# SebastianBitsch/SRGAN-ST

Measured on AMD Instinct MI355X. Metric: HR images/sec (96px x4, B=16/GPU) G+D+ST-loss step, higher is better.
Workload: dtype f32; 1 GPU; srgan_x4_hr96_b16_G+D+ST-loss step: adv+mse+st, D updated every step (train.py:116-164; BASELINE metric); global_batch=16, hr=96, lr=24, parallelism=dp1, hip_graph=True, d_update_interval=1, d_sr_forward=run: all three discriminator forwards of train.py:136,155,158

## Files before the change

include/srganst.h:

```cpp
#ifndef SRGANST_H
#define SRGANST_H
#include <stdint.h>
#ifdef __cplusplus
extern "C" {
#endif

const char* sst_last_error(void);
int sst_version(void);
const char* sst_arch(void);
int sst_clear_error(void);
int sst_reload_env(void);

int sst_st_loss_workspace(int B, int H, int W, int64_t* partial_floats);
int sst_st_loss_fwd(const float* sr, const float* gt, float* loss, float* gS, float* partials,
                    unsigned* counter, int B, int H, int W, float sigma, float rho, int normalize,
                    void* stream);
int sst_st_loss_bwd(const float* sr, const float* gS, float* dsr, const float* scale_dev,
                    float scale_host, int accumulate, int B, int H, int W, float sigma, float rho,
                    void* stream);
int sst_st_maps_workspace(int B, int H, int W, int64_t* tile_floats);
int sst_st_maps(const float* x, const float* gt, float* Sx, float* Sgt, float* Fx, float* Fgt, float* d, float* tile_sums,
                int B, int H, int W, float sigma, float rho, int normalize, void* stream);
int sst_st_pixel_loss_fwd(const float* sr, const float* gt, float* loss, float* gS, float* partials, unsigned* counter,
                          float* pix_loss, float* pix_partials, int pix_mode, int B, int H, int W, float sigma, float rho,
                          int normalize, void* stream);
int sst_st_pixel_loss_bwd(const float* sr, const float* gt, const float* gS, float* dsr, const float* scale_dev, float scale_host,
                          float pix_weight, int pix_mode, int accumulate, int B, int H, int W, float sigma, float rho,
                          void* stream);

int64_t sst_conv_packed_floats(int Cout, int Cin, int ksize);
int sst_conv_pack(const float* w, float* wp, int Cout, int Cin, int ksize, int mode, void* stream);
int sst_conv_pack_multi(const void* jobs, int njobs, int total_blocks, void* stream);
int sst_conv_mtiles(int B, int Ho, int Wo);
int sst_conv_stat_tiles(int B, int H, int W, int Cin, int Cout, int ksize, int stride);
const char* sst_conv_kernel_name(int B, int H, int W, int Cin, int Cout, int ksize, int stride, int out_mode, int fused_in);
const char* sst_conv_wgrad_kernel_name(int B, int H, int W, int Cin, int Cout, int ksize, int stride, int njobs);
long sst_debug_big_tile_launches(void);
long sst_debug_band_launches(void);
long sst_debug_wgrad_band_launches(void);
int sst_debug_mfma_peak(float* out, int blocks, int iters, void* stream);
int sst_debug_bf16x3(const float* A, const float* B, float* C32, float* C3, int K, int mode, int blocks, void* stream);
int sst_debug_stamp(unsigned long long* out, int slot, void* stream);
int sst_conv_fwd(const float* x, const float* wp, float* y, float* y_pre, const float* bias,
                 const float* in_scale, const float* in_shift, const float* in_slope,
                 float in_slope_const, int in_act, const float* residual, float* stats,
                 float* stats_cnt, int out_mode, int B, int H, int W, int Cin, int Cout, int ksize,
                 int stride, void* stream);
int sst_conv_pipe_supported(int B, int H, int W, int Cin, int Cout, int ksize, int stride);
int sst_conv_pipe_stat_tiles(int B, int H, int W, int Cin, int Cout, int ksize, int stride);
int64_t sst_conv_pipe_ws_floats(int B, int H, int W, int Cin, int Cout, int ksize, int stride);
int sst_conv_pipe_fwd(const float* x, const float* wp, float* y, const float* bias, const float* in_scale,
                      const float* in_shift, const float* in_slope, float in_slope_const, int in_act, float* stats,
                      float* stats_cnt, const float* epi_y, const float* epi_scale, const float* epi_shift,
                      const float* epi_slope, float epi_slope_const, int epi_act, float* epi_partial, float* ws, int B,
                      int H, int W, int Cin, int Cout, int ksize, int stride, void* stream);
int sst_conv_pipe_groups_ok(int B, int H, int W, int Cin, int Cout, int ksize, int stride, int grp_images);
int sst_conv_pipe_fwd_grp(const float* x, const float* wp, float* y, const float* bias, const float* in_scale,
                          const float* in_shift, const float* in_slope, float in_slope_const, int in_act, float* stats,
                          float* stats_cnt, const float* epi_y, const float* epi_scale, const float* epi_shift,
                          const float* epi_slope, float epi_slope_const, int epi_act, float* epi_partial, float* ws, int B,
                          int H, int W, int Cin, int Cout, int ksize, int stride, int grp_images, void* stream);
int sst_conv_ns_supported(int B, int H, int W, int Cin, int Cout, int ksize, int stride, int out_mode);
int sst_conv_ns_fwd(const float* x, const float* wp, float* y, const float* bias, const float* in_scale,
                    const float* in_shift, const float* in_slope, float in_slope_const, int in_act, float* stats,
                    float* stats_cnt, const float* epi_y, const float* epi_scale, const float* epi_shift,
                    const float* epi_slope, float epi_slope_const, int epi_act, float* epi_partial, int B, int H, int W,
                    int Cin, int Cout, int ksize, int stride, int out_mode, int grp_images, void* stream);
int sst_conv_s2_dgrad_pipe_supported(int B, int H, int W, int Cin, int Cout);
int64_t sst_conv_s2_dgrad_pipe_ws_floats(int B, int H, int W, int Cin, int Cout);
int sst_conv_s2_dgrad_pipe(const float* dy, const float* wp, float* dx, float* ws, int B, int H, int W, int Cin, int Cout,
                           void* stream);
int sst_conv_s2_dgrad_pipe_stat_tiles(int B, int H, int W, int Cin, int Cout);
int sst_conv_s2_dgrad_pipe_bwdstats(const float* dy, const float* wp, float* dx, float* ws, const float* epi_y,
                                    const float* epi_scale, const float* epi_shift, const float* epi_slope,
                                    float epi_slope_const, int epi_act, float* epi_partial, int B, int H, int W, int Cin,
                                    int Cout, void* stream);
int sst_conv_s2_dgrad_pipe_groups_ok(int B, int H, int W, int Cin, int Cout, int grp_images);
int sst_conv_s2_dgrad_pipe_bwdstats_grp(const float* dy, const float* wp, float* dx, float* ws, const float* epi_y,
                                    const float* epi_scale, const float* epi_shift, const float* epi_slope,
                                    float epi_slope_const, int epi_act, float* epi_partial, int B, int H, int W, int Cin,
                                    int Cout, int grp_images, void* stream);
int sst_conv_dgrad_bwdstats(const float* x, const float* wp, float* y, const float* residual, const float* epi_y,
                            const float* epi_scale, const float* epi_shift, const float* epi_slope,
                            float epi_slope_const, int epi_act, float* epi_partial, int B, int H, int W, int Cin,
                            int Cout, int ksize, void* stream);
int sst_conv_acc_supported(int B, int H, int W, int Cin, int Cout, int ksize, int stride);
int sst_conv_fwd_acc(const float* x, const float* in2, float* side_out, const float* ones, const float* wp, float* y,
                     const float* bias, const float* in_slope, float in_slope_const, int in_act, const double* in_acc,
                     const float* in_gamma, const float* in_beta, float in_n, float eps, float momentum, float* o_mean,
                     float* o_rstd, float* o_scale, float* o_shift, float* run_mean, float* run_var, double* st_acc,
                     int nrep, int B, int H, int W, int Cin, int Cout, int ksize, void* stream);
int sst_conv_dgrad_fused_acc(const float* g, const float* y2, const float* in_scale, const float* in_shift,
                             const float* in_slope, float in_slope_const, int in_act, float* dy_out, const float* wp,
                             float* out, const float* residual, const float* epi_y, const float* epi_scale,
                             const float* epi_shift, const float* epi_slope, float epi_slope_const, int epi_act,
                             const double* bw_in_acc, const float* mean, const float* rstd, const float* gamma, float n,
                             float* dgamma, float* dbeta, float* dslope, double* bw_st_acc, int nrep, int B, int H,
                             int W, int Cin, int Cout, int ksize, void* stream);
int sst_bn_finalize_acc(const double* acc, int nrep, int C, float n, const float* gamma, const float* beta,
                        float* run_mean, float* run_var, float* mean, float* rstd, float* scale, float* shift,
                        float eps, float momentum, void* stream);
int sst_conv_fwd_resin(const float* x, const float* y2, const float* ones, const float* bn_scale, const float* bn_shift,
                       float* h_out, const float* wp, float* y, const float* bias, float* stats, float* stats_cnt,
                       int B, int H, int W, int Cin, int Cout, int ksize, void* stream);
int sst_conv_dgrad_fused(const float* g, const float* y2, const float* cA, const float* cB, const float* cC,
                         const float* in_scale, const float* in_shift, const float* in_slope, float in_slope_const,
                         int in_act, float* dy_out, const float* wp, float* out, const float* residual,
                         const float* epi_y, const float* epi_scale, const float* epi_shift, const float* epi_slope,
                         float epi_slope_const, int epi_act, float* epi_partial, int B, int H, int W, int Cin, int Cout,
                         int ksize, void* stream);
int sst_conv_wgrad_chunks(int B, int Ho, int Wo, int Cin, int Cout, int ksize);
int sst_conv_wgrad_chunks2(int B, int H, int W, int Cin, int Cout, int ksize, int stride, int njobs);
int sst_conv_wgrad(const float* x, const float* dy, float* slab, float* dw, const float* in_scale,
                   const float* in_shift, const float* in_slope, float in_slope_const, int in_act,
                   int B, int H, int W, int Cin, int Cout, int stride, int ksize, int accumulate,
                   void* stream);
int sst_conv_wgrad_groups_ok(int B, int H, int W, int Cin, int Cout, int ksize, int stride, int grp_images);
int sst_conv_wgrad_grp(const float* x, const float* dy, float* slab, float* dw, const float* in_scale,
                   const float* in_shift, const float* in_slope, float in_slope_const, int in_act,
                   int B, int H, int W, int Cin, int Cout, int stride, int ksize, int accumulate,
                       int grp_images, void* stream);
int sst_conv_wgrad_pending_reduce(int B, int H, int W, int Cin, int Cout, int ksize, int stride, int has_in_scale, int in_act);
int sst_wgrad_reduce_multi(const void* jobs, int njobs, void* stream);
int sst_wgrad_c3_supported(int C, int ksize);
int64_t sst_wgrad_c3_slab_floats(int B, int H, int W, int C);
int sst_wgrad_c3(const float* big, const float* small, float* slab, float* dw, const float* in_slope,
                 float in_slope_const, int in_act, int kind, int B, int H, int W, int C, int accumulate,
                 void* stream);

int64_t sst_conv9_c3_packed_floats(int Cout_eff);
int sst_conv9_c3_pack(const float* w, float* wp, int Cout, int Cin, int mode, void* stream);
int sst_conv9_c3_fwd(const float* x, const float* wp, float* y, const float* bias, int B, int H, int W,
                     int Cout, void* stream);
int64_t sst_conv9_to3_packed_floats(int C);
int sst_conv9_to3_pack(const float* w, float* wp, int C, void* stream);
int sst_conv9_to3_fwd(const float* x, const float* wp, float* y, float* y_pre, const float* bias,
                      const float* in_slope, float in_slope_const, int in_act, int B, int H, int W, int C,
                      void* stream);

int64_t sst_conv_s2_dgrad_packed_floats(int Cout, int Cin);
int sst_conv_s2_dgrad_pack(const float* w, float* wp, int Cout, int Cin, void* stream);
int sst_conv_s2_dgrad(const float* dy, const float* wp, float* dx, int B, int H, int W, int Cin, int Cout,
                      void* stream);
int sst_conv_s2_dgrad_tiles(int B, int H, int W);
const char* sst_conv_s2_dgrad_kernel_name(int B, int H, int W, int Cin, int Cout, int fused);
int sst_conv_s2_dgrad_fused(const float* g, const float* y2, const float* cA, const float* cB, const float* cC,
                            const float* in_scale, const float* in_shift, const float* in_slope, float in_slope_const,
                            int in_act, float* dy_out, const float* wp, float* dx, const float* epi_y,
                            const float* epi_scale, const float* epi_shift, const float* epi_slope, float epi_slope_const,
                            int epi_act, float* epi_partial, int B, int H, int W, int Cin, int Cout, void* stream);

int sst_conv_wgrad_grouped(const void* jobs, int njobs, int B, int H, int W, int Cin, int Cout, int stride,
                           int ksize, int accumulate, void* stream);

int sst_bn_finalize(const float* stats, const float* cnt, int ntiles, int C, const float* gamma,
                    const float* beta, float* run_mean, float* run_var, float* mean, float* rstd,
                    float* scale, float* shift, float eps, float momentum, void* stream);
int sst_bn_finalize_grp(const float* stats, const float* cnt, int ntiles, int C, int groups, const float* gamma,
                        const float* beta, float* run_mean, float* run_var, float* mean, float* rstd, float* scale,
                        float* shift, float eps, float momentum, void* stream);
int sst_bn_eval_affine(const float* gamma, const float* beta, const float* run_mean,
                       const float* run_var, float* scale, float* shift, int C, float eps, void* stream);
int sst_bn_residual(const float* y, const float* scale, const float* shift, const float* res,
                    const float* res_slope, float* out, int64_t R, int C, void* stream);
int sst_bwd_reduce_blocks(int64_t R, int C);
int sst_bwd_reduce(const float* g, const float* g2, const float* y, const float* scale,
                   const float* shift, const float* slope, float slope_const, int act, float* partial,
                   int64_t R, int C, void* stream);
int sst_bwd_finalize(const float* partial, int nblk, int C, float n, const float* mean,
                     const float* rstd, const float* gamma, float* dgamma, float* dbeta, float* cA,
                     float* cB, float* cC, float* dslope, int accumulate, void* stream);
int sst_bwd_reduce_grp(const float* g, const float* g2, const float* y, const float* scale, const float* shift,
                       const float* slope, float slope_const, int act, float* partial, int64_t R, int C, int groups,
                       void* stream);
int sst_bwd_finalize_grp(const float* partial, int nblk, int C, float n, int groups, const float* mean, const float* rstd,
                         const float* gamma, float* dgamma, float* dbeta, float* cA, float* cB, float* cC, int accumulate,
                         void* stream);
int sst_bwd_apply_grp(const float* g, const float* g2, const float* y, const float* scale, const float* shift,
                      const float* slope, float slope_const, int act, const float* cA, const float* cB, const float* cC,
                      float* dy, int64_t R, int C, int groups, void* stream);
int sst_bwd_finalize_wide(const float* partial, int nblk, int C, float n, const float* mean, const float* rstd,
                          const float* gamma, float* dgamma, float* dbeta, float* cA, float* cB, float* cC,
                          float* dslope, int accumulate, float* scratch, unsigned* counter, void* stream);
int sst_act_bwd_partial_blocks(int64_t stored_rows);
int sst_act_bwd_partial(const float* g, const float* g2, const float* y, const float* slope, float slope_const,
                        float* dy, float* partial, int64_t R, int C, int unshuffle_H, int unshuffle_W, void* stream);
int sst_bwd_apply(const float* g, const float* g2, const float* y, const float* scale,
                  const float* shift, const float* slope, float slope_const, int act, const float* cA,
                  const float* cB, const float* cC, float* dy, int64_t R, int C, int unshuffle_H,
                  int unshuffle_W, void* stream);
int sst_add(const float* a, const float* b, float* out, int64_t n, void* stream);

int sst_transpose(const float* src, float* dst, int B, int C, int H, int W, int to_nchw, void* stream);
int sst_feat_loss_fwd(const float* x, const float* gt, const float* scale, const float* shift, float slope, int C,
                      float* loss, float* partials, unsigned* counter, int64_t n, int mode, void* stream);
int sst_feat_loss_bwd(const float* x, const float* gt, const float* scale, const float* shift, float slope, int C,
                      float* dx, const float* scale_dev, float scale_host, int accumulate, int64_t n, int mode,
                      void* stream);
int sst_transpose_affine(const float* src, float* dst, int B, int C, int H, int W, int to_nchw,
                         const float* scale, const float* shift, void* stream);
int sst_maxpool_relu_fwd(const float* y, float* out, int B, int H, int W, int C, void* stream);
int sst_maxpool_relu_bwd(const float* g, const float* y, float* dy, int B, int H, int W, int C, void* stream);
int sst_clamp_bwd_blocks(int B, int H, int W);
int sst_clamp_bwd(const float* g, const float* pre, float* out, float* partial, float* dbias,
                  int accumulate, int B, int C, int H, int W, void* stream);
int sst_pixel_loss_blocks(int64_t n);
int sst_pixel_loss_fwd(const float* x, const float* gt, float* loss, float* partials, unsigned* counter,
                       int64_t n, int mode, void* stream);
int sst_pixel_loss_bwd(const float* x, const float* gt, float* dx, const float* scale_dev,
                       float scale_host, int accumulate, int64_t n, int mode, void* stream);
int sst_bce_logits(const float* logits, float target, float* loss, float* dlogits,
                   const float* scale_dev, float scale_host, int n, void* stream);
int sst_bicubic(const float* x, float* y, const float* wy, const int* iy, const float* wx, const int* ix,
                int64_t planes, int H, int W, int oh, int ow, int Ty, int Tx, int round_grid, void* stream);
int sst_gather_batch(const uint8_t* src, int64_t N, const int* idx, int B, int H, int W, const float* lut, float* gt, float* lr,
                     const float* wy, const int* iy, const float* wx, const int* ix, int oh, int ow, int Ty, int Tx,
                     void* stream);
int sst_gather_crops(const uint8_t* arena, int64_t arena_bytes, const int64_t* table, int64_t N, const int* desc, int B, int S,
                     const float* lut, float* gt, float* lr, const float* wy, const int* iy, const float* wx, const int* ix,
                     int oh, int ow, int Ty, int Tx, int span, void* stream);
int sst_image_metrics_workspace(int B, int H, int W, int64_t* partial_doubles);
int sst_image_metrics(const float* sr, const float* hr, int B, int H, int W, double* out, uint8_t* sr_u8, uint8_t* hr_u8,
                      double* workspace, void* stream);
int sst_bb_blocks(int B, int H, int W);
int sst_bb_feature_dim(int mode);
int sst_bb_patches(const float* img, float* cand, float* cnrm, int B, int H, int W, int ncand_total, int cand_off,
                   int mode, const float* st_mats, void* stream);
int sst_bb_match(const float* sr, const float* cand, const float* cnrm, int* ind, float* dsr, float* partials, int B,
                 int H, int W, int ncand, float alpha, float beta, int criterion_l2, int mode, const float* st_mats,
                 void* stream);
int sst_bb_match_dist(const float* sr, const float* cand, const float* cnrm, int* ind, float* dsr, float* partials, int B,
                 int H, int W, int ncand, float alpha, float beta, int criterion_l2, int mode, const float* st_mats, int dist_l1,
                      void* stream);
int sst_bbg_patches(int H, int W, int k, int pad, int stride);
int sst_bbg_blocks(int B, int np);
int sst_bbg_unfold(const float* img, float* table, float* nrm, int B, int H, int W, int k, int pad, int stride, int nrows_total,
                   int row_off, void* stream);
int sst_bbg_match(const float* srf, const float* cand, const float* cnrm, int* ind, float* gfeat, float* partials, int B, int np,
                  int ncand, int D, float alpha, float beta, int criterion_l2, int dist_l1, void* stream);
int sst_bbg_fold(const float* gfeat, float* dsr, int B, int H, int W, int k, int pad, int stride, void* stream);
int sst_weighted_sum(const float* const* terms, const float* weights, int n, float* out, float* weighted,
                     void* stream);

int sst_linear_ksplit(int M, int N, int K);
int sst_linear_fwd(const float* x, const float* w, const float* bias, float* y, float* slab, int M, int N,
                   int K, void* stream);
int sst_linear_dgrad(const float* dy, const float* w, float* dx, int M, int N, int K, int nhwc_C,
                     int nhwc_HW, void* stream);
int sst_linear_wgrad(const float* dy, const float* x, float* dw, float* db, int M, int N, int K,
                     int accumulate, void* stream);
int sst_head_fwd(const float* h, const float* w, const float* b, float* y, int M, int N, int K, float slope,
                 void* stream);
int sst_head_bwd(const float* h, const float* w, const float* dy, float* dh, float* dw, float* db, int M,
                 int N, int K, float slope, int accumulate, void* stream);
int sst_flatten_act(const float* y, const float* scale, const float* shift, float slope, int act,
                    float* flat, int B, int HW, int C, void* stream);
int sst_flatten_act_grp(const float* y, const float* scale, const float* shift, float slope, int act,
                        float* flat, int B, int HW, int C, int grp_images, void* stream);

int sst_adam_flat(float* p, const float* g, float* m, float* v, int64_t n, const float* lr, float* steps,
                  int nsteps, double beta1, double beta2, double eps, double weight_decay, void* stream);

#ifdef __cplusplus
}
#endif
#endif
```

srgan-st_amd/csrc/api.hip:

```cpp
#include "common.h"
#include <cstring>

static thread_local char g_err[512] = "";

int sst_set_error(int code, const char* fmt, ...) {
  va_list ap;
  va_start(ap, fmt);
  vsnprintf(g_err, sizeof(g_err), fmt, ap);
  va_end(ap);
  return code;
}

SST_API const char* sst_last_error(void) { return g_err; }

#include <cstdlib>
#include <mutex>
namespace {
struct EnvEntry { char name[40]; char value[24]; bool set; };
constexpr int ENV_MAX = 64;
EnvEntry g_env[ENV_MAX];
int g_env_n = 0;
std::mutex g_env_mu;
}
const char* sst_env(const char* name) {
  std::lock_guard<std::mutex> lk(g_env_mu);
  for (int i = 0; i < g_env_n; ++i)
    if (!strcmp(g_env[i].name, name)) return g_env[i].set ? g_env[i].value : nullptr;
  const char* v = std::getenv(name);
  if (g_env_n == ENV_MAX || strlen(name) >= sizeof(g_env[0].name)) return v;
  EnvEntry& e = g_env[g_env_n++];
  snprintf(e.name, sizeof(e.name), "%s", name);
  e.set = v != nullptr;
  snprintf(e.value, sizeof(e.value), "%s", v ? v : "");
  return e.set ? e.value : nullptr;
}
SST_API int sst_reload_env(void) {
  std::lock_guard<std::mutex> lk(g_env_mu);
  g_env_n = 0;
  return SST_OK;
}
SST_API int sst_version(void) { return 100; }
SST_API const char* sst_arch(void) { return "gfx950"; }
SST_API int sst_clear_error(void) { g_err[0] = 0; return (int)hipGetLastError(); }

typedef float f32x16_t __attribute__((ext_vector_type(16)));
template <int SHAPE>
__global__ __launch_bounds__(256) void mfma_peak_kernel(float* out, int iters) {
  f32x16_t acc[4];
#pragma unroll
  for (int k = 0; k < 4; ++k)
#pragma unroll
    for (int r = 0; r < 16; ++r) acc[k][r] = 0.f;
  unsigned ua = threadIdx.x * 2654435761u + blockIdx.x, ub = ua ^ 0x9e3779b9u;
  for (int i = 0; i < iters; ++i) {
    ua = ua * 1664525u + 1013904223u;
    ub = ub * 22695477u + 1u;
    const float a = __uint_as_float((ua >> 9) | 0x3f800000u) - 1.5f, b = __uint_as_float((ub >> 9) | 0x3f800000u) - 1.5f;
#pragma unroll
    for (int k = 0; k < 4; ++k) acc[k] = __builtin_amdgcn_mfma_f32_32x32x2f32(a, b, acc[k], 0, 0, 0);
  }
  float s = 0.f;
#pragma unroll
  for (int k = 0; k < 4; ++k)
#pragma unroll
    for (int r = 0; r < 16; ++r) s += acc[k][r];
  if (s == 12345.678f) out[0] = s;
}
SST_API int sst_debug_mfma_peak(float* out, int blocks, int iters, void* stream) {
  SST_REQUIRE(out && blocks > 0 && iters > 0, "sst_debug_mfma_peak: bad argument");
  mfma_peak_kernel<0><<<blocks, 256, 0, sst_stream(stream)>>>(out, iters);
  SST_LAUNCH_CHECK("mfma_peak_kernel");
  return SST_OK;
}

typedef __bf16 bf16x8_t __attribute__((ext_vector_type(8)));
__device__ __forceinline__ void split3(float x, __bf16& a, __bf16& b, __bf16& c) {
  a = (__bf16)x;
  const float r1 = x - (float)a;
  b = (__bf16)r1;
  c = (__bf16)(r1 - (float)b);
}
__global__ __launch_bounds__(64) void bf16x3_probe_kernel(const float* __restrict__ A, const float* __restrict__ B, float* __restrict__ C32,
                                                          float* __restrict__ C3, int K) {
  const int lane = threadIdx.x, li = lane & 31, lh = lane >> 5;
  f32x16_t acc32, acc3;
#pragma unroll
  for (int r = 0; r < 16; ++r) acc32[r] = acc3[r] = 0.f;
  for (int k = 0; k < K; k += 2)
    acc32 = __builtin_amdgcn_mfma_f32_32x32x2f32(A[li * K + k + lh], B[(k + lh) * 32 + li], acc32, 0, 0, 0);
  for (int k = 0; k < K; k += 16) {
    bf16x8_t a[3], b[3];
#pragma unroll
    for (int j = 0; j < 8; ++j) {
      __bf16 t0, t1, t2;
      split3(A[li * K + k + 8 * lh + j], t0, t1, t2);
      a[0][j] = t0; a[1][j] = t1; a[2][j] = t2;
      split3(B[(k + 8 * lh + j) * 32 + li], t0, t1, t2);
      b[0][j] = t0; b[1][j] = t1; b[2][j] = t2;
    }
    acc3 = __builtin_amdgcn_mfma_f32_32x32x16_bf16(a[2], b[0], acc3, 0, 0, 0);
    acc3 = __builtin_amdgcn_mfma_f32_32x32x16_bf16(a[1], b[1], acc3, 0, 0, 0);
    acc3 = __builtin_amdgcn_mfma_f32_32x32x16_bf16(a[0], b[2], acc3, 0, 0, 0);
    acc3 = __builtin_amdgcn_mfma_f32_32x32x16_bf16(a[1], b[0], acc3, 0, 0, 0);
    acc3 = __builtin_amdgcn_mfma_f32_32x32x16_bf16(a[0], b[1], acc3, 0, 0, 0);
    acc3 = __builtin_amdgcn_mfma_f32_32x32x16_bf16(a[0], b[0], acc3, 0, 0, 0);
  }
#pragma unroll
  for (int r = 0; r < 16; ++r) {
    const int row = (r & 3) + 8 * (r >> 2) + 4 * lh;
    C32[row * 32 + li] = acc32[r];
    C3[row * 32 + li] = acc3[r];
  }
}
typedef unsigned u32x4_t __attribute__((ext_vector_type(4)));
__global__ __launch_bounds__(256) void bf16x3_rate_kernel(float* out, int iters) {
  f32x16_t acc[4];
#pragma unroll
  for (int k = 0; k < 4; ++k)
#pragma unroll
    for (int r = 0; r < 16; ++r) acc[k][r] = 0.f;
  u32x4_t a[3], b[3];
  unsigned ua = threadIdx.x * 2654435761u + blockIdx.x;
#pragma unroll
  for (int t = 0; t < 3; ++t)
#pragma unroll
    for (int j = 0; j < 4; ++j) {
      ua = ua * 1664525u + 1013904223u;
      a[t][j] = (ua & 0x807F807Fu) | 0x3F803F80u;
      ua = ua * 1664525u + 1013904223u;
      b[t][j] = (ua & 0x807F807Fu) | 0x3F803F80u;
    }
  for (int i = 0; i < iters; i += 12) {
#pragma unroll
    for (int u = 0; u < 12; ++u) {
      ua = ua * 1664525u + 1013904223u;
      a[u % 3][u / 3] ^= ua & 0x807F807Fu;
      b[(u + 1) % 3][u / 3] ^= (ua >> 3) & 0x807F807Fu;
      bf16x8_t av[3], bv[3];
#pragma unroll
      for (int t = 0; t < 3; ++t) {
        av[t] = __builtin_bit_cast(bf16x8_t, a[t]);
        bv[t] = __builtin_bit_cast(bf16x8_t, b[t]);
      }
#pragma unroll
      for (int k = 0; k < 4; ++k) {
        acc[k] = __builtin_amdgcn_mfma_f32_32x32x16_bf16(av[2], bv[0], acc[k], 0, 0, 0);
        acc[k] = __builtin_amdgcn_mfma_f32_32x32x16_bf16(av[1], bv[1], acc[k], 0, 0, 0);
        acc[k] = __builtin_amdgcn_mfma_f32_32x32x16_bf16(av[0], bv[2], acc[k], 0, 0, 0);
        acc[k] = __builtin_amdgcn_mfma_f32_32x32x16_bf16(av[1], bv[0], acc[k], 0, 0, 0);
        acc[k] = __builtin_amdgcn_mfma_f32_32x32x16_bf16(av[0], bv[1], acc[k], 0, 0, 0);
        acc[k] = __builtin_amdgcn_mfma_f32_32x32x16_bf16(av[0], bv[0], acc[k], 0, 0, 0);
      }
    }
  }
  float s = 0.f;
#pragma unroll
  for (int k = 0; k < 4; ++k)
#pragma unroll
    for (int r = 0; r < 16; ++r) s += acc[k][r];
  if (s == 12345.678f) out[0] = s;
}
SST_API int sst_debug_bf16x3(const float* A, const float* B, float* C32, float* C3, int K, int mode, int blocks, void* stream) {
  if (mode == 0) {
    SST_REQUIRE(A && B && C32 && C3 && K > 0 && K % 16 == 0, "sst_debug_bf16x3: bad argument");
    bf16x3_probe_kernel<<<1, 64, 0, sst_stream(stream)>>>(A, B, C32, C3, K);
  } else {
    SST_REQUIRE(C32 && K > 0 && blocks > 0, "sst_debug_bf16x3: bad argument");
    bf16x3_rate_kernel<<<blocks, 256, 0, sst_stream(stream)>>>(C32, K);
  }
  SST_LAUNCH_CHECK("bf16x3 probe");
  return SST_OK;
}

__global__ void stamp_kernel(unsigned long long* out, int slot) { out[slot] = wall_clock64(); }
SST_API int sst_debug_stamp(unsigned long long* out, int slot, void* stream) {
  SST_REQUIRE(out && slot >= 0, "sst_debug_stamp: bad argument");
  stamp_kernel<<<1, 1, 0, sst_stream(stream)>>>(out, slot);
  SST_LAUNCH_CHECK("stamp_kernel");
  return SST_OK;
}
```

srgan-st_amd/csrc/common.h:

```cpp
#pragma once
#include <hip/hip_runtime.h>
#include <cstdarg>
#include <cstdio>
#include <cstdint>

#define SST_API extern "C" __attribute__((visibility("default")))

enum : int {
  SST_OK = 0,
  SST_ERR_ARG = -1,
  SST_ERR_UNSUPPORTED = -2,
  SST_ERR_HIP = -3,
};

int sst_set_error(int code, const char* fmt, ...);

#define SST_REQUIRE(cond, ...)                                   \
  do {                                                           \
    if (!(cond)) return sst_set_error(SST_ERR_ARG, __VA_ARGS__); \
  } while (0)

#define SST_LAUNCH_CHECK(name)                                                                   \
  do {                                                                                           \
    hipError_t e_ = hipGetLastError();                                                           \
    if (e_ != hipSuccess) return sst_set_error(SST_ERR_HIP, "%s: %s", name, hipGetErrorString(e_)); \
  } while (0)

const char* sst_env(const char* name);

static inline hipStream_t sst_stream(void* s) { return reinterpret_cast<hipStream_t>(s); }

__device__ __forceinline__ float wave_sum(float v) {
#pragma unroll
  for (int o = 32; o > 0; o >>= 1) v += __shfl_xor(v, o, 64);
  return v;
}

template <int NT>
__device__ __forceinline__ float block_sum(float v, float* red) {
  v = wave_sum(v);
  const int wid = threadIdx.x >> 6, lane = threadIdx.x & 63;
  __syncthreads();
  if (lane == 0) red[wid] = v;
  __syncthreads();
  float t = 0.f;
#pragma unroll
  for (int i = 0; i < NT / 64; ++i) t += red[i];
  return t;
}

__device__ __forceinline__ double wave_sum_d(double v) {
#pragma unroll
  for (int o = 32; o > 0; o >>= 1) v += __shfl_xor(v, o, 64);
  return v;
}
template <int NT>
__device__ __forceinline__ double block_sum_d(double v, double* red) {
  v = wave_sum_d(v);
  const int wid = threadIdx.x >> 6, lane = threadIdx.x & 63;
  __syncthreads();
  if (lane == 0) red[wid] = v;
  __syncthreads();
  double t = 0.0;
#pragma unroll
  for (int i = 0; i < NT / 64; ++i) t += red[i];
  return t;
}

__device__ __forceinline__ unsigned publish_and_ticket(unsigned* counter) {
  __builtin_amdgcn_fence(__ATOMIC_RELEASE, "agent");
  asm volatile("s_waitcnt vmcnt(0)" ::: "memory");
  return __hip_atomic_fetch_add(counter, 1u, __ATOMIC_RELAXED, __HIP_MEMORY_SCOPE_AGENT);
}
__device__ __forceinline__ void acquire_after_ticket() {
  __builtin_amdgcn_fence(__ATOMIC_ACQUIRE, "agent");
  asm volatile("s_waitcnt vmcnt(0)" ::: "memory");
}
__device__ __forceinline__ float load_agent(const float* p) {
  return __hip_atomic_load(p, __ATOMIC_RELAXED, __HIP_MEMORY_SCOPE_AGENT);
}

template <int NT>
__device__ __forceinline__ bool last_block_total(const float* partials, unsigned* counter, unsigned nblk, unsigned* s_flag,
                                                 float* red, float& total) {
  if (threadIdx.x == 0) *s_flag = (publish_and_ticket(counter) == nblk - 1) ? 1u : 0u;
  __syncthreads();
  if (!*s_flag) return false;
  if (threadIdx.x == 0) acquire_after_ticket();
  __syncthreads();
  float t = 0.f;
  for (unsigned i = threadIdx.x; i < nblk; i += NT) t += load_agent(partials + i);
  total = block_sum<NT>(t, red);
  if (threadIdx.x == 0) __hip_atomic_store(counter, 0u, __ATOMIC_RELAXED, __HIP_MEMORY_SCOPE_AGENT);
  return true;
}
```

srgan-st_amd/csrc/conv_fwd.hip:

```cpp
#include "conv_common.h"
#include <cstdlib>
#include "conv_epilogue.h"

int sst_launch_conv_fwd2(const Conv3Args& a, int stride, hipStream_t st);
int sst_launch_conv_band(const Conv3Args& a, int R, hipStream_t st, const BandAcc* acc);
int sst_conv_band_rows(int B, int H, int W, int Cin, int Cout, int ksize, int stride);

namespace {

constexpr int BIG_MIN_TILES = 2048;
inline bool use_big_tiles(const Conv3Args& a, int ksize) {
  if (ksize != 3 || a.Cout < 64 || a.in2 || a.side_out) return false;
  if (a.out_mode != OUT_NHWC && a.out_mode != OUT_SHUFFLE && a.out_mode != OUT_STRIDE2) return false;
  if (const char* e = sst_env("SST_CONV_BIG")) return atoi(e) != 0;
  const long tiles = (long)a.B * ((a.Ho + 7) / 8) * ((a.Wo + 7) / 8) * ((a.Cout + 63) / 64);
  return tiles >= BIG_MIN_TILES;
}

template <int KS, int S>
__device__ __forceinline__ void conv_fwd_body(const Conv3Args& a, const int bx, const int by) {
  const int KK = a.ksy * a.ksx;
  constexpr int PW = (TWO - 1) * S + KS, PH = (THO - 1) * S + KS, NP = PW * PH;
  constexpr int LDS_FLOATS = (NP * LDSC > 4 * 32 * 33) ? NP * LDSC : 4 * 32 * 33;
  __shared__ __attribute__((aligned(16))) float lds[LDS_FLOATS];
// ... 316 lines not shown
#pragma unroll
        for (int i = 0; i < 6; ++i) bq[(g + 1) & 1][i] = load_b((g + 1) * 6 + i);
      }
#pragma unroll
      for (int i = 0; i < 6; ++i) {
        const int q = g * 6 + i, combo = q >> 1, cls = CLS_OF[combo], tap = TAP_OF[combo];
        const int ntx = 1 + (cls & 1), jy = tap / ntx, jx = tap - jy * ntx;
        const int ks = 2 * wave + (q & 1);
        if (ks < nks) {
          const f32x4 av = *reinterpret_cast<const f32x4*>(&lds[a_base + (jy * PW + jx) * LDSC + ks * 8]);
          const f32x4 bv = bq[g & 1][i];
#pragma unroll
          for (int j = 0; j < 4; ++j) acc[cls] = __builtin_amdgcn_mfma_f32_32x32x2f32(av[j], bv[j], acc[cls], 0, 0, 0);
        }
      }
    }
  }
  const bool tile_ok = oy0 < nh && ox0 < nw;
#pragma unroll
  for (int cls = 0; cls < 4; ++cls) {
    Conv3Args t = a;
    t.sub_y = cls >> 1;
    t.sub_x = cls & 1;
    t.Ho = nh;
    t.Wo = nw;
    t.in2 = nullptr;
    t.side_out = nullptr;
    if (FUSED && a.epi_partial) t.epi_partial = a.epi_partial + (size_t)c.tile_base[cls] * 3 * a.Cout;
    if (!FUSED) t.epi_partial = nullptr;
    conv_tile_epilogue(t, lds, sstat, acc[cls], b, oy0, ox0, nf, mt, tile_ok, tid, wave, lane);
  }
}

__global__ __launch_bounds__(CONV_NT) void conv3_c3in_kernel(const float* __restrict__ x, const float* __restrict__ wp,
                                                             const float* __restrict__ bias, float* __restrict__ y, int B, int H, int W,
                                                             int Cout) {
  extern __shared__ __attribute__((aligned(16))) float xs[];
  const int RS = (W + 2) * 3 + 1;
  const int b = blockIdx.x / H, oy = blockIdx.x - b * H;
  for (int i = threadIdx.x; i < 3 * RS; i += CONV_NT) {
    const int r = i / RS, o = i - r * RS;
    const int px = o / 3 - 1, iy = oy - 1 + r;
    float v = 0.f;
    if (o < (W + 2) * 3 && (unsigned)px < (unsigned)W && (unsigned)iy < (unsigned)H)
      v = x[(((size_t)b * H + iy) * W + px) * 3 + (o - (px + 1) * 3)];
    xs[i] = v;
  }
  const int nq = Cout >> 2;
  const int cq = threadIdx.x % nq, pl = threadIdx.x / nq, npl = CONV_NT / nq;
  const int co = cq * 4;
  float w[27][4];
#pragma unroll
  for (int t = 0; t < 9; ++t)
#pragma unroll
    for (int ci = 0; ci < 3; ++ci)
#pragma unroll
      for (int j = 0; j < 4; ++j) w[t * 3 + ci][j] = wp[((((co + j) >> 5) * 9 + t) * 512 + ((co + j) & 31)) * 4 + ci];
  f32x4 bv = {0.f, 0.f, 0.f, 0.f};
  if (bias) bv = *reinterpret_cast<const f32x4*>(bias + co);
  __syncthreads();
  for (int ox = pl; ox < W; ox += npl) {
    f32x4 acc = bv;
#pragma unroll
    for (int ky = 0; ky < 3; ++ky) {
      const float* row = xs + ky * RS + ox * 3;
#pragma unroll
      for (int q = 0; q < 9; ++q) {
        const float v = row[q];
#pragma unroll
        for (int j = 0; j < 4; ++j) acc[j] = fmaf(v, w[ky * 9 + q][j], acc[j]);
      }
    }
    *reinterpret_cast<f32x4*>(y + (((size_t)b * H + oy) * W + ox) * Cout + co) = acc;
  }
}

constexpr int C3F_ROW = 104;
constexpr int C3F_OST = 68;
__global__ __launch_bounds__(CONV_NT) void conv3_c3in_mfma_kernel(const float* __restrict__ x, const float* __restrict__ wp,
                                                                  const float* __restrict__ bias, float* __restrict__ y, int B, int H,
                                                                  int W, int ntiles) {
  __shared__ __attribute__((aligned(16))) float ost[4][32 * C3F_OST];
  __shared__ float wl[15 * 2 * 64];
  constexpr int Cout = 64;
  const int tid = threadIdx.x, wave = __builtin_amdgcn_readfirstlane(tid >> 6), lane = tid & 63;
  const int li = lane & 31, lh = lane >> 5;
  for (int i = tid; i < 15 * 2 * 64; i += CONV_NT) {
    const int l = i & 63, h = (i >> 6) & 1, ks = i >> 7;
    const int ky = ks / 5, j = 2 * (ks - ky * 5) + (l >> 5);
    wl[i] = j < 9 ? wp[((size_t)(h * 9 + ky * 3 + j / 3) * 512 + (l & 31)) * 4 + j % 3] : 0.f;
  }
  float* const ps = ost[wave];
  const int tpr = W >> 5;
  float pv[5];
  auto load_patch = [&](int t) {
    const int b = t / (H * tpr), rem = t - b * (H * tpr);
    const int oy = rem / tpr, x0 = (rem - oy * tpr) << 5;
#pragma unroll
    for (int u = 0; u < 5; ++u) {
      const int i = lane + 64 * u;
      const int r = i / C3F_ROW, c = i - r * C3F_ROW;
      const int iy = oy - 1 + r, fx = (x0 - 1) * 3 + c;
      const bool ok = i < 3 * C3F_ROW + 8 && r < 3 && c < 102 && (unsigned)iy < (unsigned)H && (unsigned)fx < (unsigned)(W * 3);
      pv[u] = ok ? x[((size_t)b * H + iy) * W * 3 + fx] : 0.f;
    }
  };
  int t = blockIdx.x * 4 + wave;
  if (t < ntiles) load_patch(t);
  __syncthreads();
  const float* const bl = ps + li * 3 + lh;
  for (; t < ntiles; t += gridDim.x * 4) {
#pragma unroll
    for (int u = 0; u < 5; ++u) {
      const int i = lane + 64 * u;
      if (i < 3 * C3F_ROW + 8) ps[i] = pv[u];
    }
    const int tn = t + gridDim.x * 4;
    if (tn < ntiles) load_patch(tn);
    f32x16 acc[2];
#pragma unroll
    for (int h = 0; h < 2; ++h)
#pragma unroll
      for (int r = 0; r < 16; ++r) acc[h][r] = 0.f;
#pragma unroll
    for (int ky = 0; ky < 3; ++ky)
#pragma unroll
      for (int s2 = 0; s2 < 5; ++s2) {
        const float bv = bl[ky * C3F_ROW + 2 * s2];
        const int ks = ky * 5 + s2;
        acc[0] = __builtin_amdgcn_mfma_f32_32x32x2f32(wl[(ks * 2 + 0) * 64 + lane], bv, acc[0], 0, 0, 0);
        acc[1] = __builtin_amdgcn_mfma_f32_32x32x2f32(wl[(ks * 2 + 1) * 64 + lane], bv, acc[1], 0, 0, 0);
      }
#pragma unroll
    for (int h = 0; h < 2; ++h)
#pragma unroll
      for (int q = 0; q < 4; ++q) {
        const int c = 32 * h + 8 * q + 4 * lh;
        f32x4 v = {acc[h][4 * q], acc[h][4 * q + 1], acc[h][4 * q + 2], acc[h][4 * q + 3]};
        if (bias) v += *reinterpret_cast<const f32x4*>(bias + c);
        *reinterpret_cast<f32x4*>(ps + li * C3F_OST + c) = v;
      }
    const int b = t / (H * tpr), rem = t - b * (H * tpr);
    const int oy = rem / tpr, x0 = (rem - oy * tpr) << 5;
    float* const yp = y + (((size_t)b * H + oy) * W + x0) * Cout;
#pragma unroll
    for (int i = 0; i < 8; ++i) {
      const int idx = lane + 64 * i, px = idx >> 4, c4 = (idx & 15) * 4;
      *reinterpret_cast<f32x4*>(yp + (size_t)px * Cout + c4) = *reinterpret_cast<const f32x4*>(ps + px * C3F_OST + c4);
    }
  }
}

typedef float f32x4c __attribute__((ext_vector_type(4)));
__global__ __launch_bounds__(CONV_NT) void conv3_to3_kernel(const float* __restrict__ x, const float* __restrict__ wp,
                                                            float* __restrict__ y, int B, int H, int W, int nmt, int nsp) {
  extern __shared__ __attribute__((aligned(16))) float pl_all[];
  const int wave = __builtin_amdgcn_readfirstlane(threadIdx.x >> 6), lane = threadIdx.x & 63;
  const int seg = blockIdx.x * 4 + wave;
  if (seg >= B * H * nsp) return;
  const int row = seg / nsp, Ws = W / nsp, xb = (seg - row * nsp) * Ws;
  const int b = row / H, oy = row - b * H;
  const int lm = lane & 15, lg = lane >> 4;
  float* const pl = pl_all + (size_t)wave * nmt * 16 * 12;
  float bw[3][4][4];
  {
    const int tx = lm / 3, ci = lm - tx * 3;
#pragma unroll
    for (int ty = 0; ty < 3; ++ty)
#pragma unroll
      for (int q = 0; q < 4; ++q)
#pragma unroll
        for (int t = 0; t < 4; ++t) {
          const int co = 16 * q + 4 * lg + t, tap = ty * 3 + tx;
          bw[ty][q][t] = lm < 9 ? wp[(size_t)(tap * 8 + (co >> 3)) * 256 + (((co & 7) >> 2) * 32 + ci) * 4 + (co & 3)] : 0.f;
        }
  }
  auto load_tile = [&](int mt, f32x4c (&a)[3][4]) {
    const int xp = xb + mt * 16 + lm - 1;
#pragma unroll
    for (int ty = 0; ty < 3; ++ty) {
      const int iy = oy - 1 + ty;
      const bool ok = (unsigned)iy < (unsigned)H && (unsigned)xp < (unsigned)W;
      const float* src = x + (((size_t)b * H + (ok ? iy : 0)) * W + (ok ? xp : 0)) * 64 + 4 * lg;
#pragma unroll
      for (int q = 0; q < 4; ++q) {
        const f32x4c v = *reinterpret_cast<const f32x4c*>(src + 16 * q);
        a[ty][q] = ok ? v : f32x4c{0.f, 0.f, 0.f, 0.f};
      }
    }
  };
  f32x4c ac[3][4], an[3][4];
  load_tile(0, ac);
  for (int mt = 0; mt < nmt; ++mt) {
    if (mt + 1 < nmt) load_tile(mt + 1, an);
    f32x4c acc = {0.f, 0.f, 0.f, 0.f};
#pragma unroll
    for (int ty = 0; ty < 3; ++ty)
#pragma unroll
      for (int q = 0; q < 4; ++q)
#pragma unroll
        for (int t = 0; t < 4; ++t) acc = __builtin_amdgcn_mfma_f32_16x16x4f32(ac[ty][q][t], bw[ty][q][t], acc, 0, 0, 0);
    if (lm < 9) {
#pragma unroll
      for (int r = 0; r < 4; ++r) pl[(mt * 16 + 4 * lg + r) * 12 + lm] = acc[r];
    }
#pragma unroll
    for (int ty = 0; ty < 3; ++ty)
#pragma unroll
      for (int q = 0; q < 4; ++q) ac[ty][q] = an[ty][q];
  }
  float* const out = y + (((size_t)b * H + oy) * W + xb) * 3;
  for (int i = lane; i < 3 * Ws; i += 64) {
    const int xo = i / 3, ci = i - xo * 3;
    out[i] = (pl[xo * 12 + ci] + pl[(xo + 1) * 12 + 3 + ci]) + pl[(xo + 2) * 12 + 6 + ci];
  }
}

__global__ void pack_conv_kernel(const float* __restrict__ w, float* __restrict__ wp, int Cout, int Cin, int KK,
                                 int mode, int64_t total) {
  const int O = mode ? Cin : Cout, I = mode ? Cout : Cin;
  const int ncb = (I + 63) / 64;
  const int64_t base = packed_floats_base(O, I, KK);
  for (int64_t idx = blockIdx.x * (int64_t)blockDim.x + threadIdx.x; idx < total; idx += (int64_t)gridDim.x * blockDim.x) {
    if (idx >= base) {
      const int64_t q = idx - base;
      const int l = (q >> 2) & 63, tap = (q >> 10) % 9;
      const int o = (int)((q >> 10) / 9) * 16 + (l & 15), i = ((q >> 8) & 3) * 16 + (l >> 4) * 4 + (q & 3);
      wp[idx] = mode == 0 ? w[((size_t)o * Cin + i) * KK + tap] : w[((size_t)i * Cin + o) * KK + (KK - 1 - tap)];
      continue;
    }
    const int j = idx & 3;
    const int l = (idx >> 2) & 63;
    const int ks = (idx >> 8) & 7;
    int64_t rest = idx >> 11;
    const int tap = rest % KK;
    rest /= KK;
    const int cbk = rest % ncb;
    const int of = rest / ncb;
    const int o = of * 32 + (l & 31);
    const int i = cbk * 64 + ks * 8 + (l >> 5) * 4 + j;
    float v = 0.f;
    if (of < (O + 31) / 32 && o < O && i < I) {
      if (mode == 0)
        v = w[((size_t)o * Cin + i) * KK + tap];
      else
        v = w[((size_t)i * Cin + o) * KK + (KK - 1 - tap)];
    }
    wp[idx] = v;
  }
}

struct PackJob {
  const float* w;
  float* wp;
  int Cout, Cin, KK, mode;
  long long total;
  long long block_begin;
};
constexpr int PM_MAXJOBS = 512;
__global__ __launch_bounds__(256) void pack_multi_kernel(const PackJob* __restrict__ jobs, int njobs) {
  __shared__ long long s_begin[PM_MAXJOBS];
  for (int j = threadIdx.x; j < njobs; j += 256) s_begin[j] = jobs[j].block_begin;
  __syncthreads();
  int lo = 0, hi = njobs - 1;
  while (lo < hi) {
    const int mid = (lo + hi + 1) >> 1;
    if (s_begin[mid] <= (long long)blockIdx.x) lo = mid; else hi = mid - 1;
  }
  const PackJob jb = jobs[lo];
  if (jb.mode >= 2) {
    const long long base = ((long long)blockIdx.x - jb.block_begin) * 1024;
#pragma unroll
    for (int u = 0; u < 4; ++u) {
      const long long idx = base + u * 256 + threadIdx.x;
      if (idx >= jb.total) break;
      if (jb.mode == 5) { jb.wp[idx] = 0.f; continue; }
      if (jb.mode == 6) { reinterpret_cast<long long*>(jb.wp)[idx] += jb.Cout; continue; }
      jb.wp[idx] = jb.mode == 4 ? pack_to3_value(jb.w, idx, jb.Cin) : pack_c3_value(jb.w, idx, jb.Cout, jb.Cin, jb.mode - 2);
    }
    return;
  }
  const int O = jb.mode ? jb.Cin : jb.Cout, I = jb.mode ? jb.Cout : jb.Cin;
  const int ncb = (I + 63) / 64;
  const unsigned wl = (unsigned)((long long)blockIdx.x - jb.block_begin);
  const unsigned bbase = (unsigned)packed_floats_base(O, I, jb.KK), total = (unsigned)jb.total;
  if (jb.KK == 9) {
    __shared__ float tile[64 * 145];
    const unsigned nhalf = (unsigned)((O + 31) / 32) * ncb * 9 * 2;
    const bool band = wl >= nhalf + PACK_PAD / 1024;
    if (!band && wl >= nhalf) {
#pragma unroll
      for (int u = 0; u < 4; ++u) jb.wp[wl * 1024 + u * 256 + threadIdx.x] = 0.f;
      return;
    }
    if (!band) {
      const unsigned ngrp = nhalf / 9;
      if (wl >= ngrp) return;
      const int h = wl & 1, cbk = (wl >> 1) % (unsigned)ncb, of = (wl >> 1) / (unsigned)ncb;
      const int o0 = of * 32, i0 = cbk * 64 + h * 32;
      float v[36];
#pragma unroll
      for (int k = 0; k < 36; ++k) {
        const int e = k * 256 + threadIdx.x;
        const int r = e / 288, c = e - r * 288, q = c / 9;
        v[k] = 0.f;
        if (jb.mode == 0) {
          if (o0 + r < O && i0 + q < I) v[k] = jb.w[((size_t)(o0 + r) * jb.Cin + i0) * 9 + c];
        } else {
          if (i0 + r < I && o0 + q < O) v[k] = jb.w[((size_t)(i0 + r) * jb.Cin + o0) * 9 + c];
        }
      }
#pragma unroll
      for (int k = 0; k < 36; ++k) {
        const int e = k * 256 + threadIdx.x;
        const int r = e / 288, c = e - r * 288;
        tile[r * 289 + c] = v[k];
      }
      __syncthreads();
      for (int tap = 0; tap < 9; ++tap) {
        float* dst = jb.wp + ((size_t)((of * ncb + cbk) * 9 + tap) * 2 + h) * 1024;
#pragma unroll
        for (int u = 0; u < 4; ++u) {
          const int x = u * 256 + threadIdx.x;
          const int j = x & 3, l = (x >> 2) & 63, ks = x >> 8;
          const int ol = l & 31, il = ks * 8 + (l >> 5) * 4 + j;
          dst[x] = jb.mode == 0 ? tile[ol * 289 + il * 9 + tap] : tile[il * 289 + ol * 9 + (8 - tap)];
        }
      }
      return;
    }
    const unsigned wb = wl - nhalf - PACK_PAD / 1024;
    if (wb >= (unsigned)(O / 16)) return;
    const int o0 = wb * 16;
    {
      float v[36];
      const int RL = jb.mode == 0 ? 576 : 144;
#pragma unroll
      for (int k = 0; k < 36; ++k) {
        const int e = k * 256 + threadIdx.x;
        const int r = e / RL, c = e - r * RL;
        v[k] = jb.mode == 0 ? jb.w[((size_t)(o0 + r) * jb.Cin) * 9 + c] : jb.w[((size_t)r * jb.Cin + o0) * 9 + c];
      }
#pragma unroll
      for (int k = 0; k < 36; ++k) {
        const int e = k * 256 + threadIdx.x;
        const int r = e / RL, c = e - r * RL;
        tile[r * (RL + 1) + c] = v[k];
      }
    }
    __syncthreads();
    for (int tap = 0; tap < 9; ++tap) {
      float* dst = jb.wp + bbase + ((size_t)wb * 9 + tap) * 1024;
#pragma unroll
      for (int u = 0; u < 4; ++u) {
        const int x = u * 256 + threadIdx.x;
        const int l = (x >> 2) & 63;
        const int ol = l & 15, i = (x >> 8) * 16 + (l >> 4) * 4 + (x & 3);
        dst[x] = jb.mode == 0 ? tile[ol * 577 + i * 9 + tap] : tile[i * 145 + ol * 9 + (8 - tap)];
      }
    }
    return;
  }
  const unsigned base = wl * 1024;
  const unsigned top = base >> 11;
  int tap = top % (unsigned)jb.KK;
  const unsigned rr = top / (unsigned)jb.KK;
  int a2 = (int)(rr % (unsigned)ncb) * 64, a1 = (int)(rr / (unsigned)ncb) * 32;
  tap = __builtin_amdgcn_readfirstlane(tap); a1 = __builtin_amdgcn_readfirstlane(a1); a2 = __builtin_amdgcn_readfirstlane(a2);
#pragma unroll
  for (int u = 0; u < 4; ++u) {
    const unsigned idx = base + u * 256 + threadIdx.x;
    if (idx >= total) break;
    const int j = idx & 3, l = (idx >> 2) & 63, ks = (idx >> 8) & 7;
    const int o = a1 + (l & 31), i = a2 + ks * 8 + (l >> 5) * 4 + j;
    float v = 0.f;
    if (a1 < ((O + 31) / 32) * 32 && o < O && i < I) {
      if (jb.mode == 0)
        v = jb.w[((size_t)o * jb.Cin + i) * jb.KK + tap];
      else
        v = jb.w[((size_t)i * jb.Cin + o) * jb.KK + (jb.KK - 1 - tap)];
    }
    jb.wp[idx] = v;
  }
}

__host__ __device__ inline int64_t s2_class_offset(int cls, int Cin, int Cout) {
  int64_t off = 0;
  for (int c = 0; c < cls; ++c) off += packed_floats(Cin, Cout, (1 + (c >> 1)) * (1 + (c & 1)));
  return off;
}
__global__ void pack_s2_dgrad_kernel(const float* __restrict__ w, float* __restrict__ wp, int Cout, int Cin) {
  if (blockIdx.y == 4) {
    const int O = Cin, I = Cout, ncb = (I + 63) / 64;
    float* dst = wp + s2_class_offset(4, Cin, Cout);
    const int64_t total = packed_floats_base(O, I, 9);
    for (int64_t idx = blockIdx.x * (int64_t)blockDim.x + threadIdx.x; idx < total; idx += (int64_t)gridDim.x * blockDim.x) {
      const int j = idx & 3, l = (idx >> 2) & 63, ks = (idx >> 8) & 7;
      int64_t rest = idx >> 11;
      const int combo = rest % 9;
      rest /= 9;
      const int cbk = rest % ncb;
      const int of = rest / ncb;
      const int o = of * 32 + (l & 31), i = cbk * 64 + ks * 8 + (l >> 5) * 4 + j;
      float v = 0.f;
      if (of < (O + 31) / 32 && o < O && i < I) {
        const int cls = combo == 0 ? 0 : (combo < 3 ? 1 : (combo < 5 ? 2 : 3));
        const int tap = combo == 0 ? 0 : (combo < 3 ? combo - 1 : (combo < 5 ? combo - 3 : combo - 5));
        const int py = cls >> 1, px = cls & 1, ntx = 1 + px;
        const int jy = tap / ntx, jx = tap - jy * ntx;
        const int ky = py ? (jy ? 0 : 2) : 1, kx = px ? (jx ? 0 : 2) : 1;
        v = w[(((size_t)i * Cin + o) * 3 + ky) * 3 + kx];
      }
      dst[idx] = v;
    }
    return;
  }
  const int cls = blockIdx.y, py = cls >> 1, px = cls & 1;
  const int nty = 1 + py, ntx = 1 + px, KKc = nty * ntx;
  const int O = Cin, I = Cout, ncb = (I + 63) / 64;
  float* dst = wp + s2_class_offset(cls, Cin, Cout);
  const int64_t total = packed_floats(O, I, KKc);
  for (int64_t idx = blockIdx.x * (int64_t)blockDim.x + threadIdx.x; idx < total; idx += (int64_t)gridDim.x * blockDim.x) {
    const int j = idx & 3, l = (idx >> 2) & 63, ks = (idx >> 8) & 7;
    int64_t rest = idx >> 11;
    const int tap = rest % KKc;
    rest /= KKc;
    const int cbk = rest % ncb;
    const int of = rest / ncb;
    const int o = of * 32 + (l & 31), i = cbk * 64 + ks * 8 + (l >> 5) * 4 + j;
    float v = 0.f;
    if (of < (O + 31) / 32 && o < O && i < I) {
      const int jy = tap / ntx, jx = tap - jy * ntx;
      const int ky = py ? (jy ? 0 : 2) : 1, kx = px ? (jx ? 0 : 2) : 1;
      v = w[(((size_t)i * Cin + o) * 3 + ky) * 3 + kx];
    }
    dst[idx] = v;
  }
}

}

SST_API int64_t sst_conv_packed_floats(int Cout, int Cin, int ksize) { return packed_floats(Cout, Cin, ksize * ksize); }

SST_API int sst_conv_pack(const float* w, float* wp, int Cout, int Cin, int ksize, int mode, void* stream) {
  SST_REQUIRE(w && wp && Cout > 0 && Cin > 0 && (ksize == 3 || ksize == 9) && (mode == 0 || mode == 1),
              "sst_conv_pack: bad argument");
  const int O = mode ? Cin : Cout, I = mode ? Cout : Cin;
  const int64_t total = packed_floats(O, I, ksize * ksize);
  const int blocks = (int)((total + 255) / 256 < 2048 ? (total + 255) / 256 : 2048);
  pack_conv_kernel<<<blocks, 256, 0, sst_stream(stream)>>>(w, wp, Cout, Cin, ksize * ksize, mode, total);
  SST_LAUNCH_CHECK("pack_conv_kernel");
  return SST_OK;
}

SST_API int sst_conv_pack_multi(const void* jobs, int njobs, int total_blocks, void* stream) {
  SST_REQUIRE(jobs && njobs > 0 && njobs <= PM_MAXJOBS && total_blocks > 0, "sst_conv_pack_multi: bad argument (at most %d jobs)", PM_MAXJOBS);
  static_assert(sizeof(PackJob) == 48, "PackJob layout");
  pack_multi_kernel<<<total_blocks, 256, 0, sst_stream(stream)>>>(reinterpret_cast<const PackJob*>(jobs), njobs);
  SST_LAUNCH_CHECK("pack_multi_kernel");
  return SST_OK;
}

SST_API int sst_conv_mtiles(int B, int Ho, int Wo) { return B * ((Ho + THO - 1) / THO) * ((Wo + TWO - 1) / TWO); }

SST_API int sst_conv_stat_tiles(int B, int H, int W, int Cin, int Cout, int ksize, int stride) {
  const int R = sst_conv_band_rows(B, H, W, Cin, Cout, ksize, stride);
  if (R) return B * (H / R);
  const int p = ksize / 2;
  return sst_conv_mtiles(B, (H + 2 * p - ksize) / stride + 1, (W + 2 * p - ksize) / stride + 1);
}

namespace {
enum class FwdKind { TO3, C3IN_MFMA, C3IN, BAND, BIG_TILES, GENERAL };
struct FwdSel {
  FwdKind kind;
  int nsp, nmt;
  int wgs;
  int R;
  size_t lds;
  const char* name;
};

void conv_shape_args(Conv3Args& a, int B, int H, int W, int Cin, int Cout, int ksize, int stride) {
  a.B = B; a.H = H; a.W = W; a.Cin = Cin; a.Cout = Cout;
  a.ksy = a.ksx = ksize; a.pad_y = a.pad_x = ksize / 2; a.sub_y = a.sub_x = 0; a.Hy = a.Wy = 0;
  a.Ho = (H + 2 * (ksize / 2) - ksize) / stride + 1;
  a.Wo = (W + 2 * (ksize / 2) - ksize) / stride + 1;
}

FwdSel conv_fwd_select(const Conv3Args& a, int ksize, int stride, int dbg_bits) {
  FwdSel s{};
  const bool bare = ksize == 3 && stride == 1 && a.out_mode == OUT_NHWC && !a.in_scale && a.in_act == ACT_NONE && !a.residual && !a.stats &&
                    !a.y_pre && !a.epi_partial && !a.in2 && dbg_bits == 0;
  if (bare && a.Cin == 64 && a.Cout == 3 && !a.bias && !sst_env("SST_NO_TO3")) {
    s.nsp = (a.W % 32 == 0 && a.W >= 64 && !sst_env("SST_TO3_NO_SPLIT")) ? 2 : 1;
    s.nmt = (a.W / s.nsp + 2 + 15) / 16;
    s.lds = (size_t)4 * s.nmt * 16 * 12 * sizeof(float);
    if (s.lds <= 60 * 1024) {
      s.kind = FwdKind::TO3; s.name = "conv3_to3_kernel";
      return s;
    }
  }
  if (bare && a.Cin == 3 && (a.Cout & 3) == 0 && CONV_NT % (a.Cout >> 2) == 0 && !sst_env("SST_NO_C3IN")) {
    if ((a.W & 31) == 0 && a.Cout == 64 && !sst_env("SST_NO_C3IN_MFMA")) {
      s.kind = FwdKind::C3IN_MFMA; s.name = "conv3_c3in_mfma_kernel";
      s.wgs = (a.B * a.H * (a.W >> 5) + 3) / 4;
      return s;
    }
    s.lds = (size_t)3 * ((a.W + 2) * 3 + 1) * sizeof(float);
    if (s.lds <= 48 * 1024) {
      s.kind = FwdKind::C3IN; s.name = "conv3_c3in_kernel";
      return s;
    }
  }
  if (a.out_mode == OUT_NHWC && !(dbg_bits & 8)) {
    s.R = sst_conv_band_rows(a.B, a.H, a.W, a.Cin, a.Cout, ksize, stride);
    if (s.R) {
      s.kind = FwdKind::BAND; s.name = s.R * a.W / 16 == 9 ? "conv_band_kernel<9>" : "conv_band_kernel<3>";
      return s;
    }
  }
  if (dbg_bits == 0 && use_big_tiles(a, ksize)) {
    s.kind = FwdKind::BIG_TILES; s.name = stride == 1 ? "conv_fwd2_kernel<1>" : "conv_fwd2_kernel<2>";
    return s;
  }
  s.kind = FwdKind::GENERAL;
  s.name = ksize != 3 ? "conv_fwd_kernel<9, 1>" : (stride == 1 ? "conv_fwd_kernel<3, 1>" : "conv_fwd_kernel<3, 2>");
  return s;
}
}

static int conv_fwd_impl(const float* x, const float* wp, float* y, float* y_pre, const float* bias, const float* in_scale,
                         const float* in_shift, const float* in_slope, float in_slope_const, int in_act,
                         const float* residual, float* stats, float* stats_cnt, int out_mode, int B, int H, int W, int Cin,
                         int Cout, int ksize, int stride, const float* epi_y, const float* epi_scale, const float* epi_shift,
                         const float* epi_slope, float epi_slope_const, int epi_act, float* epi_partial, void* stream,
                         const float* in2 = nullptr, const float* in_cA = nullptr, const float* in_cB = nullptr,
                         const float* in_cC = nullptr, float* side_out = nullptr, const BandAcc* band_acc = nullptr) {
  SST_REQUIRE(x && wp && y, "sst_conv_fwd: null pointer");
  SST_REQUIRE(B > 0 && H > 0 && W > 0 && Cin > 0 && Cout > 0 && (stride == 1 || stride == 2) && (ksize == 3 || ksize == 9),
              "sst_conv_fwd: bad shape B=%d H=%d W=%d Cin=%d Cout=%d k=%d stride=%d", B, H, W, Cin, Cout, ksize, stride);
  SST_REQUIRE(!(ksize == 9 && stride == 2), "sst_conv_fwd: 9x9 stride 2 not built");
  SST_REQUIRE((in_scale == nullptr) == (in_shift == nullptr), "sst_conv_fwd: in_scale/in_shift must come together");
  SST_REQUIRE(!stats || stats_cnt, "sst_conv_fwd: stats needs stats_cnt");
  const int dbg_bits = out_mode >> 8;
  out_mode &= 0xff;
  SST_REQUIRE(out_mode >= 0 && out_mode <= 3, "sst_conv_fwd: bad out_mode");
  SST_REQUIRE(out_mode != OUT_SHUFFLE || (Cout & 3) == 0, "sst_conv_fwd: shuffle store needs Cout %% 4 == 0");
  SST_REQUIRE(out_mode == OUT_NHWC || (!residual && !stats && !epi_partial), "sst_conv_fwd: residual/stats only with NHWC store");
  SST_REQUIRE(!epi_partial || (epi_y && !stats && ((epi_scale == nullptr) == (epi_shift == nullptr))),
              "sst_conv_fwd: backward partials need epi_y and exclude forward stats");
  Conv3Args a;
  a.x = x; a.wp = wp; a.y = y; a.y_pre = y_pre; a.bias = bias; a.in_scale = in_scale; a.in_shift = in_shift;
  a.in_slope = in_slope; a.in_slope_const = in_slope_const; a.in_act = in_act; a.residual = residual; a.stats = stats;
  a.stats_cnt = stats_cnt; a.out_mode = out_mode; a.dbg = dbg_bits;
  a.epi_y = epi_y; a.epi_scale = epi_scale; a.epi_shift = epi_shift; a.epi_slope = epi_slope;
  a.epi_slope_const = epi_slope_const; a.epi_act = epi_act; a.epi_partial = epi_partial;
  a.in2 = in2; a.in_cA = in_cA; a.in_cB = in_cB; a.in_cC = in_cC; a.side_out = side_out;
  SST_REQUIRE(!in2 || ((Cin & 3) == 0 && stride == 1), "sst_conv_fwd: fused BN-backward input needs Cin %% 4 == 0, stride 1");
  SST_REQUIRE(!in_cA || (in2 && in_cB && in_cC), "sst_conv_fwd: cA/cB/cC need in2");
  conv_shape_args(a, B, H, W, Cin, Cout, ksize, stride);
  SST_REQUIRE(out_mode != OUT_UNSHUFFLE || ((a.Ho & 1) == 0 && (a.Wo & 1) == 0), "sst_conv_fwd: unshuffle needs even Ho,Wo");
  const int64_t mt = sst_conv_mtiles(B, a.Ho, a.Wo);
  SST_REQUIRE(mt < (1ll << 31), "sst_conv_fwd: too many tiles");
  dim3 grid((unsigned)mt, (Cout + 31) / 32);
  hipStream_t st = sst_stream(stream);
  const size_t extra_lds = (size_t)(dbg_bits >> 4) * 1024;
  a.dbg = dbg_bits & 15;
  const FwdSel s = conv_fwd_select(a, ksize, stride, dbg_bits);
  switch (s.kind) {
    case FwdKind::TO3:
      conv3_to3_kernel<<<(unsigned)((B * H * s.nsp + 3) / 4), CONV_NT, s.lds, st>>>(x, wp, y, B, H, W, s.nmt, s.nsp);
      break;
    case FwdKind::C3IN_MFMA:
      conv3_c3in_mfma_kernel<<<(unsigned)(s.wgs < 768 ? s.wgs : 768), CONV_NT, 0, st>>>(x, wp, bias, y, B, H, W, B * H * (W >> 5));
      break;
    case FwdKind::C3IN:
      conv3_c3in_kernel<<<(unsigned)(B * H), CONV_NT, s.lds, st>>>(x, wp, bias, y, B, H, W, Cout);
      break;
    case FwdKind::BAND: return sst_launch_conv_band(a, s.R, st, band_acc);
    case FwdKind::BIG_TILES: return sst_launch_conv_fwd2(a, stride, st);
    case FwdKind::GENERAL:
      if (ksize == 3 && stride == 1)
        conv_fwd_kernel<3, 1><<<grid, CONV_NT, extra_lds, st>>>(a);
      else if (ksize == 3)
        conv_fwd_kernel<3, 2><<<grid, CONV_NT, 0, st>>>(a);
      else
        conv_fwd_kernel<9, 1><<<grid, CONV_NT, 0, st>>>(a);
      break;
  }
  SST_LAUNCH_CHECK(s.name);
  return SST_OK;
}

SST_API const char* sst_conv_kernel_name(int B, int H, int W, int Cin, int Cout, int ksize, int stride, int out_mode, int fused_in) {
  Conv3Args a{};
  conv_shape_args(a, B, H, W, Cin, Cout, ksize, stride);
  a.out_mode = out_mode;
  a.in2 = fused_in ? reinterpret_cast<const float*>(1) : nullptr;
  return conv_fwd_select(a, ksize, stride, 0).name;
}

SST_API int sst_conv_fwd(const float* x, const float* wp, float* y, float* y_pre, const float* bias, const float* in_scale,
                         const float* in_shift, const float* in_slope, float in_slope_const, int in_act,
                         const float* residual, float* stats, float* stats_cnt, int out_mode, int B, int H, int W, int Cin,
                         int Cout, int ksize, int stride, void* stream) {
  return conv_fwd_impl(x, wp, y, y_pre, bias, in_scale, in_shift, in_slope, in_slope_const, in_act, residual, stats, stats_cnt,
                       out_mode, B, H, W, Cin, Cout, ksize, stride, nullptr, nullptr, nullptr, nullptr, 0.f, 0, nullptr, stream);
}

SST_API int sst_conv_dgrad_bwdstats(const float* x, const float* wp, float* y, const float* residual, const float* epi_y,
                                    const float* epi_scale, const float* epi_shift, const float* epi_slope,
                                    float epi_slope_const, int epi_act, float* epi_partial, int B, int H, int W, int Cin,
                                    int Cout, int ksize, void* stream) {
  SST_REQUIRE(epi_y && epi_partial, "sst_conv_dgrad_bwdstats: epi_y / epi_partial");
  return conv_fwd_impl(x, wp, y, nullptr, nullptr, nullptr, nullptr, nullptr, 0.f, ACT_NONE, residual, nullptr, nullptr, OUT_NHWC,
                       B, H, W, Cin, Cout, ksize, 1, epi_y, epi_scale, epi_shift, epi_slope, epi_slope_const, epi_act, epi_partial,
                       stream);
}

SST_API int sst_conv_dgrad_fused(const float* g, const float* y2, const float* cA, const float* cB, const float* cC,
                                 const float* in_scale, const float* in_shift, const float* in_slope, float in_slope_const,
                                 int in_act, float* dy_out, const float* wp, float* out, const float* residual,
                                 const float* epi_y, const float* epi_scale, const float* epi_shift, const float* epi_slope,
                                 float epi_slope_const, int epi_act, float* epi_partial, int B, int H, int W, int Cin, int Cout,
                                 int ksize, void* stream) {
  SST_REQUIRE(g && y2 && dy_out, "sst_conv_dgrad_fused: g / y2 / dy_out");
  SST_REQUIRE((epi_partial == nullptr) == (epi_y == nullptr), "sst_conv_dgrad_fused: epi_y and epi_partial come together");
  return conv_fwd_impl(g, wp, out, nullptr, nullptr, in_scale, in_shift, in_slope, in_slope_const, in_act, residual, nullptr,
                       nullptr, OUT_NHWC, B, H, W, Cin, Cout, ksize, 1, epi_y, epi_scale, epi_shift, epi_slope, epi_slope_const,
                       epi_act, epi_partial, stream, y2, cA, cB, cC, dy_out);
}

SST_API int sst_conv_fwd_resin(const float* x, const float* y2, const float* ones, const float* bn_scale, const float* bn_shift,
                               float* h_out, const float* wp, float* y, const float* bias, float* stats, float* stats_cnt, int B,
                               int H, int W, int Cin, int Cout, int ksize, void* stream) {
  SST_REQUIRE(x && y2 && ones && bn_scale && bn_shift && h_out, "sst_conv_fwd_resin: null pointer");
  return conv_fwd_impl(x, wp, y, nullptr, bias, nullptr, nullptr, nullptr, 0.f, ACT_NONE, nullptr, stats, stats_cnt, OUT_NHWC, B, H, W,
                       Cin, Cout, ksize, 1, nullptr, nullptr, nullptr, nullptr, 0.f, 0, nullptr, stream, y2, ones, bn_scale, bn_shift,
                       h_out);
}

SST_API int sst_conv_acc_supported(int B, int H, int W, int Cin, int Cout, int ksize, int stride) {
  return Cin == 64 && sst_conv_band_rows(B, H, W, Cin, Cout, ksize, stride) != 0;
}

SST_API int sst_conv_fwd_acc(const float* x, const float* in2, float* side_out, const float* ones, const float* wp, float* y,
                             const float* bias, const float* in_slope, float in_slope_const, int in_act, const double* in_acc,
                             const float* in_gamma, const float* in_beta, float in_n, float eps, float momentum, float* o_mean,
                             float* o_rstd, float* o_scale, float* o_shift, float* run_mean, float* run_var, double* st_acc,
                             int nrep, int B, int H, int W, int Cin, int Cout, int ksize, void* stream) {
  SST_REQUIRE(sst_conv_acc_supported(B, H, W, Cin, Cout, ksize, 1), "sst_conv_fwd_acc: shape not covered by the band kernel");
  SST_REQUIRE(nrep > 0 && nrep <= 16 && (in_acc || st_acc), "sst_conv_fwd_acc: no accumulator given / nrep > 16");
  SST_REQUIRE(!in_acc || (in_gamma && in_beta && in_n > 0.f), "sst_conv_fwd_acc: in_acc needs gamma / beta / n");
  SST_REQUIRE(!in2 || (side_out && ones), "sst_conv_fwd_acc: residual form needs side_out and the ones vector");
  BandAcc ba{};
  ba.st_acc = st_acc; ba.in_acc = in_acc; ba.nrep = nrep; ba.in_target = in2 ? 1 : 0;
  ba.in_gamma = in_gamma; ba.in_beta = in_beta; ba.in_n = in_n; ba.in_eps = eps; ba.momentum = momentum;
  ba.o_mean = o_mean; ba.o_rstd = o_rstd; ba.o_scale = o_scale; ba.o_shift = o_shift; ba.run_mean = run_mean; ba.run_var = run_var;
  return conv_fwd_impl(x, wp, y, nullptr, bias, nullptr, nullptr, in_slope, in_slope_const, in_act, nullptr, nullptr, nullptr, OUT_NHWC,
                       B, H, W, Cin, Cout, ksize, 1, nullptr, nullptr, nullptr, nullptr, 0.f, 0, nullptr, stream, in2, in2 ? ones : nullptr,
                       in2 ? ones : nullptr, in2 ? ones : nullptr, side_out, &ba);
}

SST_API int sst_conv_dgrad_fused_acc(const float* g, const float* y2, const float* in_scale, const float* in_shift, const float* in_slope,
                                     float in_slope_const, int in_act, float* dy_out, const float* wp, float* out,
                                     const float* residual, const float* epi_y, const float* epi_scale, const float* epi_shift,
                                     const float* epi_slope, float epi_slope_const, int epi_act, const double* bw_in_acc,
                                     const float* mean, const float* rstd, const float* gamma, float n, float* dgamma, float* dbeta,
                                     float* dslope, double* bw_st_acc, int nrep, int B, int H, int W, int Cin, int Cout, int ksize,
                                     void* stream) {
  SST_REQUIRE(sst_conv_acc_supported(B, H, W, Cin, Cout, ksize, 1), "sst_conv_dgrad_fused_acc: shape not covered by the band kernel");
  SST_REQUIRE(nrep > 0 && nrep <= 16 && (bw_in_acc || bw_st_acc), "sst_conv_dgrad_fused_acc: no accumulator given / nrep > 16");
  SST_REQUIRE(!bw_in_acc || (y2 && dy_out && mean && rstd && gamma && dgamma && dbeta && n > 0.f),
              "sst_conv_dgrad_fused_acc: bw_in_acc needs y2 / dy_out / mean / rstd / gamma / dgamma / dbeta / n");
  SST_REQUIRE(!bw_st_acc || epi_y, "sst_conv_dgrad_fused_acc: bw_st_acc needs epi_y");
  SST_REQUIRE(!y2 || dy_out, "sst_conv_dgrad_fused_acc: y2 needs dy_out");
  BandAcc ba{};
  ba.nrep = nrep;
  ba.bw_st_acc = bw_st_acc; ba.bw_in_acc = bw_in_acc; ba.bw_mean = mean; ba.bw_rstd = rstd; ba.bw_gamma = gamma; ba.bw_n = n;
  ba.o_dgamma = dgamma; ba.o_dbeta = dbeta; ba.o_dslope = dslope;
  return conv_fwd_impl(g, wp, out, nullptr, nullptr, in_scale, in_shift, in_slope, in_slope_const, in_act, residual, nullptr, nullptr,
                       OUT_NHWC, B, H, W, Cin, Cout, ksize, 1, epi_y, epi_scale, epi_shift, epi_slope, epi_slope_const, epi_act, nullptr,
                       stream, y2, nullptr, nullptr, nullptr, y2 ? dy_out : nullptr, &ba);
}

SST_API int64_t sst_conv_s2_dgrad_packed_floats(int Cout, int Cin) { return s2_class_offset(4, Cin, Cout) + packed_floats_base(Cin, Cout, 9); }
int64_t sst_conv_s2_dgrad_pipe_section(int Cout, int Cin) { return s2_class_offset(4, Cin, Cout); }

SST_API int sst_conv_s2_dgrad_pack(const float* w, float* wp, int Cout, int Cin, void* stream) {
  SST_REQUIRE(w && wp && Cout > 0 && Cin > 0, "sst_conv_s2_dgrad_pack: bad argument");
  pack_s2_dgrad_kernel<<<dim3(256, 5), 256, 0, sst_stream(stream)>>>(w, wp, Cout, Cin);
  SST_LAUNCH_CHECK("pack_s2_dgrad_kernel");
  return SST_OK;
}

struct S2Fused {
  const float* in2; const float* cA; const float* cB; const float* cC; const float* in_scale; const float* in_shift;
  const float* in_slope; float in_slope_const; int in_act; float* dy_out;
  const float* epi_y; const float* epi_scale; const float* epi_shift; const float* epi_slope; float epi_slope_const; int epi_act;
  float* epi_partial;
};
SST_API int sst_conv_s2_dgrad_tiles(int B, int H, int W) {
  int t = 0;
  for (int cls = 0; cls < 4; ++cls) {
    const int nh = (H - (cls >> 1) + 1) / 2, nw = (W - (cls & 1) + 1) / 2;
    if (nh > 0 && nw > 0) t += sst_conv_mtiles(B, nh, nw);
  }
  return t;
}
namespace {
enum class S2Kind { MERGED4, MERGED, PER_CLASS };
struct S2Sel {
  S2Kind kind;
  S2Classes c;
  int max_tiles;
  const char* name;
};

Conv3Args s2_dgrad_args(const float* dy, const float* wp, float* dx, int B, int H, int W, int Cin, int Cout, int cls) {
  Conv3Args a{};
  const int py = cls < 0 ? 0 : cls >> 1, px = cls < 0 ? 0 : cls & 1;
  a.x = dy; a.wp = cls < 0 ? wp : wp + s2_class_offset(cls, Cin, Cout); a.y = dx;
  a.in_act = ACT_NONE; a.out_mode = OUT_STRIDE2;
  a.B = B; a.H = (H - 1) / 2 + 1; a.W = (W - 1) / 2 + 1; a.Cin = Cout; a.Cout = Cin;
  a.ksy = 1 + py; a.ksx = 1 + px; a.sub_y = py; a.sub_x = px;
  if (cls >= 0) { a.Ho = (H - py + 1) / 2; a.Wo = (W - px + 1) / 2; }
  a.Hy = H; a.Wy = W;
  return a;
}

S2Sel s2_dgrad_select(int B, int H, int W, int Cin, int Cout, bool fused) {
  S2Sel s{};
  bool ok = !sst_env("SST_S2_SPLIT") || fused;
  int tbase = 0;
  for (int cls = 0; cls < 4; ++cls) {
    const Conv3Args t = s2_dgrad_args(nullptr, nullptr, nullptr, B, H, W, Cin, Cout, cls);
    S2Classes& c = s.c;
    c.nh[cls] = t.Ho;
    c.nw[cls] = t.Wo;
    c.wp_off[cls] = s2_class_offset(cls, Cin, Cout);
    c.tiles[cls] = (t.Ho > 0 && t.Wo > 0) ? sst_conv_mtiles(B, t.Ho, t.Wo) : 0;
    c.tile_base[cls] = tbase;
    tbase += c.tiles[cls];
    if (!fused && (c.tiles[cls] == 0 || use_big_tiles(t, 3))) ok = false;
    if (cls == 0) s.name = use_big_tiles(t, 3) ? "conv_fwd2_kernel<1>" : "conv_fwd_kernel<3, 1>";
    s.max_tiles = c.tiles[cls] > s.max_tiles ? c.tiles[cls] : s.max_tiles;
  }
  const bool s2d4 = !(sst_env("SST_S2DGRAD4") && atoi(sst_env("SST_S2DGRAD4")) == 0);
  s.kind = S2Kind::PER_CLASS;
  if (ok && s2d4 && !(H & 1) && !(W & 1) && !(Cout & 3) && !(Cin & 3)) {
    s.kind = S2Kind::MERGED4;
    s.name = fused ? "conv_s2dgrad4_kernel<true>" : "conv_s2dgrad4_kernel<false>";
// ... 72 lines not shown
```

srgan-st_amd/csrc/conv_wgrad.hip:

```cpp
#include "conv_common.h"
#include <cstring>
#include <cstdlib>

namespace {

constexpr int SUB = 64;
constexpr int WLD = 64 + 4;

struct WgJob {
  const float* x; const float* dy; float* slab; float* dw;
  const float* in_scale; const float* in_shift; const float* in_slope;
  float in_slope_const; int in_act;
};

constexpr int WG_TAB_MAX = 40;
struct WgJobTab { WgJob j[WG_TAB_MAX]; };

struct WgradArgs {
  int grouped;
  int nchunk;
  const float* x;
  const float* dy;
  float* slab;
  const float* in_scale;
// ... 228 lines not shown
    }
  };
  auto stage_store = [&]() {
#pragma unroll
    for (int u = 0; u < XS; ++u) {
      const int p = (tid + u * CONV_NT) >> 4;
      if (p >= npx_x) break;
      f32x4 xv = rx[u];
      if (a.in_scale) {
#pragma unroll
        for (int j = 0; j < 4; ++j) xv[j] = fmaf(xv[j], sc4[j], sh4[j]);
      }
      if (a.in_act == ACT_SLOPE) {
#pragma unroll
        for (int j = 0; j < 4; ++j) xv[j] = xv[j] > 0.f ? xv[j] : xv[j] * slope;
      }
      if (!((rvalid >> u) & 1u)) xv = f32x4{0.f, 0.f, 0.f, 0.f};
      *reinterpret_cast<f32x4*>(&sX[p * WLD + c4]) = xv;
    }
#pragma unroll
    for (int u = 0; u < WB_DS; ++u) {
      const int p = (tid + u * CONV_NT) >> 4;
      if (p < npx_d) *reinterpret_cast<f32x4*>(&sD[p * WLD + c4]) = rd[u];
    }
  };

  f32x16 acc[9];
#pragma unroll
  for (int t = 0; t < 9; ++t)
#pragma unroll
    for (int r = 0; r < 16; ++r) acc[t][r] = 0.f;

  const int la = lh * WLD + wco + li, lb = lh * WLD + wci + li;
  int tofs[9];
#pragma unroll
  for (int t = 0; t < 9; ++t) tofs[t] = ((t / 3) * PW + (t % 3)) * WLD;
  const int halfw = W >> 1, npairs = R * halfw;

  if (band_begin < band_end) stage_load(band_begin);
  for (int band = band_begin; band < band_end; ++band) {
    __syncthreads();
    stage_store();
    __syncthreads();
    if (band + 1 < band_end && !(a.dbg & 1)) stage_load(band + 1);
    if (a.dbg & 2) continue;
    int pa = 0, pb = 0, x2 = 0;
    auto advance = [&]() {
      pa += 2 * WLD;
      pb += 2 * WLD;
      if (++x2 == halfw) { x2 = 0; pb += 2 * WLD; }
    };
    float av0 = sD[pa + la], av1;
    float bv0[9], bv1[9];
#pragma unroll
    for (int t = 0; t < 9; ++t) bv0[t] = sX[pb + tofs[t] + lb];
    for (int i = 0; i < npairs; i += 2) {
      advance();
      av1 = sD[pa + la];
#pragma unroll
      for (int t = 0; t < 9; ++t) bv1[t] = sX[pb + tofs[t] + lb];
#pragma unroll
      for (int t = 0; t < 9; ++t) acc[t] = __builtin_amdgcn_mfma_f32_32x32x2f32(av0, bv0[t], acc[t], 0, 0, 0);
      if (i + 2 < npairs) advance();
      av0 = sD[pa + la];
#pragma unroll
      for (int t = 0; t < 9; ++t) bv0[t] = sX[pb + tofs[t] + lb];
#pragma unroll
      for (int t = 0; t < 9; ++t) acc[t] = __builtin_amdgcn_mfma_f32_32x32x2f32(av1, bv1[t], acc[t], 0, 0, 0);
    }
  }

  if (a.dbg & 4) {
    if (acc[0][0] == 12345.f) a.slab[0] = 1.f;
    return;
  }
  const int ci = ci0 + wci + li;
#pragma unroll
  for (int t = 0; t < 9; ++t) {
    float* out = a.slab + ((size_t)chunk * 9 + t) * a.Cout * a.Cin;
#pragma unroll
    for (int r = 0; r < 16; ++r) {
      const int co = co0 + wco + (r & 3) + 8 * (r >> 2) + 4 * lh;
      out[(size_t)co * a.Cin + ci] = acc[t][r];
    }
  }
}

constexpr int C3_ROWS = 8;
__global__ __launch_bounds__(CONV_NT) void wgrad_k3c3_kernel(const float* __restrict__ x, const float* __restrict__ dy,
                                                             float* __restrict__ slab, int B, int H, int W, int Cout) {
  extern __shared__ __attribute__((aligned(16))) float xs[];
  __shared__ float red[3][64][28];
  const int bands = (H + C3_ROWS - 1) / C3_ROWS;
  const int b = blockIdx.x / bands, y0 = (blockIdx.x - b * bands) * C3_ROWS;
  const int rows = min(C3_ROWS, H - y0);
  const int RS = (W + 2) * 3 + 3;
  for (int i = threadIdx.x; i < (C3_ROWS + 2) * RS; i += CONV_NT) {
    const int r = i / RS, o = i - r * RS;
    const int px = o / 3 - 1, y = y0 - 1 + r;
    float v = 0.f;
    if (o < (W + 2) * 3 && (unsigned)px < (unsigned)W && (unsigned)y < (unsigned)H)
      v = x[(((size_t)b * H + y) * W + px) * 3 + (o - (px + 1) * 3)];
    xs[i] = v;
  }
  __syncthreads();
  const int co = threadIdx.x & 63, pl = threadIdx.x >> 6;
  for (int cob = blockIdx.y * 64; cob < Cout; cob += gridDim.y * 64) {
    float acc[27];
#pragma unroll
    for (int k = 0; k < 27; ++k) acc[k] = 0.f;
    if (cob + co < Cout) {
      constexpr int UNR = 8;
      const int npx = rows * W;
      const float* dyb = dy + ((size_t)b * H + y0) * W * Cout + cob + co;
      for (int p0 = pl; p0 < npx; p0 += UNR * (CONV_NT / 64)) {
        float g[UNR];
#pragma unroll
        for (int u = 0; u < UNR; ++u) {
          const int p = p0 + u * (CONV_NT / 64);
          g[u] = p < npx ? dyb[(size_t)p * Cout] : 0.f;
        }
#pragma unroll
        for (int u = 0; u < UNR; ++u) {
          const int p = min(p0 + u * (CONV_NT / 64), npx - 1);
          const int r = p / W, c = p - r * W;
          const float* w0 = xs + r * RS + c * 3;
#pragma unroll
          for (int ky = 0; ky < 3; ++ky)
#pragma unroll
            for (int q = 0; q < 9; ++q) acc[ky * 9 + q] = fmaf(g[u], w0[ky * RS + q], acc[ky * 9 + q]);
        }
      }
    }
    __syncthreads();
    if (pl > 0) {
#pragma unroll
      for (int k = 0; k < 27; ++k) red[pl - 1][co][k] = acc[k];
    }
    __syncthreads();
    if (pl == 0 && cob + co < Cout) {
      float* out = slab + (size_t)blockIdx.x * 9 * Cout * 3;
#pragma unroll
      for (int k = 0; k < 27; ++k) {
        const float t = ((acc[k] + red[0][co][k]) + red[1][co][k]) + red[2][co][k];
        const int ky = k / 9, kx = (k % 9) / 3, ci = k % 3;
        out[((size_t)(ky * 3 + kx) * Cout + cob + co) * 3 + ci] = t;
      }
    }
  }
}
constexpr int C3M_ROW = 104;
constexpr int C3M_WAVE = 3 * C3M_ROW + 96;
constexpr int C3M_TPW = 4;
__global__ __launch_bounds__(CONV_NT) void wgrad_k3c3_mfma_kernel(const float* __restrict__ x, const float* __restrict__ dy,
                                                                  float* __restrict__ slab, int B, int H, int W, int ntiles) {
  __shared__ float patch[4 * C3M_WAVE];
  __shared__ float scr[4 * 32 * 33];
  const int tid = threadIdx.x, wave = __builtin_amdgcn_readfirstlane(tid >> 6), lane = tid & 63;
  const int li = lane & 31, lh = lane >> 5;
  constexpr int Cout = 64;
  float* const ps = patch + wave * C3M_WAVE;
  const int tpr = W >> 5;
  const int ky = li / 9, kr = li - ky * 9;
  const float* const bl = ps + (li < 27 ? ky * C3M_ROW + kr + 3 * lh : 3 * C3M_ROW);
  f32x16 acc[2];
#pragma unroll
  for (int h = 0; h < 2; ++h)
#pragma unroll
    for (int r = 0; r < 16; ++r) acc[h][r] = 0.f;
  for (int i = lane; i < 96; i += 64) ps[3 * C3M_ROW + i] = 0.f;
  float av[2][16][2], xv[2][5];
  auto issue = [&](int it, float (&a_)[16][2], float (&x_)[5]) {
    const int t = (blockIdx.x * C3M_TPW + it) * 4 + wave;
    const bool live = it < C3M_TPW && t < ntiles;
    const int b = t / (H * tpr), rem = t - b * (H * tpr);
    const int y = rem / tpr, x0 = (rem - y * tpr) << 5;
    const float* dp = dy + (live ? (((size_t)b * H + y) * W + x0 + lh) * Cout + li : 0);
#pragma unroll
    for (int ks = 0; ks < 16; ++ks) {
      a_[ks][0] = live ? dp[(size_t)(2 * ks) * Cout] : 0.f;
      a_[ks][1] = live ? dp[(size_t)(2 * ks) * Cout + 32] : 0.f;
    }
#pragma unroll
    for (int u = 0; u < 5; ++u) {
      const int i = lane + 64 * u;
      const int r = i / 102, c = i - r * 102;
      const int iy = y - 1 + r, fx = (x0 - 1) * 3 + c;
      const bool ok = live && i < 306 && (unsigned)iy < (unsigned)H && (unsigned)fx < (unsigned)(W * 3);
      x_[u] = ok ? x[((size_t)b * H + iy) * W * 3 + fx] : 0.f;
    }
  };
  issue(0, av[0], xv[0]);
#pragma unroll
  for (int it = 0; it < C3M_TPW; ++it) {
#pragma unroll
    for (int u = 0; u < 5; ++u) {
      const int i = lane + 64 * u;
      if (i < 306) ps[(i / 102) * C3M_ROW + i % 102] = xv[it & 1][u];
    }
    if (it + 1 < C3M_TPW) issue(it + 1, av[(it + 1) & 1], xv[(it + 1) & 1]);
#pragma unroll
    for (int ks = 0; ks < 16; ++ks) {
      const float bv = bl[6 * ks];
      acc[0] = __builtin_amdgcn_mfma_f32_32x32x2f32(av[it & 1][ks][0], bv, acc[0], 0, 0, 0);
      acc[1] = __builtin_amdgcn_mfma_f32_32x32x2f32(av[it & 1][ks][1], bv, acc[1], 0, 0, 0);
    }
  }
  float* const out = slab + (size_t)blockIdx.x * 9 * Cout * 3;
#pragma unroll
  for (int h = 0; h < 2; ++h) {
    __syncthreads();
#pragma unroll
    for (int r = 0; r < 16; ++r) scr[(wave * 32 + (r & 3) + 8 * (r >> 2) + 4 * lh) * 33 + li] = acc[h][r];
    __syncthreads();
#pragma unroll
    for (int j = 0; j < 4; ++j) {
      const int row = 8 * wave + 4 * lh + j;
      const float v = ((scr[row * 33 + li] + scr[(32 + row) * 33 + li]) + scr[(64 + row) * 33 + li]) + scr[(96 + row) * 33 + li];
      if (li < 27) out[((size_t)(li / 3) * Cout + 32 * h + row) * 3 + li % 3] = v;
    }
  }
}
constexpr int C3R_OUT = 16, C3R_GRP = 1024 / C3R_OUT;
__global__ __launch_bounds__(1024) void c3m_reduce_kernel(const float* __restrict__ slab, float* __restrict__ dw, int nchunk,
                                                          int accumulate) {
  __shared__ float part[C3R_GRP][C3R_OUT + 1];
  constexpr int TOTAL = 9 * 64 * 3;
  const int o = threadIdx.x & (C3R_OUT - 1), gq = threadIdx.x / C3R_OUT;
  const int i = blockIdx.x * C3R_OUT + o;
  float t = 0.f;
  int c = gq;
  for (; c + 7 * C3R_GRP < nchunk; c += 8 * C3R_GRP) {
    float v[8];
#pragma unroll
    for (int u = 0; u < 8; ++u) v[u] = slab[(size_t)(c + C3R_GRP * u) * TOTAL + i];
#pragma unroll
    for (int u = 0; u < 8; ++u) t += v[u];
  }
  {
    float v[8];
#pragma unroll
    for (int u = 0; u < 8; ++u) v[u] = c + C3R_GRP * u < nchunk ? slab[(size_t)(c + C3R_GRP * u) * TOTAL + i] : 0.f;
#pragma unroll
    for (int u = 0; u < 8; ++u) t += v[u];
  }
  part[gq][o] = t;
  __syncthreads();
  if (threadIdx.x < 64) {
    const int oo = threadIdx.x & (C3R_OUT - 1), q = threadIdx.x / C3R_OUT;
    t = 0.f;
#pragma unroll
    for (int k = 0; k < C3R_GRP / 4; ++k) t += part[q * (C3R_GRP / 4) + k][oo];
    t += __shfl_xor(t, 16, 64);
    t += __shfl_xor(t, 32, 64);
    if (q == 0) {
      const int ii = blockIdx.x * C3R_OUT + oo;
      const int tap = ii / 192, oc = ii - tap * 192;
      float* d = dw + (size_t)oc * 9 + tap;
      *d = accumulate ? *d + t : t;
    }
  }
}
inline bool k3c3_mfma_applies(int W, int Cout) { return (W & 31) == 0 && Cout == 64 && !sst_env("SST_WGRAD_NO_K3C3_MFMA"); }
inline int k3c3_mfma_chunks(int B, int H, int W) { return (B * H * (W >> 5) + 4 * C3M_TPW - 1) / (4 * C3M_TPW); }

inline bool k3c3_applies(int Cin, int ksize, int stride, bool has_in_scale, int in_act) {
  return Cin == 3 && ksize == 3 && stride == 1 && !has_in_scale && in_act == ACT_NONE;
}

struct WgBandPlan { int R, bpc, nchunk, nbands; size_t lds; };
inline WgBandPlan wgrad_band_plan(int B, int H, int W, int Cin, int Cout, int ksize, int stride, int njobs) {
  WgBandPlan best{0, 0, 0, 0, 0};
  if (ksize != 3 || stride != 1 || (Cin & 63) || (Cout & 63) || (W & 3) || W < 4) return best;
  if (const char* e = sst_env("SST_WGRAD_BAND")) {
    if (atoi(e) == 0) return best;
  }
  if (2.0 * B * H * W * Cin * Cout * 9 * njobs < 2.5e9 && !sst_env("SST_WGRAD_BAND")) return best;
  const int nblk = (Cout >> 6) * (Cin >> 6);
  long slots = 512;
  int rmax = 2;
  if (const char* e = sst_env("SST_WGRAD_BAND_SLOTS")) slots = atoi(e);
  if (const char* e = sst_env("SST_WGRAD_BAND_R")) rmax = atoi(e);
  double best_cost = 1e30;
  for (int R = rmax; R >= 1; --R) {
    if (H % R) continue;
    const int npx_x = (R + 2) * (W + 2), npx_d = R * W;
    if ((npx_x * 16 + CONV_NT - 1) / CONV_NT > WB_XS || (npx_d * 16 + CONV_NT - 1) / CONV_NT > WB_DS) continue;
    const size_t lds = (size_t)(npx_x + npx_d) * WLD * sizeof(float);
    if (lds > 78 * 1024) continue;
    const long nbands = (long)B * (H / R);
    const long per = (long)nblk * njobs;
    long bpc = (nbands * per + slots - 1) / slots;
    if (bpc < 1) bpc = 1;
    const long nchunk = (nbands + bpc - 1) / bpc;
    const long rounds = (nchunk * per + slots - 1) / slots;
    const double cost = (double)rounds * ((double)bpc * R + 1.4);
    if (cost < best_cost) {
      best_cost = cost;
      best = WgBandPlan{R, (int)bpc, (int)nchunk, (int)nbands, lds};
    }
  }
  return best;
}

__global__ __launch_bounds__(256) void wgrad_reduce_kernel(const float* __restrict__ slab, float* __restrict__ dw, int nchunk,
                                                           int KK, int Cout, int Cin, int accumulate, int grouped, WgJobTab tab) {
  if (grouped) {
    slab = tab.j[blockIdx.y].slab;
    dw = tab.j[blockIdx.y].dw;
  }
  const int64_t per_tap = (int64_t)Cout * Cin, total = per_tap * KK;
  const bool split = accumulate & 2;
  accumulate &= 1;
  if (split) {
    __shared__ f32x4 part[4][64];
    const int item = threadIdx.x & 63, cg = threadIdx.x >> 6;
    const int64_t i4 = blockIdx.x * 64ll + item, total4 = total >> 2;
    f32x4 t = {0.f, 0.f, 0.f, 0.f};
    if (i4 < total4) {
#pragma unroll 4
      for (int s = cg; s < nchunk; s += 4) t += *reinterpret_cast<const f32x4*>(slab + (size_t)s * total + (i4 << 2));
    }
    part[cg][item] = t;
    __syncthreads();
    if (cg == 0 && i4 < total4) {
      t = part[0][item] + part[1][item];
      t += part[2][item];
      t += part[3][item];
      const int64_t i = i4 << 2;
      const int tap = (int)(i / per_tap);
      const int64_t oc = i - (int64_t)tap * per_tap;
#pragma unroll
      for (int j = 0; j < 4; ++j) {
        float* d = dw + (oc + j) * KK + tap;
        *d = accumulate ? *d + t[j] : t[j];
      }
    }
    return;
  }
  if ((Cin & 3) == 0) {
    const int64_t total4 = total >> 2;
    for (int64_t i4 = blockIdx.x * 256ll + threadIdx.x; i4 < total4; i4 += (int64_t)gridDim.x * 256) {
      const int64_t i = i4 << 2;
      const int tap = (int)(i / per_tap);
      const int64_t oc = i - (int64_t)tap * per_tap;
      f32x4 t = {0.f, 0.f, 0.f, 0.f};
#pragma unroll 4
      for (int s = 0; s < nchunk; ++s) t += *reinterpret_cast<const f32x4*>(slab + (size_t)s * total + i);
#pragma unroll
      for (int j = 0; j < 4; ++j) {
        float* d = dw + (oc + j) * KK + tap;
        *d = accumulate ? *d + t[j] : t[j];
      }
// ... 217 lines not shown
#pragma unroll
    for (int u = 0; u < DQ; ++u) *reinterpret_cast<f32x4*>(ds + ((lane >> 3) + 8 * u) * 32 + q4) = dr[u];
  };

  int t = t0 + wave;
  if (t < t1 && !(a.dbg & 2)) issue_any(t);
  const float* const dl = ds + lh * 32 + li;
  const float* const xl = xs + S * lh * 32 + li;
  for (; t < t1; t += S2_NW) {
    if (!(a.dbg & 1)) {
      if (edge) store(std::true_type{}); else store(std::false_type{});
    }
    if (t + S2_NW < t1 && !(a.dbg & 2)) issue_any(t + S2_NW);
    if (a.dbg & 4) continue;
    float av, bv[9];
    auto fetch = [&](int ks, float& a_, float (&b_)[9]) {
      const int py = (2 * ks) / TW, px = (2 * ks) % TW;
      a_ = dl[2 * ks * 32];
#pragma unroll
      for (int tap = 0; tap < 9; ++tap) b_[tap] = xl[((S * py + tap / 3) * PW + S * px + tap % 3) * 32];
    };
    fetch(0, av, bv);
    __builtin_amdgcn_sched_barrier(0);
#pragma unroll
    for (int ks = 0; ks < NPIX / 2; ++ks) {
      float an = 0.f, bn[9] = {0.f, 0.f, 0.f, 0.f, 0.f, 0.f, 0.f, 0.f, 0.f};
      if (ks + 1 < NPIX / 2) fetch(ks + 1, an, bn);
      __builtin_amdgcn_sched_barrier(0);
#pragma unroll
      for (int tap = 0; tap < 9; ++tap) acc[tap] = __builtin_amdgcn_mfma_f32_32x32x2f32(av, bv[tap], acc[tap], 0, 0, 0);
      __builtin_amdgcn_sched_barrier(0);
      av = an;
#pragma unroll
      for (int tap = 0; tap < 9; ++tap) bv[tap] = bn[tap];
    }
  }

  if (a.dbg & 8) {
    if (acc[0][0] == 12345.f) a.slab[0] = 1.f;
    return;
  }
  float* const scr = wlds;
  float* const out = a.slab + (size_t)blockIdx.x * 9 * a.Cout * a.Cin;
  __syncthreads();
#pragma unroll
  for (int tap = 0; tap < 9; ++tap) {
    float* const sb = scr + (tap & 1) * (S2_NW * 32 * 33);
#pragma unroll
    for (int r = 0; r < 16; ++r) {
      const int row = (r & 3) + 8 * (r >> 2) + 4 * lh;
      sb[(wave * 32 + row) * 33 + li] = acc[tap][r];
    }
    __syncthreads();
    constexpr int RPW = 32 / S2_NW;
#pragma unroll
    for (int j = 0; j < RPW / 2; ++j) {
      const int row = RPW * wave + (RPW / 2) * lh + j;
      float v = sb[row * 33 + li];
#pragma unroll
      for (int w = 1; w < S2_NW; ++w) v += sb[(w * 32 + row) * 33 + li];
      if (a.dw) {
        float* d = a.dw + ((size_t)(co0 + row) * a.Cin + ci0 + li) * 9 + tap;
        *d = a.accumulate ? *d + v : v;
      } else {
        out[((size_t)tap * a.Cout + co0 + row) * a.Cin + ci0 + li] = v;
      }
    }
  }
}

struct WgS2Plan { int th, tw, nw, nchunk, tpc, ntiles; };
inline WgS2Plan wgrad_s2_plan(int B, int H, int W, int Cin, int Cout, int ksize, int stride) {
  WgS2Plan pl{0, 0, 0, 0, 0, 0};
  if (ksize != 3 || (stride != 1 && stride != 2) || (Cin & 31) || (Cout & 31) || B <= 0) return pl;
  if (stride == 2 && ((H | W) & 1)) return pl;
  bool force = false;
  if (const char* e = sst_env(stride == 2 ? "SST_WGRAD_S2" : "SST_WGRAD_S1T")) {
    if (atoi(e) == 0) return pl;
    force = true;
  }
  const int Ho = H / stride, Wo = W / stride;
  constexpr int NW = 8;
  int th = 0, tw = 0;
  if (stride == 2) {
    if (Wo % 8 == 0 && Ho % 2 == 0) { th = 2; tw = 8; }
    else if (Wo % 6 == 0 && Ho % 2 == 0) { th = 2; tw = 6; }
  } else {
    if (2.0 * B * H * W * Cin * Cout * 9 < 2.5e9 && !force) return pl;
    if (Wo % 8 == 0 && Ho % 4 == 0) { th = 4; tw = 8; }
    else if (Wo % 6 == 0 && Ho % 4 == 0) { th = 4; tw = 6; }
  }
  if (!th || (int64_t)B * H * W * Cin >= (1ll << 31)) return pl;
  const int ntiles = B * (Ho / th) * (Wo / tw);
  const int nblk = (Cout >> 5) * (Cin >> 5);
  int nchunk = 256 / nblk;
  if (nchunk < 1) nchunk = 1;
  int tpc = ((ntiles + nchunk - 1) / nchunk + NW - 1) / NW * NW;
  if (tpc < NW) tpc = NW;
  nchunk = (ntiles + tpc - 1) / tpc;
  pl = WgS2Plan{th, tw, NW, nchunk, tpc, ntiles};
  return pl;
}

template <int S, int TH, int TW, int S2_NW>
static int launch_wgrad_s2_t(const WgS2Args& a, const WgS2Plan& pl, hipStream_t st) {
  using G = WgS2Geom<S, TH, TW, S2_NW>;
  static bool lds_ok = false;
  if (!lds_ok) {
    if (hipFuncSetAttribute(reinterpret_cast<const void*>(&conv_wgrad_tile_kernel<S, TH, TW, S2_NW>),
                            hipFuncAttributeMaxDynamicSharedMemorySize, (int)G::LDS_BYTES) != hipSuccess)
      return sst_set_error(SST_ERR_HIP, "conv_wgrad_tile: cannot raise the LDS limit");
    lds_ok = true;
  }
  conv_wgrad_tile_kernel<S, TH, TW, S2_NW><<<dim3(pl.nchunk, (a.Cout >> 5) * (a.Cin >> 5)), S2_NW * 64, G::LDS_BYTES, st>>>(a);
  return SST_OK;
}

static long g_wgrad_band_launches = 0;
SST_API long sst_debug_wgrad_band_launches(void) { return g_wgrad_band_launches; }

static int launch_wgrad_band(WgradArgs& a, const WgBandPlan& pl, int njobs, hipStream_t st, const WgJobTab& tab) {
  ++g_wgrad_band_launches;
  static bool big_lds_enabled = false;
  if (!big_lds_enabled) {
    if (hipFuncSetAttribute(reinterpret_cast<const void*>(&conv_wgrad_band_kernel<7>), hipFuncAttributeMaxDynamicSharedMemorySize,
                            80 * 1024) != hipSuccess ||
        hipFuncSetAttribute(reinterpret_cast<const void*>(&conv_wgrad_band_kernel<WB_XS>),
                            hipFuncAttributeMaxDynamicSharedMemorySize, 80 * 1024) != hipSuccess)
      return sst_set_error(SST_ERR_HIP, "conv_wgrad_band: cannot raise the LDS limit");
    big_lds_enabled = true;
  }
  a.R = pl.R; a.bpc = pl.bpc; a.nbands = pl.nbands; a.nchunk = pl.nchunk;
  dim3 grid((unsigned)pl.nchunk * njobs, (a.Cout >> 6) * (a.Cin >> 6));
  const int xslots = ((pl.R + 2) * (a.W + 2) * 16 + CONV_NT - 1) / CONV_NT;
  if (xslots <= 7)
    conv_wgrad_band_kernel<7><<<grid, CONV_NT, pl.lds, st>>>(a, tab);
  else
    conv_wgrad_band_kernel<WB_XS><<<grid, CONV_NT, pl.lds, st>>>(a, tab);
  SST_LAUNCH_CHECK("conv_wgrad_band_kernel");
  return SST_OK;
}

namespace {
enum class WgKind { TILE, BAND, K3C3_MFMA, K3C3, GENERAL_VEC, GENERAL_SCALAR };
struct WgradPlan {
  WgKind kind;
  int nchunk;
  int pending;
  int slab_chunks;
  int chunk_px;
  WgS2Plan tile;
  WgBandPlan band;
  const char* name;
};

WgradPlan wgrad_plan(int B, int H, int W, int Cin, int Cout, int ksize, int stride, int njobs, bool has_in_scale, int in_act,
                     bool grouped) {
  WgradPlan p{};
  if (!grouped) p.tile = wgrad_s2_plan(B, H, W, Cin, Cout, ksize, stride);
  if (p.tile.th) {
    static const char* const names[2][2] = {{"conv_wgrad_tile_kernel<1, 4, 8, 8>", "conv_wgrad_tile_kernel<1, 4, 6, 8>"},
                                            {"conv_wgrad_tile_kernel<2, 2, 8, 8>", "conv_wgrad_tile_kernel<2, 2, 6, 8>"}};
    const bool direct = p.tile.nchunk == 1 && !sst_env("SST_WGRAD_TILE_NO_DIRECT");
    p.kind = WgKind::TILE;
    p.nchunk = p.slab_chunks = p.tile.nchunk;
    p.pending = direct ? 0 : p.nchunk;
    p.name = names[stride == 2][p.tile.tw == 6];
    return p;
  }
  p.band = wgrad_band_plan(B, H, W, Cin, Cout, ksize, stride, njobs);
  if (p.band.R) {
    p.kind = WgKind::BAND;
    p.nchunk = p.slab_chunks = p.band.nchunk;
    p.pending = grouped ? 0 : p.nchunk;
    p.name = ((p.band.R + 2) * (W + 2) * 16 + CONV_NT - 1) / CONV_NT <= 7 ? "conv_wgrad_band_kernel<7>" : "conv_wgrad_band_kernel<10>";
    return p;
  }
  const int pad = ksize / 2, Ho = (H + 2 * pad - ksize) / stride + 1, Wo = (W + 2 * pad - ksize) / stride + 1;
  const int64_t M = (int64_t)B * Ho * Wo;
  int nchunk = sst_conv_wgrad_chunks(B, Ho, Wo, Cin, Cout, ksize);
  p.slab_chunks = nchunk;
  if (Cin == 3 && ksize == 3 && stride == 1) {
    const int rows = B * ((H + C3_ROWS - 1) / C3_ROWS);
    const bool mfma = k3c3_mfma_applies(W, Cout);
    if (rows > p.slab_chunks) p.slab_chunks = rows;
    if (mfma && k3c3_mfma_chunks(B, H, W) > p.slab_chunks) p.slab_chunks = k3c3_mfma_chunks(B, H, W);
    if (!grouped && k3c3_applies(Cin, ksize, stride, has_in_scale, in_act)) {
      if (mfma) {
        p.kind = WgKind::K3C3_MFMA;
        p.nchunk = k3c3_mfma_chunks(B, H, W);
        p.name = "wgrad_k3c3_mfma_kernel";
        return p;
      }
      if (!sst_env("SST_WGRAD_NO_K3C3")) {
        p.kind = WgKind::K3C3;
        p.nchunk = p.pending = rows;
        p.name = "wgrad_k3c3_kernel";
        return p;
      }
    }
  }
  if (grouped) {
    int target = 2048;
    if (const char* e = sst_env("SST_WGRAD_GROUP_WGS")) target = atoi(e);
    const int nblk = ((Cout + 63) / 64) * ((Cin + 63) / 64);
    int want = (target + ksize * ksize * nblk * njobs - 1) / (ksize * ksize * nblk * njobs);
    if (want < 1) want = 1;
    if (target > 0 && want < nchunk) {
      const int64_t cpx = ((M + want - 1) / want + SUB - 1) / SUB * SUB;
      nchunk = (int)((M + cpx - 1) / cpx);
    }
  }
  const bool vec = (Cin & 3) == 0 && (Cout & 3) == 0;
  p.kind = vec ? WgKind::GENERAL_VEC : WgKind::GENERAL_SCALAR;
  p.nchunk = nchunk;
  p.pending = grouped ? 0 : nchunk;
  p.chunk_px = (int)(((M + nchunk - 1) / nchunk + SUB - 1) / SUB * SUB);
  p.name = vec ? "conv_wgrad_kernel<true>" : "conv_wgrad_kernel<false>";
  return p;
}

void wgrad_shape_args(WgradArgs& a, const WgradPlan& pl, int B, int H, int W, int Cin, int Cout, int ksize, int stride) {
  a.B = B; a.H = H; a.W = W; a.Cin = Cin; a.Cout = Cout; a.stride = stride; a.KS = ksize; a.pad = ksize / 2;
  a.Ho = (H + 2 * a.pad - ksize) / stride + 1;
  a.Wo = (W + 2 * a.pad - ksize) / stride + 1;
  a.chunk_px = pl.chunk_px;
}
}

SST_API int sst_conv_wgrad_chunks2(int B, int H, int W, int Cin, int Cout, int ksize, int stride, int njobs) {
  return wgrad_plan(B, H, W, Cin, Cout, ksize, stride, njobs, false, ACT_NONE, njobs > 1).slab_chunks;
}

SST_API const char* sst_conv_wgrad_kernel_name(int B, int H, int W, int Cin, int Cout, int ksize, int stride, int njobs) {
  return wgrad_plan(B, H, W, Cin, Cout, ksize, stride, njobs, false, ACT_NONE, njobs > 1).name;
}

SST_API int sst_conv_wgrad_groups_ok(int B, int H, int W, int Cin, int Cout, int ksize, int stride, int grp_images) {
  return grp_images > 0 && B > 0 && B % grp_images == 0 &&
         wgrad_plan(B, H, W, Cin, Cout, ksize, stride, 1, true, ACT_NONE, false).kind == WgKind::TILE;
}

SST_API int sst_conv_wgrad_pending_reduce(int B, int H, int W, int Cin, int Cout, int ksize, int stride, int has_in_scale, int in_act) {
  return wgrad_plan(B, H, W, Cin, Cout, ksize, stride, 1, has_in_scale != 0, in_act, false).pending;
}

SST_API int sst_conv_wgrad_grp(const float* x, const float* dy, float* slab, float* dw, const float* in_scale,
                               const float* in_shift, const float* in_slope, float in_slope_const, int in_act, int B, int H,
                               int W, int Cin, int Cout, int stride, int ksize, int accumulate, int grp_images, void* stream) {
  SST_REQUIRE(x && dy && slab && dw, "sst_conv_wgrad: null pointer");
  SST_REQUIRE(B > 0 && H > 0 && W > 0 && Cin > 0 && Cout > 0 && (stride == 1 || stride == 2) && (ksize & 1) && ksize <= 9,
              "sst_conv_wgrad: bad shape");
  const WgradPlan pl = wgrad_plan(B, H, W, Cin, Cout, ksize, stride, 1, in_scale != nullptr, in_act, false);
  const bool grouped = grp_images > 0 && grp_images < B && in_scale;
  SST_REQUIRE(!grouped || (B % grp_images == 0 && pl.kind == WgKind::TILE),
              "sst_conv_wgrad: coefficient groups are only taken by the all-taps tile kernel (B=%d H=%d W=%d Cin=%d Cout=%d stride=%d)", B, H, W,
              Cin, Cout, stride);
  WgradArgs a;
  a.grouped = 0; a.nchunk = 0;
  static const WgJobTab no_tab{};
  a.x = x; a.dy = dy; a.slab = slab; a.in_scale = in_scale; a.in_shift = in_shift; a.in_slope = in_slope;
  a.in_slope_const = in_slope_const; a.in_act = in_act;
  wgrad_shape_args(a, pl, B, H, W, Cin, Cout, ksize, stride);
  SST_REQUIRE((int64_t)B * a.Ho * a.Wo < (1ll << 31), "sst_conv_wgrad: too many pixels");
  {
    const char* e = sst_env("SST_WGRAD_DBG");
    a.dbg = e ? atoi(e) : 0;
  }
  const int KK = ksize * ksize;
  const dim3 grid(pl.nchunk, KK, ((Cout + 63) / 64) * ((Cin + 63) / 64));
  hipStream_t st = sst_stream(stream);
  switch (pl.kind) {
    case WgKind::BAND: {
      const int rc = launch_wgrad_band(a, pl.band, 1, st, no_tab);
      if (rc != SST_OK) return rc;
      break;
    }
    case WgKind::TILE: {
      const WgS2Plan& p2 = pl.tile;
      WgS2Args s2;
      s2.x = x; s2.dy = dy; s2.slab = slab; s2.in_scale = in_scale; s2.in_shift = in_shift; s2.in_slope = in_slope;
      s2.in_slope_const = in_slope_const; s2.in_act = in_act;
      s2.B = B; s2.H = H; s2.W = W; s2.Cin = Cin; s2.Cout = Cout; s2.Ho = a.Ho; s2.Wo = a.Wo;
      s2.dbg = sst_env("SST_WGRAD_S2_DBG") ? atoi(sst_env("SST_WGRAD_S2_DBG")) : 0;
      s2.dw = pl.pending ? nullptr : dw;
      s2.accumulate = accumulate & 1;
      s2.gB = grouped ? grp_images : 0;
      s2.tiles_x = a.Wo / p2.tw; s2.tiles_img = (a.Ho / p2.th) * s2.tiles_x; s2.ntiles = p2.ntiles; s2.tpc = p2.tpc;
      int rc;
      if (stride == 2) rc = p2.tw == 8 ? launch_wgrad_s2_t<2, 2, 8, 8>(s2, p2, st) : launch_wgrad_s2_t<2, 2, 6, 8>(s2, p2, st);
      else rc = p2.tw == 8 ? launch_wgrad_s2_t<1, 4, 8, 8>(s2, p2, st) : launch_wgrad_s2_t<1, 4, 6, 8>(s2, p2, st);
      if (rc != SST_OK) return rc;
      break;
    }
    case WgKind::K3C3_MFMA:
      wgrad_k3c3_mfma_kernel<<<pl.nchunk, CONV_NT, 0, st>>>(x, dy, slab, B, H, W, B * H * (W >> 5));
      SST_LAUNCH_CHECK("wgrad_k3c3_mfma_kernel");
      c3m_reduce_kernel<<<9 * 64 * 3 / C3R_OUT, 1024, 0, st>>>(slab, dw, pl.nchunk, accumulate & 1);
      SST_LAUNCH_CHECK("c3m_reduce_kernel");
      return SST_OK;
    case WgKind::K3C3: {
      const size_t lds = (size_t)(C3_ROWS + 2) * ((W + 2) * 3 + 3) * sizeof(float);
      SST_REQUIRE(lds <= 48 * 1024, "sst_conv_wgrad: image too wide for the 3-channel-input kernel (W=%d)", W);
      wgrad_k3c3_kernel<<<dim3(pl.nchunk, 1), CONV_NT, lds, st>>>(x, dy, slab, B, H, W, Cout);
      break;
    }
    case WgKind::GENERAL_VEC: conv_wgrad_kernel<true><<<grid, CONV_NT, 0, st>>>(a, no_tab); break;
    case WgKind::GENERAL_SCALAR: conv_wgrad_kernel<false><<<grid, CONV_NT, 0, st>>>(a, no_tab); break;
  }
  SST_LAUNCH_CHECK(pl.name);
  if (pl.pending == 0 || (accumulate & 4)) return SST_OK;
  launch_wgrad_reduce(slab, dw, pl.nchunk, KK, Cout, Cin, accumulate, nullptr, 1, st);
  SST_LAUNCH_CHECK("wgrad_reduce_kernel");
  return SST_OK;
}

SST_API int sst_conv_wgrad(const float* x, const float* dy, float* slab, float* dw, const float* in_scale,
                           const float* in_shift, const float* in_slope, float in_slope_const, int in_act, int B, int H,
                           int W, int Cin, int Cout, int stride, int ksize, int accumulate, void* stream) {
  return sst_conv_wgrad_grp(x, dy, slab, dw, in_scale, in_shift, in_slope, in_slope_const, in_act, B, H, W, Cin, Cout, stride, ksize,
                            accumulate, 0, stream);
}

SST_API int sst_wgrad_reduce_multi(const void* jobs, int njobs, void* stream) {
  static_assert(sizeof(WrJob) == 40, "WrJob layout");
  SST_REQUIRE(jobs && njobs > 0 && njobs <= WR_TAB_MAX, "sst_wgrad_reduce_multi: 1..%d jobs", WR_TAB_MAX);
  WrJobTab tab{};
  memcpy(tab.j, jobs, (size_t)njobs * sizeof(WrJob));
  int maxb = 0;
  for (int i = 0; i < njobs; ++i) {
    WrJob& j = tab.j[i];
    SST_REQUIRE(j.slab && j.dw && j.nchunk > 0 && j.KK > 0 && j.Cout > 0 && j.Cin > 0, "sst_wgrad_reduce_multi: bad job %d", i);
    const int64_t total = (int64_t)j.KK * j.Cout * j.Cin;
    if ((j.Cin & 3) == 0 && j.nchunk >= 8) {
      j.blocks = (int)((total / 4 + 63) / 64);
    } else {
      const int64_t items = (j.Cin & 3) == 0 ? total / 4 : total;
      j.blocks = (int)((items + 255) / 256 < 1024 ? (items + 255) / 256 : 1024);
    }
    if (j.blocks > maxb) maxb = j.blocks;
  }
  wgrad_reduce_multi_kernel<<<dim3(maxb, njobs), 256, 0, sst_stream(stream)>>>(tab);
  SST_LAUNCH_CHECK("wgrad_reduce_multi_kernel");
  return SST_OK;
}

SST_API int sst_conv_wgrad_grouped(const void* jobs, int njobs, int B, int H, int W, int Cin, int Cout, int stride, int ksize,
                                   int accumulate, void* stream) {
  static_assert(sizeof(WgJob) == 64, "WgJob layout");
  SST_REQUIRE(jobs && njobs > 0 && njobs <= WG_TAB_MAX && B > 0 && H > 0 && W > 0 && Cin > 0 && Cout > 0 && (stride == 1 || stride == 2) &&
                  (ksize & 1) && ksize <= 9, "sst_conv_wgrad_grouped: bad argument (at most %d jobs per call)", WG_TAB_MAX);
  WgJobTab tab{};
  memcpy(tab.j, jobs, (size_t)njobs * sizeof(WgJob));
  const WgradPlan pl = wgrad_plan(B, H, W, Cin, Cout, ksize, stride, njobs, true, ACT_NONE, true);
  WgradArgs a;
  a.grouped = 1;
  a.x = a.dy = nullptr; a.slab = nullptr; a.in_scale = a.in_shift = a.in_slope = nullptr; a.in_slope_const = 0.f; a.in_act = 0;
  wgrad_shape_args(a, pl, B, H, W, Cin, Cout, ksize, stride);
  SST_REQUIRE((int64_t)B * a.Ho * a.Wo < (1ll << 31), "sst_conv_wgrad_grouped: too many pixels");
  a.nchunk = pl.nchunk;
  a.dbg = 0;
  const int KK = ksize * ksize;
  const dim3 grid((unsigned)pl.nchunk * njobs, KK, ((Cout + 63) / 64) * ((Cin + 63) / 64));
  hipStream_t st = sst_stream(stream);
  if (pl.kind == WgKind::BAND) {
    const int rc = launch_wgrad_band(a, pl.band, njobs, st, tab);
    if (rc != SST_OK) return rc;
  } else if (pl.kind == WgKind::GENERAL_VEC)
    conv_wgrad_kernel<true><<<grid, CONV_NT, 0, st>>>(a, tab);
  else
    conv_wgrad_kernel<false><<<grid, CONV_NT, 0, st>>>(a, tab);
  SST_LAUNCH_CHECK("conv_wgrad_kernel (grouped)");
  launch_wgrad_reduce(nullptr, nullptr, pl.nchunk, KK, Cout, Cin, accumulate, &tab, njobs, st);
  SST_LAUNCH_CHECK("wgrad_reduce_kernel (grouped)");
  return SST_OK;
}
```

srgan-st_amd/srganst/_abi.py:

```python
from __future__ import annotations

import ctypes
import os
from ctypes import c_char_p, c_float, c_int, c_int64, c_void_p, POINTER

_HERE = os.path.dirname(os.path.abspath(__file__))
LIB_PATH = os.environ.get("SST_LIB_PATH") or os.path.join(_HERE, "lib", "libsrganst.so")

P = c_void_p

SIGNATURES = {
    "sst_last_error": (c_char_p, []),
    "sst_version": (c_int, []),
    "sst_arch": (c_char_p, []),
    "sst_clear_error": (c_int, []),
    "sst_reload_env": (c_int, []),
    "sst_st_loss_workspace": (c_int, [c_int, c_int, c_int, POINTER(c_int64)]),
    "sst_st_loss_fwd": (c_int, [P, P, P, P, P, P, c_int, c_int, c_int, c_float, c_float, c_int, P]),
    "sst_st_loss_bwd": (c_int, [P, P, P, P, c_float, c_int, c_int, c_int, c_int, c_float, c_float, P]),
    "sst_st_pixel_loss_fwd": (c_int, [P, P, P, P, P, P, P, P, c_int, c_int, c_int, c_int, c_float, c_float, c_int, P]),
    "sst_st_pixel_loss_bwd": (c_int, [P, P, P, P, P, c_float, c_float, c_int, c_int, c_int, c_int, c_int, c_float, c_float, P]),
    "sst_st_maps_workspace": (c_int, [c_int, c_int, c_int, POINTER(c_int64)]),
    "sst_st_maps": (c_int, [P, P, P, P, P, P, P, P, c_int, c_int, c_int, c_float, c_float, c_int, P]),
    "sst_conv_packed_floats": (c_int64, [c_int, c_int, c_int]),
    "sst_conv_pack": (c_int, [P, P, c_int, c_int, c_int, c_int, P]),
    "sst_conv_pack_multi": (c_int, [P, c_int, c_int, P]),
    "sst_conv_kernel_name": (c_char_p, [c_int, c_int, c_int, c_int, c_int, c_int, c_int, c_int, c_int]),
    "sst_conv_wgrad_kernel_name": (c_char_p, [c_int, c_int, c_int, c_int, c_int, c_int, c_int, c_int]),
    "sst_debug_big_tile_launches": (ctypes.c_long, []),
    "sst_adam_flat": (c_int, [P, P, P, P, c_int64, P, P, c_int, ctypes.c_double, ctypes.c_double, ctypes.c_double,
                            ctypes.c_double, P]),
    "sst_debug_band_launches": (ctypes.c_long, []),
    "sst_debug_wgrad_band_launches": (ctypes.c_long, []),
    "sst_debug_mfma_peak": (c_int, [P, c_int, c_int, P]),
    "sst_debug_bf16x3": (c_int, [P, P, P, P, c_int, c_int, c_int, P]),
    "sst_debug_stamp": (c_int, [P, c_int, P]),
    "sst_conv_mtiles": (c_int, [c_int, c_int, c_int]),
    "sst_conv_stat_tiles": (c_int, [c_int, c_int, c_int, c_int, c_int, c_int, c_int]),
    "sst_conv_fwd": (c_int, [P, P, P, P, P, P, P, P, c_float, c_int, P, P, P, c_int,
                             c_int, c_int, c_int, c_int, c_int, c_int, c_int, P]),
    "sst_conv_pipe_supported": (c_int, [c_int, c_int, c_int, c_int, c_int, c_int, c_int]),
    "sst_conv_pipe_stat_tiles": (c_int, [c_int, c_int, c_int, c_int, c_int, c_int, c_int]),
    "sst_conv_pipe_ws_floats": (c_int64, [c_int, c_int, c_int, c_int, c_int, c_int, c_int]),
    "sst_conv_pipe_fwd": (c_int, [P, P, P, P, P, P, P, c_float, c_int, P, P, P, P, P, P, c_float, c_int, P, P,
                                  c_int, c_int, c_int, c_int, c_int, c_int, c_int, P]),
    "sst_conv_pipe_groups_ok": (c_int, [c_int, c_int, c_int, c_int, c_int, c_int, c_int, c_int]),
    "sst_conv_pipe_fwd_grp": (c_int, [P, P, P, P, P, P, P, c_float, c_int, P, P, P, P, P, P, c_float, c_int, P, P,
                                      c_int, c_int, c_int, c_int, c_int, c_int, c_int, c_int, P]),
    "sst_conv_ns_supported": (c_int, [c_int, c_int, c_int, c_int, c_int, c_int, c_int, c_int]),
    "sst_conv_ns_fwd": (c_int, [P, P, P, P, P, P, P, c_float, c_int, P, P, P, P, P, P, c_float, c_int, P,
                                c_int, c_int, c_int, c_int, c_int, c_int, c_int, c_int, c_int, P]),
    "sst_conv_s2_dgrad_pipe_supported": (c_int, [c_int, c_int, c_int, c_int, c_int]),
    "sst_conv_s2_dgrad_pipe_ws_floats": (c_int64, [c_int, c_int, c_int, c_int, c_int]),
    "sst_conv_s2_dgrad_pipe": (c_int, [P, P, P, P, c_int, c_int, c_int, c_int, c_int, P]),
    "sst_conv_s2_dgrad_pipe_stat_tiles": (c_int, [c_int, c_int, c_int, c_int, c_int]),
    "sst_conv_s2_dgrad_pipe_bwdstats": (c_int, [P, P, P, P, P, P, P, P, c_float, c_int, P, c_int, c_int, c_int, c_int, c_int, P]),
    "sst_conv_s2_dgrad_pipe_groups_ok": (c_int, [c_int, c_int, c_int, c_int, c_int, c_int]),
    "sst_conv_s2_dgrad_pipe_bwdstats_grp": (c_int, [P, P, P, P, P, P, P, P, c_float, c_int, P, c_int, c_int, c_int, c_int, c_int, c_int, P]),
    "sst_conv_acc_supported": (c_int, [c_int, c_int, c_int, c_int, c_int, c_int, c_int]),
    "sst_conv_fwd_acc": (c_int, [P, P, P, P, P, P, P, P, c_float, c_int, P, P, P, c_float, c_float, c_float, P, P, P, P, P, P, P,
                                 c_int, c_int, c_int, c_int, c_int, c_int, c_int, P]),
    "sst_conv_dgrad_fused_acc": (c_int, [P, P, P, P, P, c_float, c_int, P, P, P, P, P, P, P, P, c_float, c_int, P, P, P, P, c_float, P, P, P,
                                         P, c_int, c_int, c_int, c_int, c_int, c_int, c_int, P]),
    "sst_bn_finalize_acc": (c_int, [P, c_int, c_int, c_float, P, P, P, P, P, P, P, P, c_float, c_float, P]),
    "sst_conv_fwd_resin": (c_int, [P, P, P, P, P, P, P, P, P, P, P, c_int, c_int, c_int, c_int, c_int, c_int, P]),
    "sst_conv_dgrad_bwdstats": (c_int, [P, P, P, P, P, P, P, P, c_float, c_int, P, c_int, c_int, c_int, c_int, c_int, c_int, P]),
    "sst_conv_dgrad_fused": (c_int, [P, P, P, P, P, P, P, P, c_float, c_int, P, P, P, P, P, P, P, P, c_float, c_int, P,
                                     c_int, c_int, c_int, c_int, c_int, c_int, P]),
    "sst_conv_wgrad_chunks": (c_int, [c_int, c_int, c_int, c_int, c_int, c_int]),
    "sst_conv_wgrad_chunks2": (c_int, [c_int, c_int, c_int, c_int, c_int, c_int, c_int, c_int]),
    "sst_conv_wgrad": (c_int, [P, P, P, P, P, P, P, c_float, c_int, c_int, c_int, c_int, c_int, c_int,
                               c_int, c_int, c_int, P]),
    "sst_conv_wgrad_groups_ok": (c_int, [c_int, c_int, c_int, c_int, c_int, c_int, c_int, c_int]),
    "sst_conv_wgrad_grp": (c_int, [P, P, P, P, P, P, P, c_float, c_int, c_int, c_int, c_int, c_int, c_int,
                                   c_int, c_int, c_int, c_int, P]),
    "sst_conv_wgrad_grouped": (c_int, [P, c_int, c_int, c_int, c_int, c_int, c_int, c_int, c_int, c_int, P]),
    "sst_conv_wgrad_pending_reduce": (c_int, [c_int, c_int, c_int, c_int, c_int, c_int, c_int, c_int, c_int]),
    "sst_wgrad_reduce_multi": (c_int, [P, c_int, P]),
    "sst_bn_finalize": (c_int, [P, P, c_int, c_int, P, P, P, P, P, P, P, P, c_float, c_float, P]),
    "sst_bn_finalize_grp": (c_int, [P, P, c_int, c_int, c_int, P, P, P, P, P, P, P, P, c_float, c_float, P]),
    "sst_bn_eval_affine": (c_int, [P, P, P, P, P, P, c_int, c_float, P]),
    "sst_bn_residual": (c_int, [P, P, P, P, P, P, c_int64, c_int, P]),
    "sst_bwd_reduce_blocks": (c_int, [c_int64, c_int]),
    "sst_bwd_reduce": (c_int, [P, P, P, P, P, P, c_float, c_int, P, c_int64, c_int, P]),
    "sst_bwd_finalize": (c_int, [P, c_int, c_int, c_float, P, P, P, P, P, P, P, P, P, c_int, P]),
    "sst_bwd_reduce_grp": (c_int, [P, P, P, P, P, P, c_float, c_int, P, c_int64, c_int, c_int, P]),
    "sst_bwd_finalize_grp": (c_int, [P, c_int, c_int, c_float, c_int, P, P, P, P, P, P, P, P, c_int, P]),
    "sst_bwd_apply_grp": (c_int, [P, P, P, P, P, P, c_float, c_int, P, P, P, P, c_int64, c_int, c_int, P]),
    "sst_bwd_finalize_wide": (c_int, [P, c_int, c_int, c_float, P, P, P, P, P, P, P, P, P, c_int, P, P, P]),
    "sst_act_bwd_partial_blocks": (c_int, [c_int64]),
    "sst_act_bwd_partial": (c_int, [P, P, P, P, c_float, P, P, c_int64, c_int, c_int, c_int, P]),
    "sst_bwd_apply": (c_int, [P, P, P, P, P, P, c_float, c_int, P, P, P, P, c_int64, c_int, c_int, c_int, P]),
    "sst_add": (c_int, [P, P, P, c_int64, P]),
    "sst_transpose": (c_int, [P, P, c_int, c_int, c_int, c_int, c_int, P]),
    "sst_transpose_affine": (c_int, [P, P, c_int, c_int, c_int, c_int, c_int, P, P, P]),
    "sst_maxpool_relu_fwd": (c_int, [P, P, c_int, c_int, c_int, c_int, P]),
    "sst_maxpool_relu_bwd": (c_int, [P, P, P, c_int, c_int, c_int, c_int, P]),
    "sst_clamp_bwd_blocks": (c_int, [c_int, c_int, c_int]),
    "sst_clamp_bwd": (c_int, [P, P, P, P, P, c_int, c_int, c_int, c_int, c_int, P]),
    "sst_pixel_loss_blocks": (c_int, [c_int64]),
    "sst_pixel_loss_fwd": (c_int, [P, P, P, P, P, c_int64, c_int, P]),
    "sst_pixel_loss_bwd": (c_int, [P, P, P, P, c_float, c_int, c_int64, c_int, P]),
    "sst_bce_logits": (c_int, [P, c_float, P, P, P, c_float, c_int, P]),
    "sst_bicubic": (c_int, [P, P, P, P, P, P, c_int64, c_int, c_int, c_int, c_int, c_int, c_int, c_int, P]),
    "sst_gather_batch": (c_int, [P, c_int64, P, c_int, c_int, c_int, P, P, P, P, P, P, P, c_int, c_int, c_int, c_int, P]),
    "sst_gather_crops": (c_int, [P, c_int64, P, c_int64, P, c_int, c_int, P, P, P, P, P, P, P, c_int, c_int, c_int, c_int, c_int, P]),
    "sst_image_metrics_workspace": (c_int, [c_int, c_int, c_int, POINTER(c_int64)]),
    "sst_image_metrics": (c_int, [P, P, c_int, c_int, c_int, P, P, P, P, P]),
    "sst_feat_loss_fwd": (c_int, [P, P, P, P, c_float, c_int, P, P, P, c_int64, c_int, P]),
    "sst_feat_loss_bwd": (c_int, [P, P, P, P, c_float, c_int, P, P, c_float, c_int, c_int64, c_int, P]),
    "sst_bb_blocks": (c_int, [c_int, c_int, c_int]),
    "sst_bb_feature_dim": (c_int, [c_int]),
    "sst_bb_patches": (c_int, [P, P, P, c_int, c_int, c_int, c_int, c_int, c_int, P, P]),
    "sst_bb_match": (c_int, [P, P, P, P, P, P, c_int, c_int, c_int, c_int, c_float, c_float, c_int, c_int, P, P]),
    "sst_bb_match_dist": (c_int, [P, P, P, P, P, P, c_int, c_int, c_int, c_int, c_float, c_float, c_int, c_int, P, c_int, P]),
    "sst_bbg_patches": (c_int, [c_int, c_int, c_int, c_int, c_int]),
    "sst_bbg_blocks": (c_int, [c_int, c_int]),
    "sst_bbg_unfold": (c_int, [P, P, P, c_int, c_int, c_int, c_int, c_int, c_int, c_int, c_int, P]),
    "sst_bbg_match": (c_int, [P, P, P, P, P, P, c_int, c_int, c_int, c_int, c_float, c_float, c_int, c_int, P]),
    "sst_bbg_fold": (c_int, [P, P, c_int, c_int, c_int, c_int, c_int, c_int, P]),
    "sst_weighted_sum": (c_int, [POINTER(c_void_p), POINTER(c_float), c_int, P, P, P]),
    "sst_wgrad_c3_supported": (c_int, [c_int, c_int]),
    "sst_wgrad_c3_slab_floats": (c_int64, [c_int, c_int, c_int, c_int]),
    "sst_wgrad_c3": (c_int, [P, P, P, P, P, c_float, c_int, c_int, c_int, c_int, c_int, c_int, c_int, P]),
    "sst_conv9_c3_packed_floats": (c_int64, [c_int]),
    "sst_conv9_c3_pack": (c_int, [P, P, c_int, c_int, c_int, P]),
    "sst_conv9_c3_fwd": (c_int, [P, P, P, P, c_int, c_int, c_int, c_int, P]),
    "sst_conv9_to3_packed_floats": (c_int64, [c_int]),
    "sst_conv9_to3_pack": (c_int, [P, P, c_int, P]),
    "sst_conv9_to3_fwd": (c_int, [P, P, P, P, P, P, c_float, c_int, c_int, c_int, c_int, c_int, P]),
    "sst_conv_s2_dgrad_tiles": (c_int, [c_int, c_int, c_int]),
    "sst_conv_s2_dgrad_kernel_name": (c_char_p, [c_int, c_int, c_int, c_int, c_int, c_int]),
    "sst_conv_s2_dgrad_fused": (c_int, [P, P, P, P, P, P, P, P, c_float, c_int, P, P, P, P, P, P, P, c_float, c_int, P,
                                        c_int, c_int, c_int, c_int, c_int, P]),
    "sst_conv_s2_dgrad_packed_floats": (c_int64, [c_int, c_int]),
    "sst_conv_s2_dgrad_pack": (c_int, [P, P, c_int, c_int, P]),
    "sst_conv_s2_dgrad": (c_int, [P, P, P, c_int, c_int, c_int, c_int, c_int, P]),
    "sst_linear_ksplit": (c_int, [c_int, c_int, c_int]),
    "sst_linear_fwd": (c_int, [P, P, P, P, P, c_int, c_int, c_int, P]),
    "sst_linear_dgrad": (c_int, [P, P, P, c_int, c_int, c_int, c_int, c_int, P]),
    "sst_linear_wgrad": (c_int, [P, P, P, P, c_int, c_int, c_int, c_int, P]),
    "sst_head_fwd": (c_int, [P, P, P, P, c_int, c_int, c_int, c_float, P]),
    "sst_head_bwd": (c_int, [P, P, P, P, P, P, c_int, c_int, c_int, c_float, c_int, P]),
    "sst_flatten_act": (c_int, [P, P, P, c_float, c_int, P, c_int, c_int, c_int, P]),
    "sst_flatten_act_grp": (c_int, [P, P, P, c_float, c_int, P, c_int, c_int, c_int, c_int, P]),
}

_lib = None


class HipPathError(RuntimeError):
    pass


def lib() -> ctypes.CDLL:
    global _lib
    if _lib is None:
        if not os.path.exists(LIB_PATH):
            raise HipPathError(
                f"{LIB_PATH} is missing - build it with `python -c 'import __graft_entry__ as g; g.build()'` "
                "(make -C srgan-st_amd/csrc).  There is no CPU fallback for the HIP path.")
        import torch
        l = ctypes.CDLL(LIB_PATH)
        for name, (res, args) in SIGNATURES.items():
            fn = getattr(l, name)
            fn.restype = res
            fn.argtypes = args
        _lib = l
    return _lib


def reload_env() -> None:
    if _lib is not None:
        _lib.sst_reload_env()


def check(rc: int, what: str) -> None:
    if rc != 0:
        msg = lib().sst_last_error().decode(errors="replace")
        raise HipPathError(f"{what} failed (code {rc}): {msg}")


def ptr(t) -> int:
    if t is None:
        return None
    if not t.is_cuda:
        raise HipPathError("HIP path needs tensors on a ROCm device (no CPU fallback)")
    if not t.is_contiguous():
        raise HipPathError("HIP path needs contiguous tensors")
    return t.data_ptr()


def stream_ptr() -> int:
    import torch
    return torch.cuda.current_stream().cuda_stream
```

srgan-st_amd/srganst/disc_graph.py:

```python
from __future__ import annotations

import torch

from . import ops
from ._state import KeptPass, state
from .ops import ACT_SLOPE

LRELU = 0.2


def param_dict(module):
    names = [n for n, _ in module.named_parameters()]
    return names, dict(zip(names, [t.detach() for t in module.parameters()]))


PLAN = [(0, None, 1), (2, 3, 2), (5, 6, 1), (8, 9, 2), (11, 12, 1), (14, 15, 2), (17, 18, 1), (20, 21, 2)]


def _packs(module, p, with_dgrad, counter_add=0):
    hs = state(module)
    cache = hs.cache
    names = [f"features.{ci}.weight" for ci, _, s in PLAN]
    n1 = [f"features.{ci}.weight" for ci, _, s in PLAN if s == 1]
    n2 = [f"features.{ci}.weight" for ci, _, s in PLAN if s == 2]
# ... 59 lines not shown
               "stride": r["stride"]}
        if r["bi"] is not None:
            rec["mean"], rec["rstd"] = arena.t[("mean", li)], arena.t[("rstd", li)]
            scale, shift = arena.t[("scale", li)], arena.t[("shift", li)]
        else:
            scale = shift = None
        rec["scale"], rec["shift"] = scale, shift
        sv["layers"].append(rec)
        h, act = rec["y"], ACT_SLOPE
    return sv


def forward(module, x, p, training, need_grad=False, arena=None):
    groups, gB = 1, 0
    ar, slot = arena if arena is not None else (None, 0)
    if ar is not None:
        assert training and not isinstance(x, (list, tuple))
        Bx = x.shape[0]
        if ar.meta is None:
            ar.meta = {"B": Bx}
        assert ar.meta["B"] == Bx

    def A(key, shape, like):
        return ar.get(key, shape, like, slot, shape[0]) if ar is not None else None
    if isinstance(x, (list, tuple)):
        groups, gB = len(x), x[0].shape[0]
        if groups == 1:
            x, gB = x[0], 0
        elif not training:
            raise NotImplementedError("batched passes are a train-mode schedule (eval mode has no per-pass statistics to keep apart)")
    sv = {"layers": [], "groups": groups, "gB": gB}
    wp, sv["wd"], sv["ws2"] = _packs(module, p, need_grad)
    if training and not state(module).counters_external:
        ops.flatten_bn_counters(module).add_(groups)
    if groups > 1:
        _, c3, hh, ww = x[0].shape
        x3 = torch.empty(groups * gB, hh, ww, c3, device=x[0].device, dtype=torch.float32)
        for gi, xi in enumerate(x):
            assert xi.shape == x[0].shape
            ops.transpose(xi.contiguous(), to_nchw=False, out=x3[gi * gB:(gi + 1) * gB])
    else:
        Bq, c3, hh, ww = x.shape
        x3 = ops.transpose(x.contiguous(), to_nchw=False, out=A("x3", (Bq, hh, ww, c3), x))
    h, scale, shift, act = x3, None, None, 0
    for ci, bi, stride in PLAN:
        w = p[f"features.{ci}.weight"]
        cout = w.shape[0]
        bias = p.get(f"features.{ci}.bias")
        ho, wo = ops.conv_out_hw(h.shape[1], h.shape[2], 3, stride)
        y, _, st, cnt = ops.conv_fwd(h, wp[f"features.{ci}.weight"], cout, 3, stride, bias=bias, in_scale=scale, in_shift=shift,
                                     in_slope_const=LRELU, in_act=act, want_stats=(bi is not None and training), grp=gB,
                                     out=A(("y", len(sv["layers"])), (h.shape[0], ho, wo, cout), h))
        rec = {"x": h, "x_scale": scale, "x_shift": shift, "x_act": act, "y": y, "ci": ci, "bi": bi, "stride": stride}
        if bi is not None:
            bn = module.features[bi]
            g, b = p[f"features.{bi}.weight"], p[f"features.{bi}.bias"]
            if training:
                rows = None
                if ar is not None:
                    li_ = len(sv["layers"])
                    rows = tuple(ar.get((k, li_), (1, cout), h, slot, 0) for k in ("mean", "rstd", "scale", "shift"))
                mean, rstd, scale, shift = ops.bn_finalize(st, cnt, g, b, bn.running_mean, bn.running_var, groups=groups, out=rows)
                rec["mean"], rec["rstd"] = mean, rstd
                rec["st"], rec["cnt"] = st, cnt
            else:
                scale, shift = ops.bn_eval_affine(g, b, bn.running_mean, bn.running_var)
        else:
            scale = shift = None
        rec["scale"], rec["shift"] = scale, shift
        sv["layers"].append(rec)
        h, act = y, ACT_SLOPE
    nfeat = h.shape[1] * h.shape[2] * h.shape[3]
    flat = ops.flatten_act(h, scale, shift, LRELU, 1, grp=gB, out=A("flat", (h.shape[0], nfeat), h))
    h1 = ops.linear_fwd(flat, p["classifier.0.weight"], p["classifier.0.bias"],
                        out=A("h1", (h.shape[0], p["classifier.0.weight"].shape[0]), h))
    if ar is not None:
        ar.filled.add(slot)
    out = ops.head_fwd(h1, p["classifier.2.weight"], p["classifier.2.bias"], LRELU)
    sv["flat"], sv["h1"] = flat, h1
    return out, sv


def replay_running_stats(module, p, sv):
    groups = sv.get("groups", 1)
    if not state(module).counters_external:
        ops.flatten_bn_counters(module).add_(groups)
    for rec in sv["layers"]:
        if rec["bi"] is None:
            continue
        bn = module.features[rec["bi"]]
        ops.bn_finalize(rec["st"], rec["cnt"], p[f"features.{rec['bi']}.weight"], p[f"features.{rec['bi']}.bias"],
                        bn.running_mean, bn.running_var, groups=groups)


def _grad_views(module, p, need_param_grads):
    names = list(p.keys())
    hs = state(module)
    scope = hs.grad_accum if need_param_grads else None
    acc = scope is not None and scope.flat is not None
    if acc:
        plist = [p[n] for n in names]
        offs, _ = ops.flat_layout(plist)
        views = {n: scope.flat[o:o + t.numel()].view(t.shape) for n, t, o in zip(names, plist, offs)}
    else:
        views = ops.flat_grads(module, names, [p[n] for n in names]) if need_param_grads else {}
        if scope is not None:
            scope.flat = hs.flat_grads[-1]
    return views, acc


def backward_classifier(module, p, sv, dout, need_param_grads, st=None):
    views, acc = _grad_views(module, p, need_param_grads)
    grads = {}

    def G(name):
        t = views[name]
        grads[name] = t
        return t

    h1, flat = sv["h1"], sv["flat"]
    wg = need_param_grads
    dh1 = ops.head_bwd(h1, p["classifier.2.weight"], dout.contiguous(), LRELU,
                       dw=G("classifier.2.weight") if wg else None, db=G("classifier.2.bias") if wg else None, accumulate=acc)
    if wg:
        dw0, db0 = G("classifier.0.weight"), G("classifier.0.bias")
        with ops.SideStream(dh1, flat, dw0, db0):
            ops.linear_wgrad(dh1, flat, dw0, db0, accumulate=acc)
    last = sv["layers"][-1]
    B, H, W, C = last["y"].shape
    g = ops.linear_dgrad(dh1, p["classifier.0.weight"], nhwc=(C, H * W)).view(B, H, W, C)
    return {"views": views, "acc": acc, "grads": grads, "g": g}


def backward_features(module, p, sv, st, need_param_grads, need_dx, defer_wgrad=None, defer_below=None):
    views, acc, grads, g = st["views"], st["acc"], st["grads"], st["g"]

    def G(name):
        t = views[name]
        grads[name] = t
        return t

    wg = need_param_grads
    dx = None
    groups, gB = sv.get("groups", 1), sv.get("gB", 0)
    wd, ws2 = sv["wd"], sv["ws2"]
    part = None
    reduces = [] if ops.WGRAD_REDUCE_MULTI else None
    for li in reversed(range(len(sv["layers"]))):
        r = sv["layers"][li]
        y = r["y"]
        n = y.numel() // y.shape[-1] // groups
        ci, bi = r["ci"], r["bi"]
        w = p[f"features.{ci}.weight"]
        if bi is not None:
            gam = p[f"features.{bi}.weight"]
            dg = G(f"features.{bi}.weight") if wg else torch.empty_like(gam)
            db = G(f"features.{bi}.bias") if wg else torch.empty_like(gam)
            kw = dict(scale=r["scale"], shift=r["shift"], slope_const=LRELU, act=1, mean=r["mean"], rstd=r["rstd"], gamma=gam,
                      dgamma=dg, dbeta=db, accumulate=acc and wg, groups=groups)
            dy = ops.bwd_finalize_apply(part, g, y, n, **kw) if part is not None else ops.bwd_reduce_apply(g, y, n, **kw)
        elif wg:
            kw = dict(slope_const=LRELU, act=1, dbeta=G(f"features.{ci}.bias"), accumulate=acc, groups=groups)
            dy = ops.bwd_finalize_apply(part, g, y, n, **kw) if part is not None else ops.bwd_reduce_apply(g, y, n, **kw)
        else:
            dy = ops.bwd_apply(g, y, slope_const=LRELU, act=1, groups=groups)
        part = None
        if wg:
            dwc = G(f"features.{ci}.weight")

            def launch(r=r, dy=dy, dwc=dwc, red=None):
                ops.conv_wgrad(r["x"], dy, dwc, 3, r["stride"], in_scale=r["x_scale"], in_shift=r["x_shift"],
                               in_slope_const=LRELU, in_act=r["x_act"], accumulate=acc, grp=gB, defer_reduce=red)
            if defer_wgrad is not None and (defer_below is None or li < defer_below):
                ev = torch.cuda.Event()
                ev.record()
                defer_wgrad.append((ev, launch, (r["x"], dy, dwc, r["x_scale"], r["x_shift"])))
            else:
                with ops.SideStream(r["x"], dy, dwc):
                    launch(red=reduces)
        if li == 0 and not need_dx:
            break
        xin = r["x"]
        if r["stride"] == 1:
            if li > 0:
                prev = sv["layers"][li - 1]
                g, part = ops.conv_dgrad_bwdstats(dy, wd[f"features.{ci}.weight"], w.shape[1], 3, prev["y"],
                                                  epi_scale=prev["scale"], epi_shift=prev["shift"], epi_slope_const=LRELU,
                                                  epi_act=1, grp=gB)
            else:
                g = ops.conv_fwd(dy, wd[f"features.{ci}.weight"], w.shape[1], 3, 1)[0]
        else:
            prev = sv["layers"][li - 1] if li > 0 else None
            epi = None
            if prev is not None and (prev["bi"] is not None or wg):
                epi = dict(y=prev["y"], scale=prev["scale"], shift=prev["shift"], slope_const=LRELU, act=1)
            out = ops.conv_s2_dgrad(dy, ws2[f"features.{ci}.weight"], xin.shape[1], xin.shape[2], w.shape[1], epi=epi, grp=gB)
            g, part = out if epi is not None else (out, None)
        if li == 0:
            dx = ops.transpose(g, to_nchw=True)
    if reduces:
        with ops.SideStream(*[t for j in reduces for t in j[:2]]):
            ops.wgrad_reduce_flush(reduces)
    ops.join_side()
    if acc:
        grads = {}
    return grads, dx


def backward(module, p, sv, dout, need_param_grads, need_dx):
    st = backward_classifier(module, p, sv, dout, need_param_grads)
    return backward_features(module, p, sv, st, need_param_grads, need_dx)


class DiscriminatorFn(torch.autograd.Function):
    @staticmethod
    def forward(ctx, x, module, grad_mode, *params):
        names, p = param_dict(module)
        need_param = grad_mode and any(ctx.needs_input_grad[3:])
        need_dx = grad_mode and ctx.needs_input_grad[0]
        need_grad = need_param or need_dx
        if need_grad and not module.training:
            raise NotImplementedError("Discriminator backward in eval() mode is not on the reference's path (train.py:110)")
        hs = state(module)
        keep = hs.keep_pass and need_grad and module.training
        req = hs.arena_request if keep else None
        arena = (PassArena(req[0]), req[1]) if req is not None else None
        out, sv = forward(module, x, p, module.training, need_grad, arena=arena)
        if keep:
            hs.last_pass = KeptPass(x.data_ptr(), tuple(x.shape), out, sv, p, arena[0] if arena is not None else None)
        if need_grad:
            ctx.module, ctx.sv, ctx.p, ctx.names = module, sv, p, names
            ctx.need_param, ctx.need_dx = need_param, need_dx
        return out

    @staticmethod
    def backward(ctx, dout):
        grads, dx = backward(ctx.module, ctx.p, ctx.sv, dout, ctx.need_param, ctx.need_dx)
        ctx.sv = None
        return (dx, None, None, *[grads.get(n) for n in ctx.names])
```

srgan-st_amd/srganst/ops.py:

```python
from __future__ import annotations

import os

import torch

from . import _abi
from ._abi import check, ptr, stream_ptr
from ._state import state

OUT_NHWC, OUT_SHUFFLE, OUT_NCHW_CLAMP, OUT_UNSHUFFLE = 0, 1, 2, 3
ACT_NONE, ACT_SLOPE = 0, 1
BN_EPS, BN_MOMENTUM = 1e-5, 0.1


PROFILE = None


TRACE = None


def _trace(name, flops, fn, *keep):
    if TRACE is not None:
        TRACE.setdefault(name, []).append((fn, flops, keep))


TRACE_HBM = None


def _trace_hbm(name, nbytes, fn, *keep):
    if TRACE_HBM is not None:
        TRACE_HBM.setdefault(name, []).append((fn, float(nbytes), keep))


def _prof_begin():
    if PROFILE is None:
        return None
    e = torch.cuda.Event(enable_timing=True)
    e.record()
    return e


def _prof_end(e0, name, flops):
    if e0 is not None:
        e1 = torch.cuda.Event(enable_timing=True)
        e1.record()
        PROFILE.append((name, flops, e0, e1))


def _launch(fn, args, what, flops, name_fn, keep):
    e0 = _prof_begin()
    check(fn(*args, stream_ptr()), what)
    name = name_fn() if (PROFILE is not None or TRACE is not None) else ""
    _prof_end(e0, name, flops)
    _trace(name, flops, lambda: fn(*args, stream_ptr()), *keep)


def _conv_name(B, H, W, cin, cout, ksize, stride, out_mode=0, fused_in=0):
    return _abi.lib().sst_conv_kernel_name(B, H, W, cin, cout, ksize, stride, int(out_mode) & 0xff, int(fused_in)).decode()


def _wgrad_name(B, H, W, cin, cout, ksize, stride, njobs):
    return _abi.lib().sst_conv_wgrad_kernel_name(B, H, W, cin, cout, ksize, stride, njobs).decode()


def _f32(*shape, like):
    return torch.empty(*shape, device=like.device, dtype=torch.float32)


def pack_conv(w: torch.Tensor, mode: int = 0, out: torch.Tensor | None = None) -> torch.Tensor:
    cout, cin, k, _ = w.shape
    o, i = (cin, cout) if mode else (cout, cin)
    n = _abi.lib().sst_conv_packed_floats(o, i, k)
    if out is None:
        out = _f32(n, like=w)
    assert out.numel() == n
    check(_abi.lib().sst_conv_pack(ptr(w), ptr(out), cout, cin, k, mode, stream_ptr()), "sst_conv_pack")
    return out


def conv_out_hw(h, w, k, stride):
    p = k // 2
    return (h + 2 * p - k) // stride + 1, (w + 2 * p - k) // stride + 1


def conv_fwd(x, wp, cout, ksize=3, stride=1, bias=None, in_scale=None, in_shift=None, in_slope=None,
             in_slope_const=0.0, in_act=ACT_NONE, residual=None, want_stats=False, out_mode=OUT_NHWC,
             want_pre=False, grp=0, out=None):
    B, H, W, cin = x.shape
    if grp and grp < B and in_scale is not None and not (out_mode == OUT_NHWC and residual is None and not want_pre
                                                         and conv_pipe_groups_ok(B, H, W, cin, cout, ksize, stride, grp)):
        raise _abi.HipPathError(f"conv_fwd: coefficient groups of {grp} images are not supported for this shape")
    ho, wo = conv_out_hw(H, W, ksize, stride)
    if out is not None:
        assert out_mode == OUT_NHWC and tuple(out.shape) == (B, ho, wo, cout) and out.is_contiguous()
        y = out
    elif out_mode == OUT_NHWC:
        y = _f32(B, ho, wo, cout, like=x)
    elif out_mode == OUT_SHUFFLE:
        y = _f32(B, 2 * ho, 2 * wo, cout // 4, like=x)
    elif out_mode == OUT_NCHW_CLAMP:
        y = _f32(B, cout, ho, wo, like=x)
    else:
        y = _f32(B, ho // 2, wo // 2, cout * 4, like=x)
    if out_mode == OUT_NHWC and residual is None and not want_pre and conv_pipe_tw(B, H, W, cin, cout, ksize, stride):
        y, stats, cnt, _ = _conv_pipe(x, wp, y, cout, ksize, stride, bias, in_scale, in_shift, in_slope, in_slope_const, in_act,
                                      want_stats, grp=grp)
        return y, None, stats, cnt
    if (out_mode == OUT_SHUFFLE and residual is None and not want_pre and not want_stats and CONV_NS
            and _abi.lib().sst_conv_ns_supported(B, H, W, cin, cout, ksize, stride, OUT_SHUFFLE)):
        y, _, _, _ = _conv_pipe(x, wp, y, cout, ksize, stride, bias, in_scale, in_shift, in_slope, in_slope_const, in_act, False,
                                out_mode=OUT_SHUFFLE)
        return y, None, None, None
    y_pre = torch.empty_like(y) if want_pre else None
    stats = cnt = None
    if want_stats:
        mt = _abi.lib().sst_conv_stat_tiles(B, H, W, cin, cout, ksize, stride)
        stats = _f32(mt, 2, cout, like=x)
        cnt = _f32(mt, like=x)
    args = (ptr(x), ptr(wp), ptr(y), ptr(y_pre), ptr(bias), ptr(in_scale), ptr(in_shift), ptr(in_slope), float(in_slope_const),
            int(in_act), ptr(residual), ptr(stats), ptr(cnt), int(out_mode), B, H, W, cin, cout, ksize, stride)
    _launch(_abi.lib().sst_conv_fwd, args, "sst_conv_fwd", 2.0 * B * ho * wo * cout * cin * ksize * ksize,
            lambda: _conv_name(B, H, W, cin, cout, ksize, stride, out_mode),
            (x, wp, y, y_pre, bias, in_scale, in_shift, in_slope, residual, stats, cnt))
    return y, y_pre, stats, cnt


def conv_pipe_tw(B, H, W, cin, cout, ksize, stride):
    if os.environ.get("SST_CONV_PIPE", "1") == "0":
        return 0
    return _abi.lib().sst_conv_pipe_supported(B, H, W, cin, cout, ksize, stride)


def conv_pipe_groups_ok(B, H, W, cin, cout, ksize, stride, grp):
    return bool(conv_pipe_tw(B, H, W, cin, cout, ksize, stride)) and \
        bool(_abi.lib().sst_conv_pipe_groups_ok(B, H, W, cin, cout, ksize, stride, int(grp)))


CONV_NS = os.environ.get("SST_CONV_NS", "1") != "0"


def _conv_pipe(x, wp, y, cout, ksize, stride, bias=None, in_scale=None, in_shift=None, in_slope=None, in_slope_const=0.0,
               in_act=ACT_NONE, want_stats=False, epi=None, grp=0, out_mode=OUT_NHWC):
    B, H, W, cin = x.shape
    L = _abi.lib()
    shp = (B, H, W, cin, cout, ksize, stride)
    stats = cnt = partial = None
    if want_stats:
        mt = L.sst_conv_pipe_stat_tiles(*shp)
        stats, cnt = _f32(mt, 2, cout, like=x), _f32(mt, like=x)
    e = epi or {}
    if epi is not None:
        partial = _f32(L.sst_conv_pipe_stat_tiles(*shp), 3, cout, like=x)
    ho, wo = conv_out_hw(H, W, ksize, stride)
    flops = 2.0 * B * ho * wo * cout * cin * ksize * ksize
    if CONV_NS and L.sst_conv_ns_supported(*shp, int(out_mode)):
        nargs = (ptr(x), ptr(wp), ptr(y), ptr(bias), ptr(in_scale), ptr(in_shift), ptr(in_slope), float(in_slope_const), int(in_act),
                 ptr(stats), ptr(cnt), ptr(e.get("y")), ptr(e.get("scale")), ptr(e.get("shift")), ptr(e.get("slope")),
                 float(e.get("slope_const", 0.0)), int(e.get("act", 0)), ptr(partial), *shp, int(out_mode), int(grp))
        _launch(L.sst_conv_ns_fwd, nargs, "sst_conv_ns_fwd", flops,
                lambda: f"conv_ns_kernel<{stride}, {L.sst_conv_ns_supported(*shp, int(out_mode))}>",
                (x, wp, y, bias, in_scale, in_shift, in_slope, stats, cnt, partial, *[v for v in e.values() if torch.is_tensor(v)]))
        return y, stats, cnt, partial
    assert out_mode == OUT_NHWC
    nws = L.sst_conv_pipe_ws_floats(*shp)
    ws = _f32(nws, like=x) if nws else None
    args = (ptr(x), ptr(wp), ptr(y), ptr(bias), ptr(in_scale), ptr(in_shift), ptr(in_slope), float(in_slope_const), int(in_act),
            ptr(stats), ptr(cnt), ptr(e.get("y")), ptr(e.get("scale")), ptr(e.get("shift")), ptr(e.get("slope")),
            float(e.get("slope_const", 0.0)), int(e.get("act", 0)), ptr(partial), ptr(ws), *shp, int(grp))
    _launch(L.sst_conv_pipe_fwd_grp, args, "sst_conv_pipe_fwd", flops, lambda: f"conv_pipe_kernel<{stride}, {L.sst_conv_pipe_supported(*shp)}, 0>",
            (x, wp, y, bias, in_scale, in_shift, in_slope, stats, cnt, partial, ws, *[v for v in e.values() if torch.is_tensor(v)]))
    return y, stats, cnt, partial


_ONES = {}


def _ones(x, cin):
    key = (x.device, cin)
    if key not in _ONES:
        _ONES[key] = torch.ones(cin, device=x.device, dtype=torch.float32)
    return _ONES[key]


def conv_fwd_resin(x, y2, bn_scale, bn_shift, wp, cout, ksize=3, bias=None, want_stats=False):
    B, H, W, cin = x.shape
    ones = _ones(x, cin)
    y = _f32(B, H, W, cout, like=x)
    h = torch.empty_like(x)
    stats = cnt = None
    if want_stats:
        mt = _abi.lib().sst_conv_stat_tiles(B, H, W, cin, cout, ksize, 1)
        stats = _f32(mt, 2, cout, like=x)
        cnt = _f32(mt, like=x)
    args = (ptr(x), ptr(y2), ptr(ones), ptr(bn_scale), ptr(bn_shift), ptr(h), ptr(wp), ptr(y), ptr(bias), ptr(stats), ptr(cnt),
            B, H, W, cin, cout, ksize)
    _launch(_abi.lib().sst_conv_fwd_resin, args, "sst_conv_fwd_resin", 2.0 * B * H * W * cout * cin * ksize * ksize,
            lambda: _conv_name(B, H, W, cin, cout, ksize, 1, 0, 1), (x, y2, ones, bn_scale, bn_shift, h, wp, y, bias, stats, cnt))
    return y, h, stats, cnt


ACC_NREP = int(os.environ.get("SST_ACC_NREP", "16"))


def conv_acc_supported(B, H, W, cin, cout, ksize=3, stride=1):
    return bool(_abi.lib().sst_conv_acc_supported(B, H, W, cin, cout, ksize, stride)) and os.environ.get("SST_ATOMIC_STATS", "1") != "0"


def conv_fwd_acc(x, wp, cout, ksize=3, in2=None, bias=None, in_slope=None, in_slope_const=0.0, in_act=ACT_NONE, in_acc=None,
                 in_bn=None, n=0.0, out_stats=None, run_stats=None, st_acc=None):
    B, H, W, cin = x.shape
    y = _f32(B, H, W, cout, like=x)
    h = torch.empty_like(x) if in2 is not None else None
    ones = _ones(x, cin) if in2 is not None else None
    g, bta = in_bn if in_bn is not None else (None, None)
    om, orr, osc, osh = out_stats if out_stats is not None else (None, None, None, None)
    rm, rv = run_stats if run_stats is not None else (None, None)
    args = (ptr(x), ptr(in2), ptr(h), ptr(ones), ptr(wp), ptr(y), ptr(bias), ptr(in_slope), float(in_slope_const), int(in_act),
            _dptr(in_acc), ptr(g), ptr(bta), float(n), float(BN_EPS), float(BN_MOMENTUM), ptr(om), ptr(orr), ptr(osc), ptr(osh),
            ptr(rm), ptr(rv), _dptr(st_acc), ACC_NREP, B, H, W, cin, cout, ksize)
    _launch(_abi.lib().sst_conv_fwd_acc, args, "sst_conv_fwd_acc", 2.0 * B * H * W * cout * cin * ksize * ksize,
            lambda: _conv_name(B, H, W, cin, cout, ksize, 1, 0, 1),
            (x, in2, h, ones, wp, y, bias, in_slope, in_acc, g, bta, om, orr, osc, osh, rm, rv, st_acc))
    return y, h


def conv_dgrad_fused_acc(g, wd, cout, ksize=3, y2=None, in_scale=None, in_shift=None, in_slope=None, in_slope_const=0.0, in_act=0,
                         residual=None, epi_y=None, epi_scale=None, epi_shift=None, epi_slope=None, epi_slope_const=0.0, epi_act=0,
                         bw_in_acc=None, bn=None, n=0.0, dgamma=None, dbeta=None, dslope=None, bw_st_acc=None):
    B, H, W, cin = g.shape
    out = _f32(B, H, W, cout, like=g)
    dy = torch.empty_like(g) if y2 is not None else None
    mean, rstd, gamma = bn if bn is not None else (None, None, None)
    args = (ptr(g), ptr(y2), ptr(in_scale), ptr(in_shift), ptr(in_slope), float(in_slope_const), int(in_act), ptr(dy), ptr(wd), ptr(out),
            ptr(residual), ptr(epi_y), ptr(epi_scale), ptr(epi_shift), ptr(epi_slope), float(epi_slope_const), int(epi_act),
            _dptr(bw_in_acc), ptr(mean), ptr(rstd), ptr(gamma), float(n), ptr(dgamma), ptr(dbeta), ptr(dslope), _dptr(bw_st_acc),
            ACC_NREP, B, H, W, cin, cout, ksize)
    _launch(_abi.lib().sst_conv_dgrad_fused_acc, args, "sst_conv_dgrad_fused_acc", 2.0 * B * H * W * cout * cin * ksize * ksize,
            lambda: _conv_name(B, H, W, cin, cout, ksize, 1, 0, 1),
            (g, y2, in_scale, in_shift, in_slope, dy, wd, out, residual, epi_y, epi_scale, epi_shift, epi_slope, bw_in_acc, mean, rstd, gamma,
             dgamma, dbeta, dslope, bw_st_acc))
    return out, dy


def _dptr(t):
    if t is None:
        return None
    assert t.is_cuda and t.is_contiguous() and t.dtype == torch.float64
    return t.data_ptr()


def bn_finalize_acc(acc, n, gamma, beta, run_mean=None, run_var=None):
    C = gamma.numel()
    mean, rstd, scale, shift = (_f32(C, like=gamma) for _ in range(4))
    check(_abi.lib().sst_bn_finalize_acc(_dptr(acc), acc.shape[0], C, float(n), ptr(gamma), ptr(beta), ptr(run_mean), ptr(run_var),
                                         ptr(mean), ptr(rstd), ptr(scale), ptr(shift), float(BN_EPS), float(BN_MOMENTUM), stream_ptr()),
          "sst_bn_finalize_acc")
    return mean, rstd, scale, shift


def conv_wgrad(x, dy, dw_out, ksize=3, stride=1, in_scale=None, in_shift=None, in_slope=None, in_slope_const=0.0,
               in_act=ACT_NONE, accumulate=False, grp=0, defer_reduce=None):
    B, H, W, cin = x.shape
    cout = dy.shape[-1]
    ho, wo = conv_out_hw(H, W, ksize, stride)
    assert tuple(dy.shape) == (B, ho, wo, cout) and tuple(dw_out.shape) == (cout, cin, ksize, ksize)
    nch = _abi.lib().sst_conv_wgrad_chunks2(B, H, W, cin, cout, ksize, stride, 1)
    slab = _f32(nch * ksize * ksize * cout * cin, like=x)
    pend = 0
    if defer_reduce is not None and PROFILE is None and TRACE is None:
        pend = _abi.lib().sst_conv_wgrad_pending_reduce(B, H, W, cin, cout, ksize, stride, int(in_scale is not None), int(in_act))
        if pend:
            assert dw_out.is_contiguous()
            defer_reduce.append((slab, dw_out, pend, ksize * ksize, cout, cin, int(bool(accumulate))))
    args = (ptr(x), ptr(dy), ptr(slab), ptr(dw_out), ptr(in_scale), ptr(in_shift), ptr(in_slope), float(in_slope_const),
            int(in_act), B, H, W, cin, cout, stride, ksize, int(bool(accumulate)) | (4 if pend else 0), int(grp))

    def name():
        n = _wgrad_name(B, H, W, cin, cout, ksize, stride, 1)
        return n + ("+c3m_reduce_kernel" if n == "wgrad_k3c3_mfma_kernel" else "+wgrad_reduce_kernel")
    _launch(_abi.lib().sst_conv_wgrad_grp, args, "sst_conv_wgrad", 2.0 * B * ho * wo * cout * cin * ksize * ksize, name,
            (x, dy, slab, dw_out, in_scale, in_shift, in_slope))
    return dw_out


WGRAD_REDUCE_MULTI = os.environ.get("SST_WGRAD_REDUCE_MULTI", "1") != "0"


def wgrad_reduce_flush(jobs):
    import ctypes
    import struct
    while jobs:
        js, jobs[:] = jobs[:24], jobs[24:]
        buf = b"".join(struct.pack("<QQiiiiii", slab.data_ptr(), dw.data_ptr(), nch, kk, cout, cin, acc, 0)
                       for slab, dw, nch, kk, cout, cin, acc in js)
        check(_abi.lib().sst_wgrad_reduce_multi(ctypes.c_char_p(buf), len(js), stream_ptr()), "sst_wgrad_reduce_multi")


def bn_finalize(stats, cnt, gamma, beta, run_mean=None, run_var=None, eps=BN_EPS, momentum=BN_MOMENTUM, groups=1, out=None):
    C = gamma.numel()
    shape = (C,) if groups == 1 else (groups, C)
    if out is not None:
        mean, rstd, scale, shift = out
        assert all(tuple(t.shape) == shape and t.is_contiguous() for t in out)
    else:
        mean, rstd, scale, shift = (_f32(*shape, like=gamma) for _ in range(4))
    check(_abi.lib().sst_bn_finalize_grp(ptr(stats), ptr(cnt), stats.shape[0], C, int(groups), ptr(gamma), ptr(beta), ptr(run_mean),
                                         ptr(run_var), ptr(mean), ptr(rstd), ptr(scale), ptr(shift), eps, momentum,
                                         stream_ptr()), "sst_bn_finalize")
    return mean, rstd, scale, shift


def bn_eval_affine(gamma, beta, run_mean, run_var, eps=BN_EPS):
    C = gamma.numel()
    scale, shift = _f32(C, like=gamma), _f32(C, like=gamma)
    check(_abi.lib().sst_bn_eval_affine(ptr(gamma), ptr(beta), ptr(run_mean), ptr(run_var), ptr(scale), ptr(shift), C, eps,
                                        stream_ptr()), "sst_bn_eval_affine")
    return scale, shift


def bn_residual(y, scale, shift, res, res_slope=None):
    C = y.shape[-1]
    out = torch.empty_like(y)
    check(_abi.lib().sst_bn_residual(ptr(y), ptr(scale), ptr(shift), ptr(res), ptr(res_slope), ptr(out), y.numel() // C, C,
                                     stream_ptr()), "sst_bn_residual")
    return out


def bwd_reduce(g, y, g2=None, scale=None, shift=None, slope=None, slope_const=0.0, act=0, groups=1):
    C = y.shape[-1]
    R = y.numel() // C // groups
    nblk = _abi.lib().sst_bwd_reduce_blocks(R, C)
    partial = _f32(groups * nblk, 3, C, like=y)
    check(_abi.lib().sst_bwd_reduce_grp(ptr(g), ptr(g2), ptr(y), ptr(scale), ptr(shift), ptr(slope), float(slope_const), int(act),
                                        ptr(partial), R, C, int(groups), stream_ptr()), "sst_bwd_reduce")
    return partial


def bwd_finalize(partial, n, mean=None, rstd=None, gamma=None, dgamma=None, dbeta=None, dslope=None, accumulate=False, groups=1):
    nblk, _, C = partial.shape
    cA = cB = cC = None
    if groups > 1:
        assert dslope is None and nblk % groups == 0
        if mean is not None:
            cA, cB, cC = (_f32(groups, C, like=partial) for _ in range(3))
        check(_abi.lib().sst_bwd_finalize_grp(ptr(partial), nblk // groups, C, float(n), int(groups), ptr(mean), ptr(rstd), ptr(gamma),
                                              ptr(dgamma), ptr(dbeta), ptr(cA), ptr(cB), ptr(cC), int(accumulate), stream_ptr()),
              "sst_bwd_finalize_grp")
        return cA, cB, cC
    if mean is not None:
        cA, cB, cC = (_f32(C, like=partial) for _ in range(3))
    if dslope is not None and C > 64:
        scratch = _f32((C + 63) // 64, like=partial)
        check(_abi.lib().sst_bwd_finalize_wide(ptr(partial), nblk, C, float(n), ptr(mean), ptr(rstd), ptr(gamma), ptr(dgamma),
                                               ptr(dbeta), ptr(cA), ptr(cB), ptr(cC), ptr(dslope), int(accumulate), ptr(scratch),
                                               _next_counter(partial.device), stream_ptr()), "sst_bwd_finalize_wide")
        return cA, cB, cC
    check(_abi.lib().sst_bwd_finalize(ptr(partial), nblk, C, float(n), ptr(mean), ptr(rstd), ptr(gamma), ptr(dgamma), ptr(dbeta),
                                      ptr(cA), ptr(cB), ptr(cC), ptr(dslope), int(accumulate), stream_ptr()),
          "sst_bwd_finalize")
    return cA, cB, cC


def act_bwd(g, y, g2=None, slope=None, slope_const=0.0, dbias=None, dslope=None, accumulate=False, unshuffle=False):
    C = y.shape[-1]
    R = y.numel() // C
    uh = uw = 0
    if unshuffle:
        B, uh, uw, _ = y.shape
        dy = _f32(B, uh // 2, uw // 2, 4 * C, like=y)
    else:
        dy = torch.empty_like(y)
    Cs = dy.shape[-1]
    nblk = _abi.lib().sst_act_bwd_partial_blocks(dy.numel() // Cs)
    partial = _f32(nblk, 3, Cs, like=y)
    check(_abi.lib().sst_act_bwd_partial(ptr(g), ptr(g2), ptr(y), ptr(slope), float(slope_const), ptr(dy), ptr(partial), R, C, uh, uw,
                                         stream_ptr()), "sst_act_bwd_partial")
    if dbias is not None or dslope is not None:
        bwd_finalize(partial, R, dbeta=dbias, dslope=dslope, accumulate=accumulate)
    return dy


def bwd_apply(g, y, g2=None, scale=None, shift=None, slope=None, slope_const=0.0, act=0, cA=None, cB=None, cC=None,
              unshuffle=False, groups=1):
    C = y.shape[-1]
    if groups > 1:
        assert not unshuffle
        dy = torch.empty_like(y)
        check(_abi.lib().sst_bwd_apply_grp(ptr(g), ptr(g2), ptr(y), ptr(scale), ptr(shift), ptr(slope), float(slope_const), int(act),
                                           ptr(cA), ptr(cB), ptr(cC), ptr(dy), y.numel() // C // groups, C, int(groups), stream_ptr()),
              "sst_bwd_apply_grp")
        return dy
    uh = uw = 0
    if unshuffle:
        B, uh, uw, _ = y.shape
        dy = _f32(B, uh // 2, uw // 2, 4 * C, like=y)
    else:
        dy = torch.empty_like(y)
    check(_abi.lib().sst_bwd_apply(ptr(g), ptr(g2), ptr(y), ptr(scale), ptr(shift), ptr(slope), float(slope_const), int(act),
                                   ptr(cA), ptr(cB), ptr(cC), ptr(dy), y.numel() // C, C, uh, uw, stream_ptr()),
          "sst_bwd_apply")
    return dy


def add(a, b):
    out = torch.empty_like(a)
    check(_abi.lib().sst_add(ptr(a), ptr(b), ptr(out), a.numel(), stream_ptr()), "sst_add")
    return out


def transpose(x, to_nchw: bool, out=None):
    if to_nchw:
        B, H, W, C = x.shape
        shape = (B, C, H, W)
    else:
        B, C, H, W = x.shape
        shape = (B, H, W, C)
    if out is None:
        out = _f32(*shape, like=x)
    assert tuple(out.shape) == shape and out.is_contiguous()
    check(_abi.lib().sst_transpose(ptr(x), ptr(out), B, C, H, W, int(to_nchw), stream_ptr()), "sst_transpose")
# ... 539 lines not shown
```

Baseline: 3261 HR images/s.

## Fuse leaky-ReLU backward into first discriminator layer's dgrad and wgrad kernels

For the discriminator's first conv layer (no BN, stride 1), the leaky-ReLU backward mask is now applied inside the conv dgrad (to3 kernel) and the k3c3 wgrad MFMA kernel, reading the activation output directly. This removes the separate elementwise pass that materialised dy. Bias grads still come from a reduce over g and y. It also adds a multi-row to3 dgrad variant (4 output rows per 64-thread block with rotating prefetch) to reuse input rows across output rows. The cost is extra loads of act_y inside both kernels and more register pressure.

```diff
diff --git a/include/srganst.h b/include/srganst.h
--- a/include/srganst.h
+++ b/include/srganst.h
@@ -120,6 +120,12 @@
                    const float* in_shift, const float* in_slope, float in_slope_const, int in_act,
                    int B, int H, int W, int Cin, int Cout, int stride, int ksize, int accumulate,
                        int grp_images, void* stream);
+int sst_conv_dgrad_dyact_supported(int B, int H, int W, int Cin, int Cout, int ksize);
+int sst_conv_dgrad_dyact(const float* g, const float* act_y, float act_slope, const float* wp, float* out, int B, int H, int W,
+                         int Cin, int Cout, int ksize, void* stream);
+int sst_conv_wgrad_dyact_supported(int B, int H, int W, int Cin, int Cout, int ksize, int stride);
+int sst_conv_wgrad_dyact(const float* x, const float* g, const float* act_y, float act_slope, float* slab, float* dw, int B, int H,
+                         int W, int Cin, int Cout, int stride, int ksize, int accumulate, void* stream);
 int sst_conv_wgrad_pending_reduce(int B, int H, int W, int Cin, int Cout, int ksize, int stride, int has_in_scale, int in_act);
 int sst_wgrad_reduce_multi(const void* jobs, int njobs, void* stream);
 int sst_wgrad_c3_supported(int C, int ksize);
diff --git a/srgan-st_amd/csrc/api.hip b/srgan-st_amd/csrc/api.hip
--- a/srgan-st_amd/csrc/api.hip
+++ b/srgan-st_amd/csrc/api.hip
@@ -33,6 +33,10 @@
   e.set = v != nullptr;
   snprintf(e.value, sizeof(e.value), "%s", v ? v : "");
   return e.set ? e.value : nullptr;
+}
+bool sst_l0_dyact_enabled() {
+  const char* e = sst_env("SST_L0_DYACT");
+  return !(e && atoi(e) == 0);
 }
 SST_API int sst_reload_env(void) {
   std::lock_guard<std::mutex> lk(g_env_mu);
diff --git a/srgan-st_amd/csrc/common.h b/srgan-st_amd/csrc/common.h
--- a/srgan-st_amd/csrc/common.h
+++ b/srgan-st_amd/csrc/common.h
@@ -27,6 +27,7 @@
   } while (0)
 
 const char* sst_env(const char* name);
+bool sst_l0_dyact_enabled();
 
 static inline hipStream_t sst_stream(void* s) { return reinterpret_cast<hipStream_t>(s); }
 
diff --git a/srgan-st_amd/csrc/conv_fwd.hip b/srgan-st_amd/csrc/conv_fwd.hip
--- a/srgan-st_amd/csrc/conv_fwd.hip
+++ b/srgan-st_amd/csrc/conv_fwd.hip
@@ -492,8 +492,10 @@
 }
 
 typedef float f32x4c __attribute__((ext_vector_type(4)));
-__global__ __launch_bounds__(CONV_NT) void conv3_to3_kernel(const float* __restrict__ x, const float* __restrict__ wp,
-                                                            float* __restrict__ y, int B, int H, int W, int nmt, int nsp) {
+template <bool ACT>
+__global__ __launch_bounds__(CONV_NT) void conv3_to3_kernel(const float* __restrict__ x, const float* __restrict__ act_y, float act_slope,
+                                                            const float* __restrict__ wp, float* __restrict__ y, int B, int H, int W,
+                                                            int nmt, int nsp) {
   extern __shared__ __attribute__((aligned(16))) float pl_all[];
   const int wave = __builtin_amdgcn_readfirstlane(threadIdx.x >> 6), lane = threadIdx.x & 63;
   const int seg = blockIdx.x * 4 + wave;
@@ -515,24 +517,44 @@
           bw[ty][q][t] = lm < 9 ? wp[(size_t)(tap * 8 + (co >> 3)) * 256 + (((co & 7) >> 2) * 32 + ci) * 4 + (co & 3)] : 0.f;
         }
   }
-  auto load_tile = [&](int mt, f32x4c (&a)[3][4]) {
+  constexpr int YT = ACT ? 3 : 1;
+  auto load_tile = [&](int mt, f32x4c (&a)[3][4], f32x4c (&ya)[YT][4]) {
     const int xp = xb + mt * 16 + lm - 1;
 #pragma unroll
     for (int ty = 0; ty < 3; ++ty) {
       const int iy = oy - 1 + ty;
       const bool ok = (unsigned)iy < (unsigned)H && (unsigned)xp < (unsigned)W;
-      const float* src = x + (((size_t)b * H + (ok ? iy : 0)) * W + (ok ? xp : 0)) * 64 + 4 * lg;
+      const size_t off = (((size_t)b * H + (ok ? iy : 0)) * W + (ok ? xp : 0)) * 64 + 4 * lg;
+      const float* src = x + off;
 #pragma unroll
       for (int q = 0; q < 4; ++q) {
         const f32x4c v = *reinterpret_cast<const f32x4c*>(src + 16 * q);
         a[ty][q] = ok ? v : f32x4c{0.f, 0.f, 0.f, 0.f};
       }
+      if constexpr (ACT) {
+#pragma unroll
+        for (int q = 0; q < 4; ++q) ya[ty][q] = *reinterpret_cast<const f32x4c*>(act_y + off + 16 * q);
+      }
     }
   };
-  f32x4c ac[3][4], an[3][4];
-  load_tile(0, ac);
+  auto take = [&](f32x4c (&c)[3][4], const f32x4c (&a)[3][4], const f32x4c (&ya)[YT][4]) {
+#pragma unroll
+    for (int ty = 0; ty < 3; ++ty)
+#pragma unroll
+      for (int q = 0; q < 4; ++q) {
+        if constexpr (ACT) {
+#pragma unroll
+          for (int t = 0; t < 4; ++t) c[ty][q][t] = ya[ty][q][t] > 0.f ? a[ty][q][t] : a[ty][q][t] * act_slope;
+        } else {
+          c[ty][q] = a[ty][q];
+        }
+      }
+  };
+  f32x4c ac[3][4], an[3][4], yn[YT][4];
+  load_tile(0, an, yn);
+  take(ac, an, yn);
   for (int mt = 0; mt < nmt; ++mt) {
-    if (mt + 1 < nmt) load_tile(mt + 1, an);
+    if (mt + 1 < nmt) load_tile(mt + 1, an, yn);
     f32x4c acc = {0.f, 0.f, 0.f, 0.f};
 #pragma unroll
     for (int ty = 0; ty < 3; ++ty)
@@ -544,15 +566,94 @@
 #pragma unroll
       for (int r = 0; r < 4; ++r) pl[(mt * 16 + 4 * lg + r) * 12 + lm] = acc[r];
     }
-#pragma unroll
-    for (int ty = 0; ty < 3; ++ty)
-#pragma unroll
-      for (int q = 0; q < 4; ++q) ac[ty][q] = an[ty][q];
+    take(ac, an, yn);
   }
   float* const out = y + (((size_t)b * H + oy) * W + xb) * 3;
   for (int i = lane; i < 3 * Ws; i += 64) {
     const int xo = i / 3, ci = i - xo * 3;
     out[i] = (pl[xo * 12 + ci] + pl[(xo + 1) * 12 + 3 + ci]) + pl[(xo + 2) * 12 + 6 + ci];
+  }
+}
+
+template <int R_, int D_> struct To3Rows { static constexpr int R = R_, D = D_; };
+template <class ROWS>
+__global__ __launch_bounds__(64) void conv3_to3_kernel(const float* __restrict__ x, const float* __restrict__ act_y, float act_slope,
+                                                       const float* __restrict__ wp, float* __restrict__ y, int B, int H, int W, int nmt,
+                                                       int nsp, int nrb) {
+  constexpr int R = ROWS::R, NJ = R + 2, D = ROWS::D;
+  static_assert(NJ % D == 0, "the prefetch buffers rotate with the input rows");
+  extern __shared__ __attribute__((aligned(16))) float pl[];
+  const int lane = threadIdx.x;
+  const int seg = blockIdx.x;
+  const int rowb = seg / nsp, Ws = W / nsp, xb = (seg - rowb * nsp) * Ws;
+  const int b = rowb / nrb, oy0 = (rowb - b * nrb) * R;
+  const int lm = lane & 15, lg = lane >> 4;
+  float bw[3][4][4];
+  {
+    const int tx = lm / 3, ci = lm - tx * 3;
+#pragma unroll
+    for (int ty = 0; ty < 3; ++ty)
+#pragma unroll
+      for (int q = 0; q < 4; ++q)
+#pragma unroll
+        for (int t = 0; t < 4; ++t) {
+          const int co = 16 * q + 4 * lg + t, tap = ty * 3 + tx;
+          bw[ty][q][t] = lm < 9 ? wp[(size_t)(tap * 8 + (co >> 3)) * 256 + (((co & 7) >> 2) * 32 + ci) * 4 + (co & 3)] : 0.f;
+        }
+  }
+  f32x4c gq[D][4], yq[D][4];
+  auto load_step = [&](int mt, int j, f32x4c (&a)[4], f32x4c (&ya)[4]) {
+    const int xp = xb + mt * 16 + lm - 1, iy = oy0 - 1 + j;
+    const bool ok = (unsigned)iy < (unsigned)H && (unsigned)xp < (unsigned)W;
+    const size_t off = (((size_t)b * H + (ok ? iy : 0)) * W + (ok ? xp : 0)) * 64 + 4 * lg;
+#pragma unroll
+    for (int q = 0; q < 4; ++q) {
+      const f32x4c v = *reinterpret_cast<const f32x4c*>(x + off + 16 * q);
+      a[q] = ok ? v : f32x4c{0.f, 0.f, 0.f, 0.f};
+    }
+#pragma unroll
+    for (int q = 0; q < 4; ++q) ya[q] = *reinterpret_cast<const f32x4c*>(act_y + off + 16 * q);
+  };
+#pragma unroll
+  for (int j = 0; j < D; ++j) load_step(0, j, gq[j], yq[j]);
+  f32x4c acc[3];
+  for (int mt = 0; mt < nmt; ++mt) {
+#pragma unroll
+    for (int j = 0; j < NJ; ++j) {
+      f32x4c c[4];
+#pragma unroll
+      for (int q = 0; q < 4; ++q)
+#pragma unroll
+        for (int t = 0; t < 4; ++t) c[q][t] = yq[j % D][q][t] > 0.f ? gq[j % D][q][t] : gq[j % D][q][t] * act_slope;
+      {
+        const int j2 = (j + D) % NJ, mt2 = mt + (j + D >= NJ ? 1 : 0);
+        if (mt2 < nmt) load_step(mt2, j2, gq[j % D], yq[j % D]);
+      }
+#pragma unroll
+      for (int ty = 0; ty < 3; ++ty) {
+        const int r = j - ty;
+        if (r < 0 || r >= R) continue;
+        f32x4c a_ = {0.f, 0.f, 0.f, 0.f};
+        if (ty > 0) a_ = acc[r % 3];
+#pragma unroll
+        for (int q = 0; q < 4; ++q)
+#pragma unroll
+          for (int t = 0; t < 4; ++t) a_ = __builtin_amdgcn_mfma_f32_16x16x4f32(c[q][t], bw[ty][q][t], a_, 0, 0, 0);
+        acc[r % 3] = a_;
+        if (ty == 2 && lm < 9) {
+#pragma unroll
+          for (int rr = 0; rr < 4; ++rr) pl[((r * nmt + mt) * 16 + 4 * lg + rr) * 12 + lm] = a_[rr];
+        }
+      }
+    }
+  }
+  for (int r = 0; r < R && oy0 + r < H; ++r) {
+    const float* const pr = pl + (size_t)r * nmt * 16 * 12;
+    float* const out = y + (((size_t)b * H + oy0 + r) * W + xb) * 3;
+    for (int i = lane; i < 3 * Ws; i += 64) {
+      const int xo = i / 3, ci = i - xo * 3;
+      out[i] = (pr[xo * 12 + ci] + pr[(xo + 1) * 12 + 3 + ci]) + pr[(xo + 2) * 12 + 6 + ci];
+    }
   }
 }
 
@@ -811,13 +912,18 @@
 }
 
 namespace {
+constexpr int TO3_ROWS = 4, TO3_DEPTH = 2;
 enum class FwdKind { TO3, C3IN_MFMA, C3IN, BAND, BIG_TILES, GENERAL };
 struct FwdSel {
   FwdKind kind;
   int nsp, nmt;
+  int rows;
+  int nsp_rows, nmt_rows;
+  size_t lds_rows;
   int wgs;
   int R;
   size_t lds;
+  bool dyact;
   const char* name;
 };
 
@@ -837,7 +943,13 @@
     s.nmt = (a.W / s.nsp + 2 + 15) / 16;
     s.lds = (size_t)4 * s.nmt * 16 * 12 * sizeof(float);
     if (s.lds <= 60 * 1024) {
-      s.kind = FwdKind::TO3; s.name = "conv3_to3_kernel";
+      s.kind = FwdKind::TO3; s.name = "conv3_to3_kernel"; s.dyact = true;
+      s.rows = 1;
+      s.nsp_rows = (a.W % 32 == 0 && a.W >= 96) ? 4 : s.nsp;
+      s.nmt_rows = (a.W / s.nsp_rows + 2 + 15) / 16;
+      s.lds_rows = (size_t)TO3_ROWS * s.nmt_rows * 16 * 12 * sizeof(float);
+      const char* e = sst_env("SST_TO3_ACT_ROWS");
+      if (!(e && atoi(e) == 0) && s.lds_rows <= 60 * 1024) s.rows = TO3_ROWS;
       return s;
     }
   }
@@ -876,7 +988,8 @@
                          int Cout, int ksize, int stride, const float* epi_y, const float* epi_scale, const float* epi_shift,
                          const float* epi_slope, float epi_slope_const, int epi_act, float* epi_partial, void* stream,
                          const float* in2 = nullptr, const float* in_cA = nullptr, const float* in_cB = nullptr,
-                         const float* in_cC = nullptr, float* side_out = nullptr, const BandAcc* band_acc = nullptr) {
+                         const float* in_cC = nullptr, float* side_out = nullptr, const BandAcc* band_acc = nullptr,
+                         const float* act_y = nullptr, float act_slope = 0.f) {
   SST_REQUIRE(x && wp && y, "sst_conv_fwd: null pointer");
   SST_REQUIRE(B > 0 && H > 0 && W > 0 && Cin > 0 && Cout > 0 && (stride == 1 || stride == 2) && (ksize == 3 || ksize == 9),
               "sst_conv_fwd: bad shape B=%d H=%d W=%d Cin=%d Cout=%d k=%d stride=%d", B, H, W, Cin, Cout, ksize, stride);
@@ -908,10 +1021,21 @@
   const size_t extra_lds = (size_t)(dbg_bits >> 4) * 1024;
   a.dbg = dbg_bits & 15;
   const FwdSel s = conv_fwd_select(a, ksize, stride, dbg_bits);
+  SST_REQUIRE(!act_y || s.dyact, "sst_conv_dgrad_dyact: the kernel of this shape does not take the fused form (B=%d H=%d W=%d Cin=%d Cout=%d)", B,
+              H, W, Cin, Cout);
   switch (s.kind) {
-    case FwdKind::TO3:
-      conv3_to3_kernel<<<(unsigned)((B * H * s.nsp + 3) / 4), CONV_NT, s.lds, st>>>(x, wp, y, B, H, W, s.nmt, s.nsp);
+    case FwdKind::TO3: {
+      const unsigned wgs = (unsigned)((B * H * s.nsp + 3) / 4);
+      if (act_y && s.rows > 1) {
+        const int nrb = (H + TO3_ROWS - 1) / TO3_ROWS;
+        conv3_to3_kernel<To3Rows<TO3_ROWS, TO3_DEPTH>><<<(unsigned)(B * nrb * s.nsp_rows), 64, s.lds_rows, st>>>(
+            x, act_y, act_slope, wp, y, B, H, W, s.nmt_rows, s.nsp_rows, nrb);
+      } else if (act_y)
+        conv3_to3_kernel<true><<<wgs, CONV_NT, s.lds, st>>>(x, act_y, act_slope, wp, y, B, H, W, s.nmt, s.nsp);
+      else
+        conv3_to3_kernel<false><<<wgs, CONV_NT, s.lds, st>>>(x, nullptr, 0.f, wp, y, B, H, W, s.nmt, s.nsp);
       break;
+    }
     case FwdKind::C3IN_MFMA:
       conv3_c3in_mfma_kernel<<<(unsigned)(s.wgs < 768 ? s.wgs : 768), CONV_NT, 0, st>>>(x, wp, bias, y, B, H, W, B * H * (W >> 5));
       break;
@@ -939,6 +1063,23 @@
   a.out_mode = out_mode;
   a.in2 = fused_in ? reinterpret_cast<const float*>(1) : nullptr;
   return conv_fwd_select(a, ksize, stride, 0).name;
+}
+
+SST_API int sst_conv_dgrad_dyact_supported(int B, int H, int W, int Cin, int Cout, int ksize) {
+  if (B <= 0 || H <= 0 || W <= 0 || Cin <= 0 || Cout <= 0 || (ksize != 3 && ksize != 9) || !sst_l0_dyact_enabled()) return 0;
+  Conv3Args a{};
+  conv_shape_args(a, B, H, W, Cin, Cout, ksize, 1);
+  a.out_mode = OUT_NHWC;
+  return conv_fwd_select(a, ksize, 1, 0).dyact ? 1 : 0;
+}
+
+SST_API int sst_conv_dgrad_dyact(const float* g, const float* act_y, float act_slope, const float* wp, float* out, int B, int H, int W,
+                                 int Cin, int Cout, int ksize, void* stream) {
+  SST_REQUIRE(g && act_y && wp && out, "sst_conv_dgrad_dyact: null pointer");
+  SST_REQUIRE(sst_conv_dgrad_dyact_supported(B, H, W, Cin, Cout, ksize), "sst_conv_dgrad_dyact: shape not taken (or SST_L0_DYACT=0)");
+  return conv_fwd_impl(g, wp, out, nullptr, nullptr, nullptr, nullptr, nullptr, 0.f, ACT_NONE, nullptr, nullptr, nullptr, OUT_NHWC, B, H, W,
+                       Cin, Cout, ksize, 1, nullptr, nullptr, nullptr, nullptr, 0.f, 0, nullptr, stream, nullptr, nullptr, nullptr, nullptr,
+                       nullptr, nullptr, act_y, act_slope);
 }
 
 SST_API int sst_conv_fwd(const float* x, const float* wp, float* y, float* y_pre, const float* bias, const float* in_scale,
diff --git a/srgan-st_amd/csrc/conv_wgrad.hip b/srgan-st_amd/csrc/conv_wgrad.hip
--- a/srgan-st_amd/csrc/conv_wgrad.hip
+++ b/srgan-st_amd/csrc/conv_wgrad.hip
@@ -404,7 +404,9 @@
 constexpr int C3M_ROW = 104;
 constexpr int C3M_WAVE = 3 * C3M_ROW + 96;
 constexpr int C3M_TPW = 4;
+template <bool ACT>
 __global__ __launch_bounds__(CONV_NT) void wgrad_k3c3_mfma_kernel(const float* __restrict__ x, const float* __restrict__ dy,
+                                                                  const float* __restrict__ act_y, float act_slope,
                                                                   float* __restrict__ slab, int B, int H, int W, int ntiles) {
   __shared__ float patch[4 * C3M_WAVE];
   __shared__ float scr[4 * 32 * 33];
@@ -421,17 +423,27 @@
 #pragma unroll
     for (int r = 0; r < 16; ++r) acc[h][r] = 0.f;
   for (int i = lane; i < 96; i += 64) ps[3 * C3M_ROW + i] = 0.f;
-  float av[2][16][2], xv[2][5];
-  auto issue = [&](int it, float (&a_)[16][2], float (&x_)[5]) {
+  constexpr int YK = ACT ? 16 : 1;
+  float av[2][16][2], yv[2][YK][2], xv[2][5];
+  auto issue = [&](int it, float (&a_)[16][2], float (&y_)[YK][2], float (&x_)[5]) {
     const int t = (blockIdx.x * C3M_TPW + it) * 4 + wave;
     const bool live = it < C3M_TPW && t < ntiles;
     const int b = t / (H * tpr), rem = t - b * (H * tpr);
     const int y = rem / tpr, x0 = (rem - y * tpr) << 5;
-    const float* dp = dy + (live ? (((size_t)b * H + y) * W + x0 + lh) * Cout + li : 0);
+    const size_t doff = live ? (((size_t)b * H + y) * W + x0 + lh) * Cout + li : 0;
+    const float* dp = dy + doff;
 #pragma unroll
     for (int ks = 0; ks < 16; ++ks) {
       a_[ks][0] = live ? dp[(size_t)(2 * ks) * Cout] : 0.f;
       a_[ks][1] = live ? dp[(size_t)(2 * ks) * Cout + 32] : 0.f;
+    }
+    if constexpr (ACT) {
+      const float* yp = act_y + doff;
+#pragma unroll
+      for (int ks = 0; ks < 16; ++ks) {
+        y_[ks][0] = live ? yp[(size_t)(2 * ks) * Cout] : 0.f;
+        y_[ks][1] = live ? yp[(size_t)(2 * ks) * Cout + 32] : 0.f;
+      }
     }
 #pragma unroll
     for (int u = 0; u < 5; ++u) {
@@ -442,7 +454,7 @@
       x_[u] = ok ? x[((size_t)b * H + iy) * W * 3 + fx] : 0.f;
     }
   };
-  issue(0, av[0], xv[0]);
+  issue(0, av[0], yv[0], xv[0]);
 #pragma unroll
   for (int it = 0; it < C3M_TPW; ++it) {
 #pragma unroll
@@ -450,7 +462,13 @@
       const int i = lane + 64 * u;
       if (i < 306) ps[(i / 102) * C3M_ROW + i % 102] = xv[it & 1][u];
     }
-    if (it + 1 < C3M_TPW) issue(it + 1, av[(it + 1) & 1], xv[(it + 1) & 1]);
+    if (it + 1 < C3M_TPW) issue(it + 1, av[(it + 1) & 1], yv[(it + 1) & 1], xv[(it + 1) & 1]);
+    if constexpr (ACT) {
+#pragma unroll
+      for (int ks = 0; ks < 16; ++ks)
+#pragma unroll
+        for (int h = 0; h < 2; ++h) av[it & 1][ks][h] = yv[it & 1][ks][h] > 0.f ? av[it & 1][ks][h] : av[it & 1][ks][h] * act_slope;
+    }
 #pragma unroll
     for (int ks = 0; ks < 16; ++ks) {
       const float bv = bl[6 * ks];
@@ -974,6 +992,7 @@
   WgS2Plan tile;
   WgBandPlan band;
   const char* name;
+  bool dyact;
 };
 
 WgradPlan wgrad_plan(int B, int H, int W, int Cin, int Cout, int ksize, int stride, int njobs, bool has_in_scale, int in_act,
@@ -1012,6 +1031,7 @@
         p.kind = WgKind::K3C3_MFMA;
         p.nchunk = k3c3_mfma_chunks(B, H, W);
         p.name = "wgrad_k3c3_mfma_kernel";
+        p.dyact = true;
         return p;
       }
       if (!sst_env("SST_WGRAD_NO_K3C3")) {
@@ -1067,14 +1087,16 @@
   return wgrad_plan(B, H, W, Cin, Cout, ksize, stride, 1, has_in_scale != 0, in_act, false).pending;
 }
 
-SST_API int sst_conv_wgrad_grp(const float* x, const float* dy, float* slab, float* dw, const float* in_scale,
-                               const float* in_shift, const float* in_slope, float in_slope_const, int in_act, int B, int H,
-                               int W, int Cin, int Cout, int stride, int ksize, int accumulate, int grp_images, void* stream) {
+static int conv_wgrad_impl(const float* x, const float* dy, float* slab, float* dw, const float* in_scale, const float* in_shift,
+                           const float* in_slope, float in_slope_const, int in_act, int B, int H, int W, int Cin, int Cout, int stride,
+                           int ksize, int accumulate, int grp_images, void* stream, const float* act_y, float act_slope) {
   SST_REQUIRE(x && dy && slab && dw, "sst_conv_wgrad: null pointer");
   SST_REQUIRE(B > 0 && H > 0 && W > 0 && Cin > 0 && Cout > 0 && (stride == 1 || stride == 2) && (ksize & 1) && ksize <= 9,
               "sst_conv_wgrad: bad shape");
   const WgradPlan pl = wgrad_plan(B, H, W, Cin, Cout, ksize, stride, 1, in_scale != nullptr, in_act, false);
   const bool grouped = grp_images > 0 && grp_images < B && in_scale;
+  SST_REQUIRE(!act_y || pl.dyact, "sst_conv_wgrad_dyact: the kernel of this shape does not take the fused form (B=%d H=%d W=%d Cin=%d Cout=%d)",
+              B, H, W, Cin, Cout);
   SST_REQUIRE(!grouped || (B % grp_images == 0 && pl.kind == WgKind::TILE),
               "sst_conv_wgrad: coefficient groups are only taken by the all-taps tile kernel (B=%d H=%d W=%d Cin=%d Cout=%d stride=%d)", B, H, W,
               Cin, Cout, stride);
@@ -1116,7 +1138,10 @@
       break;
     }
     case WgKind::K3C3_MFMA:
-      wgrad_k3c3_mfma_kernel<<<pl.nchunk, CONV_NT, 0, st>>>(x, dy, slab, B, H, W, B * H * (W >> 5));
+      if (act_y)
+        wgrad_k3c3_mfma_kernel<true><<<pl.nchunk, CONV_NT, 0, st>>>(x, dy, act_y, act_slope, slab, B, H, W, B * H * (W >> 5));
+      else
+        wgrad_k3c3_mfma_kernel<false><<<pl.nchunk, CONV_NT, 0, st>>>(x, dy, nullptr, 0.f, slab, B, H, W, B * H * (W >> 5));
       SST_LAUNCH_CHECK("wgrad_k3c3_mfma_kernel");
       c3m_reduce_kernel<<<9 * 64 * 3 / C3R_OUT, 1024, 0, st>>>(slab, dw, pl.nchunk, accumulate & 1);
       SST_LAUNCH_CHECK("c3m_reduce_kernel");
@@ -1135,6 +1160,26 @@
   launch_wgrad_reduce(slab, dw, pl.nchunk, KK, Cout, Cin, accumulate, nullptr, 1, st);
   SST_LAUNCH_CHECK("wgrad_reduce_kernel");
   return SST_OK;
+}
+
+SST_API int sst_conv_wgrad_grp(const float* x, const float* dy, float* slab, float* dw, const float* in_scale,
+                               const float* in_shift, const float* in_slope, float in_slope_const, int in_act, int B, int H,
+                               int W, int Cin, int Cout, int stride, int ksize, int accumulate, int grp_images, void* stream) {
+  return conv_wgrad_impl(x, dy, slab, dw, in_scale, in_shift, in_slope, in_slope_const, in_act, B, H, W, Cin, Cout, stride, ksize,
+                         accumulate, grp_images, stream, nullptr, 0.f);
+}
+
+SST_API int sst_conv_wgrad_dyact_supported(int B, int H, int W, int Cin, int Cout, int ksize, int stride) {
+  if (B <= 0 || H <= 0 || W <= 0 || Cin <= 0 || Cout <= 0 || (stride != 1 && stride != 2) || !(ksize & 1) || ksize > 9) return 0;
+  return sst_l0_dyact_enabled() && wgrad_plan(B, H, W, Cin, Cout, ksize, stride, 1, false, ACT_NONE, false).dyact ? 1 : 0;
+}
+
+SST_API int sst_conv_wgrad_dyact(const float* x, const float* g, const float* act_y, float act_slope, float* slab, float* dw, int B, int H,
+                                 int W, int Cin, int Cout, int stride, int ksize, int accumulate, void* stream) {
+  SST_REQUIRE(act_y, "sst_conv_wgrad_dyact: null pointer");
+  SST_REQUIRE(sst_conv_wgrad_dyact_supported(B, H, W, Cin, Cout, ksize, stride), "sst_conv_wgrad_dyact: shape not taken (or SST_L0_DYACT=0)");
+  return conv_wgrad_impl(x, g, slab, dw, nullptr, nullptr, nullptr, 0.f, ACT_NONE, B, H, W, Cin, Cout, stride, ksize, accumulate, 0, stream,
+                         act_y, act_slope);
 }
 
 SST_API int sst_conv_wgrad(const float* x, const float* dy, float* slab, float* dw, const float* in_scale,
diff --git a/srgan-st_amd/srganst/_abi.py b/srgan-st_amd/srganst/_abi.py
--- a/srgan-st_amd/srganst/_abi.py
+++ b/srgan-st_amd/srganst/_abi.py
@@ -75,6 +75,10 @@
     "sst_conv_wgrad_grp": (c_int, [P, P, P, P, P, P, P, c_float, c_int, c_int, c_int, c_int, c_int, c_int,
                                    c_int, c_int, c_int, c_int, P]),
     "sst_conv_wgrad_grouped": (c_int, [P, c_int, c_int, c_int, c_int, c_int, c_int, c_int, c_int, c_int, P]),
+    "sst_conv_dgrad_dyact_supported": (c_int, [c_int, c_int, c_int, c_int, c_int, c_int]),
+    "sst_conv_dgrad_dyact": (c_int, [P, P, c_float, P, P, c_int, c_int, c_int, c_int, c_int, c_int, P]),
+    "sst_conv_wgrad_dyact_supported": (c_int, [c_int, c_int, c_int, c_int, c_int, c_int, c_int]),
+    "sst_conv_wgrad_dyact": (c_int, [P, P, P, c_float, P, P, c_int, c_int, c_int, c_int, c_int, c_int, c_int, c_int, P]),
     "sst_conv_wgrad_pending_reduce": (c_int, [c_int, c_int, c_int, c_int, c_int, c_int, c_int, c_int, c_int]),
     "sst_wgrad_reduce_multi": (c_int, [P, c_int, P]),
     "sst_bn_finalize": (c_int, [P, P, c_int, c_int, P, P, P, P, P, P, P, P, c_float, c_float, P]),
diff --git a/srgan-st_amd/srganst/disc_graph.py b/srgan-st_amd/srganst/disc_graph.py
--- a/srgan-st_amd/srganst/disc_graph.py
+++ b/srgan-st_amd/srganst/disc_graph.py
@@ -235,7 +235,19 @@
         n = y.numel() // y.shape[-1] // groups
         ci, bi = r["ci"], r["bi"]
         w = p[f"features.{ci}.weight"]
-        if bi is not None:
+        fused = False
+        if li == 0 and bi is None and r["stride"] == 1:
+            Bq, Hq, Wq, cin0 = r["x"].shape
+            fused = ((not wg or ops.conv_wgrad_dyact_supported(Bq, Hq, Wq, cin0, w.shape[0], 3, 1))
+                     and (not need_dx or ops.conv_dgrad_dyact_supported(Bq, Hq, Wq, w.shape[0], cin0, 3)))
+        act_kw = dict(act_y=y, act_slope=LRELU) if fused else {}
+        if fused:
+            dy = g
+            if wg:
+                if part is None:
+                    part = ops.bwd_reduce(g, y, slope_const=LRELU, act=1, groups=groups)
+                ops.bwd_finalize(part, n, dbeta=G(f"features.{ci}.bias"), accumulate=acc, groups=groups)
+        elif bi is not None:
             gam = p[f"features.{bi}.weight"]
             dg = G(f"features.{bi}.weight") if wg else torch.empty_like(gam)
             db = G(f"features.{bi}.bias") if wg else torch.empty_like(gam)
@@ -251,15 +263,15 @@
         if wg:
             dwc = G(f"features.{ci}.weight")
 
-            def launch(r=r, dy=dy, dwc=dwc, red=None):
+            def launch(r=r, dy=dy, dwc=dwc, red=None, act_kw=act_kw):
                 ops.conv_wgrad(r["x"], dy, dwc, 3, r["stride"], in_scale=r["x_scale"], in_shift=r["x_shift"],
-                               in_slope_const=LRELU, in_act=r["x_act"], accumulate=acc, grp=gB, defer_reduce=red)
+                               in_slope_const=LRELU, in_act=r["x_act"], accumulate=acc, grp=gB, defer_reduce=red, **act_kw)
             if defer_wgrad is not None and (defer_below is None or li < defer_below):
                 ev = torch.cuda.Event()
                 ev.record()
-                defer_wgrad.append((ev, launch, (r["x"], dy, dwc, r["x_scale"], r["x_shift"])))
+                defer_wgrad.append((ev, launch, (r["x"], dy, dwc, r["x_scale"], r["x_shift"], act_kw.get("act_y"))))
             else:
-                with ops.SideStream(r["x"], dy, dwc):
+                with ops.SideStream(*[t for t in (r["x"], dy, dwc, act_kw.get("act_y")) if t is not None]):
                     launch(red=reduces)
         if li == 0 and not need_dx:
             break
@@ -271,7 +283,7 @@
                                                   epi_scale=prev["scale"], epi_shift=prev["shift"], epi_slope_const=LRELU,
                                                   epi_act=1, grp=gB)
             else:
-                g = ops.conv_fwd(dy, wd[f"features.{ci}.weight"], w.shape[1], 3, 1)[0]
+                g = ops.conv_fwd(dy, wd[f"features.{ci}.weight"], w.shape[1], 3, 1, **act_kw)[0]
         else:
             prev = sv["layers"][li - 1] if li > 0 else None
             epi = None
diff --git a/srgan-st_amd/srganst/ops.py b/srgan-st_amd/srganst/ops.py
--- a/srgan-st_amd/srganst/ops.py
+++ b/srgan-st_amd/srganst/ops.py
@@ -85,8 +85,17 @@
 
 def conv_fwd(x, wp, cout, ksize=3, stride=1, bias=None, in_scale=None, in_shift=None, in_slope=None,
              in_slope_const=0.0, in_act=ACT_NONE, residual=None, want_stats=False, out_mode=OUT_NHWC,
-             want_pre=False, grp=0, out=None):
+             want_pre=False, grp=0, out=None, act_y=None, act_slope=0.0):
     B, H, W, cin = x.shape
+    if act_y is not None:
+        assert (stride == 1 and out_mode == OUT_NHWC and bias is None and in_scale is None and in_act == ACT_NONE and residual is None
+                and not want_stats and not want_pre and out is None)
+        assert act_y.shape == x.shape and act_y.is_contiguous() and x.is_contiguous()
+        y = _f32(B, H, W, cout, like=x)
+        args = (ptr(x), ptr(act_y), float(act_slope), ptr(wp), ptr(y), B, H, W, cin, cout, ksize)
+        _launch(_abi.lib().sst_conv_dgrad_dyact, args, "sst_conv_dgrad_dyact", 2.0 * B * H * W * cout * cin * ksize * ksize,
+                lambda: _conv_name(B, H, W, cin, cout, ksize, 1), (x, act_y, wp, y))
+        return y, None, None, None
     if grp and grp < B and in_scale is not None and not (out_mode == OUT_NHWC and residual is None and not want_pre
                                                          and conv_pipe_groups_ok(B, H, W, cin, cout, ksize, stride, grp)):
         raise _abi.HipPathError(f"conv_fwd: coefficient groups of {grp} images are not supported for this shape")
@@ -125,6 +134,14 @@
     return y, y_pre, stats, cnt
 
 
+def conv_dgrad_dyact_supported(B, H, W, cin, cout, ksize=3):
+    return bool(_abi.lib().sst_conv_dgrad_dyact_supported(B, H, W, cin, cout, ksize))
+
+
+def conv_wgrad_dyact_supported(B, H, W, cin, cout, ksize=3, stride=1):
+    return bool(_abi.lib().sst_conv_wgrad_dyact_supported(B, H, W, cin, cout, ksize, stride))
+
+
 def conv_pipe_tw(B, H, W, cin, cout, ksize, stride):
     if os.environ.get("SST_CONV_PIPE", "1") == "0":
         return 0
@@ -259,13 +276,20 @@
 
 
 def conv_wgrad(x, dy, dw_out, ksize=3, stride=1, in_scale=None, in_shift=None, in_slope=None, in_slope_const=0.0,
-               in_act=ACT_NONE, accumulate=False, grp=0, defer_reduce=None):
+               in_act=ACT_NONE, accumulate=False, grp=0, defer_reduce=None, act_y=None, act_slope=0.0):
     B, H, W, cin = x.shape
     cout = dy.shape[-1]
     ho, wo = conv_out_hw(H, W, ksize, stride)
     assert tuple(dy.shape) == (B, ho, wo, cout) and tuple(dw_out.shape) == (cout, cin, ksize, ksize)
     nch = _abi.lib().sst_conv_wgrad_chunks2(B, H, W, cin, cout, ksize, stride, 1)
     slab = _f32(nch * ksize * ksize * cout * cin, like=x)
+    if act_y is not None:
+        assert in_scale is None and in_act == ACT_NONE and act_y.shape == dy.shape and act_y.is_contiguous() and dy.is_contiguous()
+        args = (ptr(x), ptr(dy), ptr(act_y), float(act_slope), ptr(slab), ptr(dw_out), B, H, W, cin, cout, stride, ksize,
+                int(bool(accumulate)))
+        _launch(_abi.lib().sst_conv_wgrad_dyact, args, "sst_conv_wgrad_dyact", 2.0 * B * ho * wo * cout * cin * ksize * ksize,
+                lambda: _wgrad_name(B, H, W, cin, cout, ksize, stride, 1) + "+c3m_reduce_kernel", (x, dy, act_y, slab, dw_out))
+        return dw_out
     pend = 0
     if defer_reduce is not None and PROFILE is None and TRACE is None:
         pend = _abi.lib().sst_conv_wgrad_pending_reduce(B, H, W, cin, cout, ksize, stride, int(in_scale is not None), int(in_act))
```

New measurement: 3289 HR images/s, median of 6. No clear change (+0.8%).
